# wenxuanliu/multimodal-vae

Measured on AMD Instinct MI355X. Metric: ELBO-steps/sec (whole node), MultiMNIST b=256 per GPU, higher is better.
Workload: dtype bf16; 1 GPU; multimnist_50x50_conv_mmvae_gru_text_3pass_elbo_step; batch_per_gpu=256, global_batch=256, n_latents=100, parallelism=dp1, hip_graph=False, optimizer=adam, mfma=bf16 in / fp32 acc; fp32 master weights, BN stats, PoE/KL/BCE/NLL, Adam

## Files before the change

multimodal-vae_amd/csrc/conv1.hip:

```cpp
#include "thin.h"
#include "convres_epi.h"

namespace {

constexpr int C1_IMG = 50, C1_OH = 25, C1_NPIX = 625, C1_TILES = 20, C1_ROWS = 640, C1_C = 32;
constexpr int C1_HW = 52;
constexpr int C1_PP = 48;
constexpr int C1_AP = 80;

typedef __attribute__((address_space(3))) s16x4 lds_s16x4e;
__device__ __forceinline__ bf16x8 tr_pair_e(const char* a0, const char* a1) {
    union { struct { s16x4 a, b; } s; bf16x8 v; } u;
    u.s.a = __builtin_amdgcn_ds_read_tr16_b64_v4i16((lds_s16x4e*)a0);
    u.s.b = __builtin_amdgcn_ds_read_tr16_b64_v4i16((lds_s16x4e*)a1);
    return u.v;
}

template <int NTHR>
__device__ __forceinline__ void c1_patches(const float* img, bf16* img_s, char* pat_s, int tid) {
    for (int i = tid; i < C1_HW * C1_HW; i += NTHR) {
        const int y = i / C1_HW - 1, x = i - (y + 1) * C1_HW - 1;
        img_s[i] = ((unsigned)y < (unsigned)C1_IMG && (unsigned)x < (unsigned)C1_IMG) ? (bf16)img[y * C1_IMG + x] : (bf16)0.f;
    }
    __syncthreads();
    for (int px = tid; px < C1_ROWS; px += NTHR) {
        bf16x8 lo, hi;
        if (px < C1_NPIX) {
            const int oy = px / C1_OH, ox = px - oy * C1_OH;
            const bf16* d0 = img_s + (2 * oy) * C1_HW + 2 * ox;
#pragma unroll
            for (int kw = 0; kw < 4; ++kw) {
                lo[kw] = d0[kw]; lo[4 + kw] = d0[C1_HW + kw];
                hi[kw] = d0[2 * C1_HW + kw]; hi[4 + kw] = d0[3 * C1_HW + kw];
            }
        } else {
#pragma unroll
            for (int j = 0; j < 8; ++j) { lo[j] = (bf16)0.f; hi[j] = (bf16)0.f; }
        }
        *reinterpret_cast<bf16x8*>(pat_s + px * C1_PP) = lo;
        *reinterpret_cast<bf16x8*>(pat_s + px * C1_PP + 16) = hi;
    }
    __syncthreads();
}

struct Conv1FwdArgs { const float* image; int B; const bf16* Wp; int Kpad; bf16* r1; bf16* a1; };

constexpr int C1F_WAVES = 4, C1F_NTHR = C1F_WAVES * 64;
constexpr int C1F_OFF_IMG = 0, C1F_OFF_PAT = C1F_OFF_IMG + ((C1_HW * C1_HW * 2 + 15) / 16) * 16, C1F_OFF_SCR = C1F_OFF_PAT + C1_ROWS * C1_PP,
              C1F_LDS = C1F_OFF_SCR + C1F_WAVES * 2560;

__global__ __launch_bounds__(C1F_NTHR) void conv1_fwd_mfma_kernel(const Conv1FwdArgs a) {
    extern __shared__ __attribute__((aligned(16))) char smem[];
    const int tid = threadIdx.x, lane = tid & 63;
    const int wave = __builtin_amdgcn_readfirstlane(tid >> 6);
    const int r = lane & 31, h = lane >> 5;
    const int n = blockIdx.x;
    c1_patches<C1F_NTHR>(a.image + (size_t)n * (C1_IMG * C1_IMG), reinterpret_cast<bf16*>(smem + C1F_OFF_IMG), smem + C1F_OFF_PAT, tid);
    const bf16x8 wb = *reinterpret_cast<const bf16x8*>(a.Wp + (size_t)r * a.Kpad + 8 * h);
    const size_t bytes = (size_t)a.B * C1_NPIX * C1_C * 2;
    const __amdgpu_buffer_rsrc_t rsrc_r = __builtin_amdgcn_make_buffer_rsrc(a.r1, 0, (int)bytes, 0x00020000);
    const __amdgpu_buffer_rsrc_t rsrc_a = __builtin_amdgcn_make_buffer_rsrc(a.a1, 0, (int)bytes, 0x00020000);
    char* const scr = smem + C1F_OFF_SCR + wave * 2560;
    float s1 = 0.f, s2 = 0.f;
    for (int t = wave; t < C1_TILES; t += C1F_WAVES) {
        f32x16 acc;
#pragma unroll
        for (int j = 0; j < 16; ++j) acc[j] = 0.f;
        const bf16x8 pa = *reinterpret_cast<const bf16x8*>(smem + C1F_OFF_PAT + (t * 32 + r) * C1_PP + h * 16);
        acc = __builtin_amdgcn_mfma_f32_32x32x16_bf16(pa, wb, acc, 0, 0, 0);
        const unsigned base = (unsigned)(((size_t)n * C1_NPIX + t * 32) * (C1_C * 2)) + (unsigned)((lane >> 4) * 16);
        const int p0 = t * 32 + (lane & 15), p1 = p0 + 16;
        const unsigned off0 = p0 < C1_NPIX ? base + (unsigned)((lane & 15) * (C1_C * 2)) : 0x40000000u;
        const unsigned off1 = p1 < C1_NPIX ? base + (unsigned)((16 + (lane & 15)) * (C1_C * 2)) : 0x40000000u;
        f32x16 act;
#pragma unroll
        for (int j = 0; j < 16; ++j) act[j] = swish_fast(acc[j]);
        cr_epilogue_tile<0, false>(acc, scr, lane, 32, off0, off1, rsrc_r, rsrc_r, 1.f, 0.f, 0.f, 0.f, s1, s2, true);
        cr_epilogue_tile<0, false>(act, scr, lane, 32, off0, off1, rsrc_a, rsrc_a, 1.f, 0.f, 0.f, 0.f, s1, s2, true);
    }
}

struct Conv1WgradArgs { const float* image; int B; const bf16* d1; float* dWp; int Kpad; };

constexpr int C1W_WAVES = 8, C1W_NTHR = C1W_WAVES * 64;
constexpr int C1W_OFF_D = 0, C1W_OFF_IMG = C1W_OFF_D + C1_ROWS * C1_AP, C1W_OFF_PAT = C1W_OFF_IMG + ((C1_HW * C1_HW * 2 + 15) / 16) * 16,
              C1W_OFF_RED = C1W_OFF_PAT + C1_ROWS * C1_PP, C1W_LDS = C1W_OFF_RED + C1W_WAVES * C1_C * 16 * 4;

__global__ __launch_bounds__(C1W_NTHR) void conv1_wgrad_mfma_kernel(const Conv1WgradArgs a) {
    extern __shared__ __attribute__((aligned(16))) char smem[];
    const int tid = threadIdx.x, lane = tid & 63;
    const int wave = __builtin_amdgcn_readfirstlane(tid >> 6);
    const int r = lane & 31, h = lane >> 5;
    const int n = blockIdx.x;
    char* const D_s = smem + C1W_OFF_D;
    {
        constexpr int NV = C1_NPIX * 4;
        const bf16* src = a.d1 + (size_t)n * C1_NPIX * C1_C;
        for (int v = tid; v < C1_ROWS * 4; v += C1W_NTHR) {
            i32x4c val = {0, 0, 0, 0};
            if (v < NV) val = *reinterpret_cast<const i32x4c*>(src + (size_t)v * 8);
            *reinterpret_cast<i32x4c*>(D_s + (v >> 2) * C1_AP + (v & 3) * 16) = val;
        }
    }
    c1_patches<C1W_NTHR>(a.image + (size_t)n * (C1_IMG * C1_IMG), reinterpret_cast<bf16*>(smem + C1W_OFF_IMG), smem + C1W_OFF_PAT, tid);
    const int g4 = lane >> 4, q = (lane & 15) >> 2, p = lane & 3;
    f32x16 acc;
#pragma unroll
    for (int j = 0; j < 16; ++j) acc[j] = 0.f;
    for (int ks = wave; ks < C1_ROWS / 16; ks += C1W_WAVES) {
        const int row = ks * 16 + 8 * h + q;
        const char* a0 = D_s + row * C1_AP + (16 * (g4 & 1) + 4 * p) * 2;
        const char* b0 = smem + C1W_OFF_PAT + row * C1_PP + (4 * p) * 2;
        acc = __builtin_amdgcn_mfma_f32_32x32x16_bf16(tr_pair_e(a0, a0 + 4 * C1_AP), tr_pair_e(b0, b0 + 4 * C1_PP), acc, 0, 0, 0);
    }
    float* wred = reinterpret_cast<float*>(smem + C1W_OFF_RED) + wave * (C1_C * 16);
    if (r < 16) {
#pragma unroll
        for (int j = 0; j < 16; ++j) wred[((j & 3) + 8 * (j >> 2) + 4 * h) * 16 + r] = acc[j];
    }
    __syncthreads();
    {
        const float* wr = reinterpret_cast<const float*>(smem + C1W_OFF_RED);
        for (int i = tid; i < C1_C * 16; i += C1W_NTHR) {
            float s = 0.f;
#pragma unroll
            for (int w = 0; w < C1W_WAVES; ++w) s += wr[w * C1_C * 16 + i];
            atomicAdd(a.dWp + (size_t)(i >> 4) * a.Kpad + (i & 15), s);
        }
    }
}

}

int launch_conv1_fwd_mfma(const float* image, int B, const bf16* Wp, int Kpad, bf16* r1, bf16* a1, hipStream_t s) {
    MMVAE_REQUIRE(image && Wp && r1 && a1 && Kpad >= 16 && (size_t)B * C1_NPIX * C1_C * 2 < 0x40000000ull, "conv1 fwd: arguments");
    Conv1FwdArgs a{image, B, Wp, Kpad, r1, a1};
    MMVAE_LAUNCH(conv1_fwd_mfma_kernel, dim3(B), dim3(C1F_NTHR), C1F_LDS, s, a);
    return mmvae_check_launch("conv1_fwd_mfma");
}
int launch_conv1_wgrad_mfma(const float* image, int B, const bf16* d1, float* dWp, int Kpad, hipStream_t s) {
    MMVAE_REQUIRE(image && d1 && dWp && Kpad >= 16, "conv1 wgrad: arguments");
    static std::atomic<unsigned> attr_set{0};
    if (mmvae_first_use_on_device(attr_set))
        hipFuncSetAttribute(reinterpret_cast<const void*>(&conv1_wgrad_mfma_kernel), hipFuncAttributeMaxDynamicSharedMemorySize, C1W_LDS);
    Conv1WgradArgs a{image, B, d1, dWp, Kpad};
    MMVAE_LAUNCH(conv1_wgrad_mfma_kernel, dim3(B), dim3(C1W_NTHR), C1W_LDS, s, a);
    return mmvae_check_launch("conv1_wgrad_mfma");
}
```

multimodal-vae_amd/csrc/convres_epi.h:

```cpp
#pragma once
#include "common.h"

namespace {

typedef __attribute__((ext_vector_type(16))) float f32x16;
typedef __attribute__((ext_vector_type(4))) int i32x4c;

__device__ __forceinline__ float dswish_fast(float x) {
    const float s = __builtin_amdgcn_rcpf(1.0f + __expf(-x));
    return s * (1.0f + x * (1.0f - s));
}
__device__ __forceinline__ float swish_fast(float x) { return x * __builtin_amdgcn_rcpf(1.0f + __expf(-x)); }

typedef __attribute__((ext_vector_type(2))) float f32x2;
typedef __attribute__((address_space(3))) s16x4 lds_s16x4c;

template <int MODE, bool PARTIAL>
__device__ __forceinline__ void cr_epilogue_tile(const f32x16& acc, char* scr, int lane, int rows_valid, unsigned off0, unsigned off1,
                                                 __amdgpu_buffer_rsrc_t orsrc, __amdgpu_buffer_rsrc_t rrsrc, float dsc, float dsh,
                                                 float dmean, float drstd, float& s1, float& s2, bool store) {
    constexpr int SP = 80;
    const int r = lane & 31, h = lane >> 5, g = lane >> 4, i = lane & 15, q = i >> 2, p = i & 3;
    float v[16];
#pragma unroll
    for (int j = 0; j < 16; ++j) v[j] = acc[j];
    if constexpr (MODE == 1) {
        const i32x4c r0 = __builtin_bit_cast(i32x4c, __builtin_amdgcn_raw_buffer_load_b128(rrsrc, (int)off0, 0, 0));
        const i32x4c r1 = __builtin_bit_cast(i32x4c, __builtin_amdgcn_raw_buffer_load_b128(rrsrc, (int)off1, 0, 0));
        *reinterpret_cast<i32x4c*>(scr + i * SP + g * 16) = r0;
        *reinterpret_cast<i32x4c*>(scr + (16 + i) * SP + g * 16) = r1;
        asm volatile("" ::: "memory");
        const char* rb = scr + (4 * h + q) * SP + (16 * ((lane >> 4) & 1) + 4 * p) * 2;
        f32x2 t1 = {0.f, 0.f}, t2 = {0.f, 0.f};
#pragma unroll
        for (int k = 0; k < 4; ++k) {
            const bf16x4 rv = __builtin_bit_cast(bf16x4, __builtin_amdgcn_ds_read_tr16_b64_v4i16((lds_s16x4c*)(rb + 8 * k * SP)));
#pragma unroll
            for (int e = 0; e < 4; e += 2) {
                const f32x2 rr = {(float)rv[e], (float)rv[e + 1]};
                const f32x2 x = rr * dsc + dsh;
                f32x2 d = {dswish_fast(x[0]), dswish_fast(x[1])};
                f32x2 o = {v[4 * k + e], v[4 * k + e + 1]};
                o *= d;
                if constexpr (PARTIAL) {
                    const int row = 8 * k + 4 * h + e;
                    o[0] = row < rows_valid ? o[0] : 0.f;
                    o[1] = row + 1 < rows_valid ? o[1] : 0.f;
                }
                t1 += o;
                t2 += o * ((rr - dmean) * drstd);
                v[4 * k + e] = o[0]; v[4 * k + e + 1] = o[1];
            }
        }
        s1 += t1[0] + t1[1];
        s2 += t2[0] + t2[1];
        asm volatile("" ::: "memory");
    } else {
        f32x2 t1 = {0.f, 0.f}, t2 = {0.f, 0.f};
#pragma unroll
        for (int j = 0; j < 16; j += 2) {
            f32x2 o = {v[j], v[j + 1]};
            if constexpr (PARTIAL) {
                const int row = (j & 3) + 8 * (j >> 2) + 4 * h;
                o[0] = row < rows_valid ? o[0] : 0.f;
                o[1] = row + 1 < rows_valid ? o[1] : 0.f;
                v[j] = o[0]; v[j + 1] = o[1];
            }
            t1 += o;
            t2 += o * o;
        }
        s1 += t1[0] + t1[1];
        s2 += t2[0] + t2[1];
    }
#pragma unroll
    for (int k = 0; k < 4; ++k) {
        bf16x4 o;
#pragma unroll
        for (int e = 0; e < 4; ++e) o[e] = (bf16)v[4 * k + e];
        *reinterpret_cast<bf16x4*>(scr + r * SP + (8 * k + 4 * h) * 2) = o;
    }
    asm volatile("" ::: "memory");
    if (store) {
        const char* ob = scr + (8 * g + q) * SP + (4 * p) * 2;
        union { struct { s16x4 a, b; } s; i32x4c v; } u0, u1;
        u0.s.a = __builtin_amdgcn_ds_read_tr16_b64_v4i16((lds_s16x4c*)(ob));
        u0.s.b = __builtin_amdgcn_ds_read_tr16_b64_v4i16((lds_s16x4c*)(ob + 4 * SP));
        u1.s.a = __builtin_amdgcn_ds_read_tr16_b64_v4i16((lds_s16x4c*)(ob + 32));
        u1.s.b = __builtin_amdgcn_ds_read_tr16_b64_v4i16((lds_s16x4c*)(ob + 4 * SP + 32));
        __builtin_amdgcn_raw_buffer_store_b128(u0.v, orsrc, (int)off0, 0, 0);
        __builtin_amdgcn_raw_buffer_store_b128(u1.v, orsrc, (int)off1, 0, 0);
    }
    asm volatile("" ::: "memory");
}

}
```

multimodal-vae_amd/csrc/dec_last.hip:

```cpp
#include "thin.h"
#include "bn_dev.h"
#include "convres_epi.h"

namespace {

constexpr int DL_IH = 25, DL_IW = 25, DL_OH = 50, DL_OW = 50, DL_C = 32, DL_NPIX = 625, DL_TILES = 20, DL_ROWS = 640;
constexpr int DL_AP = 80;
constexpr int DL_PP = 48;
constexpr int DL_DLW = 52;
constexpr int DL_WAVES = 8, DL_NTHR = DL_WAVES * 64;
constexpr int DL_OFF_A = 0;
constexpr int DL_OFF_P = DL_OFF_A + DL_ROWS * DL_AP;
constexpr int DL_OFF_DL = DL_OFF_P + DL_ROWS * 64;
constexpr int DL_OFF_SCR = DL_OFF_DL + DL_DLW * DL_DLW * 4;
constexpr int DL_OFF_TAB = DL_OFF_SCR + DL_WAVES * 2560;
constexpr int DL_LDS = DL_OFF_TAB + 2 * DL_C * 8;
static_assert(DL_ROWS * DL_PP <= DL_ROWS * 64, "the patches reuse the P buffer");
static_assert(DL_LDS <= 160 * 1024, "LDS budget");

typedef __attribute__((address_space(3))) s16x4 lds_s16x4d;
__device__ __forceinline__ bf16x8 tr_pair_d(const char* a0, const char* a1) {
    union { struct { s16x4 a, b; } s; bf16x8 v; } u;
    u.s.a = __builtin_amdgcn_ds_read_tr16_b64_v4i16((lds_s16x4d*)a0);
    u.s.b = __builtin_amdgcn_ds_read_tr16_b64_v4i16((lds_s16x4d*)a1);
    return u.v;
}

template <bool IW>
__global__ __launch_bounds__(DL_NTHR) void dec_last_mfma_kernel(const DecLastFusedArgs a) {
    extern __shared__ __attribute__((aligned(16))) char smem[];
    char* const A_s = smem + DL_OFF_A;
    float* const P_s = reinterpret_cast<float*>(smem + DL_OFF_P);
    char* const pat_s = smem + DL_OFF_P;
    float* const dl_s = reinterpret_cast<float*>(smem + DL_OFF_DL);
    char* const scr_s = smem + DL_OFF_SCR;
    float2* const aff_s = reinterpret_cast<float2*>(smem + DL_OFF_TAB);
    float2* const mr_s = aff_s + DL_C;
    __shared__ float part[DL_WAVES];

    const int tid = threadIdx.x, lane = tid & 63;
    const int wave = __builtin_amdgcn_readfirstlane(tid >> 6);
    const int r = lane & 31, h = lane >> 5;
    const int n_in_g = blockIdx.x, g = blockIdx.y;
    const long long n = (long long)g * a.B + n_in_g;
    const BnFinalizeArgs& f = a.fin;
    const bool bwd = g < a.bwd_groups;

    constexpr int NV = DL_NPIX * 4, IT = (NV + DL_NTHR - 1) / DL_NTHR;
    i32x4c rv[IT];
#pragma unroll
    for (int it = 0; it < IT; ++it) {
        const int v = tid + it * DL_NTHR;
        if (v < NV) rv[it] = *reinterpret_cast<const i32x4c*>(a.r + (size_t)n * DL_NPIX * DL_C + (size_t)v * 8);
    }
    if (tid < DL_C) {
        float2 aff, mr;
        bn_channel_tables(f, g, tid, aff, mr);
        aff_s[tid] = aff; mr_s[tid] = mr;
    }
    if (!IW && blockIdx.x == 0 && blockIdx.y == 0) {
        for (int i = tid; i < f.G * DL_C; i += DL_NTHR) {
            float2 aff, mr;
            bn_channel_tables(f, i / DL_C, i % DL_C, aff, mr);
            f.affine[i] = aff; f.meanrstd[i] = mr;
        }
        bn_running_update(f, tid, DL_NTHR);
    }
    {
        const i32x4c z = {0, 0, 0, 0};
        for (int i = tid * 16; i < (DL_ROWS - DL_NPIX) * DL_AP; i += DL_NTHR * 16)
            *reinterpret_cast<i32x4c*>(A_s + DL_NPIX * DL_AP + i) = z;
        if (!IW)
            for (int i = tid; i < DL_DLW * DL_DLW; i += DL_NTHR) dl_s[i] = 0.f;
    }
    bf16x8 wf[2], wd;
#pragma unroll
    for (int ks = 0; ks < 2; ++ks)
#pragma unroll
        for (int j = 0; j < 8; ++j) wf[ks][j] = r < 16 ? (bf16)a.w[(ks * 16 + 8 * h + j) * 16 + r] : (bf16)0.f;
#pragma unroll
    for (int j = 0; j < 8; ++j) wd[j] = (bf16)a.w[r * 16 + 8 * h + j];
    __syncthreads();
    {
        const int cv = tid & 3;
        float sc[8], sh[8];
#pragma unroll
        for (int j = 0; j < 8; ++j) { const float2 t = aff_s[cv * 8 + j]; sc[j] = t.x; sh[j] = t.y; }
#pragma unroll
        for (int it = 0; it < IT; ++it) {
            const int v = tid + it * DL_NTHR;
            if (v < NV) {
                const bf16x8 x = __builtin_bit_cast(bf16x8, rv[it]);
                bf16x8 o;
#pragma unroll
                for (int j = 0; j < 8; ++j) o[j] = (bf16)swish_fast((float)x[j] * sc[j] + sh[j]);
                *reinterpret_cast<bf16x8*>(A_s + (v >> 2) * DL_AP + cv * 16) = o;
            }
        }
    }
    __syncthreads();
    for (int t = wave; t < DL_TILES; t += DL_WAVES) {
        f32x16 acc;
#pragma unroll
        for (int j = 0; j < 16; ++j) acc[j] = 0.f;
        const char* ap = A_s + (t * 32 + r) * DL_AP + h * 16;
        const bf16x8 a0 = *reinterpret_cast<const bf16x8*>(ap), a1 = *reinterpret_cast<const bf16x8*>(ap + 32);
        acc = __builtin_amdgcn_mfma_f32_32x32x16_bf16(a0, wf[0], acc, 0, 0, 0);
        acc = __builtin_amdgcn_mfma_f32_32x32x16_bf16(a1, wf[1], acc, 0, 0, 0);
        if (r < 16) {
#pragma unroll
            for (int j = 0; j < 16; ++j) P_s[(t * 32 + (j & 3) + 8 * (j >> 2) + 4 * h) * 16 + r] = acc[j];
        }
    }
    __syncthreads();
    if constexpr (IW) {
        const float* const timg = a.target + (long long)(n / a.rows_per_target) * (DL_OH * DL_OW);
        float ll = 0.f;
        for (int o = tid; o < DL_OH * DL_OW; o += DL_NTHR) {
            const int oy = o / DL_OW, ox = o - oy * DL_OW;
            const int kh0 = (oy + 1) & 1, kw0 = (ox + 1) & 1;
            const int iy0 = (oy + 1 - kh0) >> 1, ix0 = (ox + 1 - kw0) >> 1;
            float acc = 0.f;
#pragma unroll
            for (int ty = 0; ty < 2; ++ty)
#pragma unroll
                for (int tx = 0; tx < 2; ++tx) {
                    const int iy = iy0 - ty, ix = ix0 - tx;
                    if ((unsigned)iy < (unsigned)DL_IH && (unsigned)ix < (unsigned)DL_IW)
                        acc += P_s[(iy * DL_IW + ix) * 16 + (kh0 + 2 * ty) * 4 + kw0 + 2 * tx];
                }
            ll += timg[o] * acc - (fmaxf(acc, 0.f) + log1pf(expf(-fabsf(acc))));
        }
        ll = wave_sum(ll);
        if (lane == 0) part[wave] = ll;
        __syncthreads();
        if (tid == 0) {
            float s = 0.f;
            for (int w = 0; w < DL_WAVES; ++w) s += part[w];
            a.loglik[n] = s;
        }
        return;
    }
    float loss = 0.f;
    for (int o = tid; o < DL_OH * DL_OW; o += DL_NTHR) {
        const int oy = o / DL_OW, ox = o - oy * DL_OW;
        const int kh0 = (oy + 1) & 1, kw0 = (ox + 1) & 1;
        const int iy0 = (oy + 1 - kh0) >> 1, ix0 = (ox + 1 - kw0) >> 1;
        float acc = 0.f;
#pragma unroll
        for (int ty = 0; ty < 2; ++ty)
#pragma unroll
            for (int tx = 0; tx < 2; ++tx) {
                const int iy = iy0 - ty, ix = ix0 - tx;
                if ((unsigned)iy < (unsigned)DL_IH && (unsigned)ix < (unsigned)DL_IW)
                    acc += P_s[(iy * DL_IW + ix) * 16 + (kh0 + 2 * ty) * 4 + kw0 + 2 * tx];
            }
        const long long oidx = n * (DL_OH * DL_OW) + o;
        const float p = __builtin_amdgcn_rcpf(1.0f + __expf(-acc));
        if (a.logits) a.logits[oidx] = acc;
        if (a.recon) a.recon[oidx] = p;
        if (a.target) {
            const float t = a.target[(long long)n_in_g * (DL_OH * DL_OW) + o];
            const float lp = fmaxf(__logf(p), -100.f), lq = fmaxf(__logf(1.0f - p), -100.f);
            loss += -(t * lp + (1.0f - t) * lq);
            const float pq = p * (1.0f - p);
            const float dl = a.coef[g] * (p - t) / fmaxf(pq, 1e-12f) * pq;
            if (a.dlogit) a.dlogit[oidx] = dl;
            dl_s[(oy + 1) * DL_DLW + ox + 1] = dl;
        }
    }
    if (a.loss_sum) {
        loss = wave_sum(loss);
        if (lane == 0) part[wave] = loss;
    }
    __syncthreads();
    if (a.loss_sum && tid == 0) {
        float s = 0.f;
        for (int w = 0; w < DL_WAVES; ++w) s += part[w];
        atomicAdd(a.loss_sum + (blockIdx.x % MMVAE_LOSS_SLOTS) * 16 + g, s);
    }
    if (!bwd) return;
    for (int px = tid; px < DL_ROWS; px += DL_NTHR) {
        bf16x8 lo, hi;
        if (px < DL_NPIX) {
            const int iy = px / DL_IW, ix = px - iy * DL_IW;
            const float* d0 = dl_s + (2 * iy) * DL_DLW + 2 * ix;
#pragma unroll
            for (int kw = 0; kw < 4; ++kw) {
                lo[kw] = (bf16)d0[kw]; lo[4 + kw] = (bf16)d0[DL_DLW + kw];
                hi[kw] = (bf16)d0[2 * DL_DLW + kw]; hi[4 + kw] = (bf16)d0[3 * DL_DLW + kw];
            }
        } else {
#pragma unroll
            for (int j = 0; j < 8; ++j) { lo[j] = (bf16)0.f; hi[j] = (bf16)0.f; }
        }
        *reinterpret_cast<bf16x8*>(pat_s + px * DL_PP) = lo;
        *reinterpret_cast<bf16x8*>(pat_s + px * DL_PP + 16) = hi;
    }
    __syncthreads();
    {
        const __amdgpu_buffer_rsrc_t orsrc = __builtin_amdgcn_make_buffer_rsrc(
            a.db, 0, (int)((size_t)a.bwd_groups * a.B * DL_NPIX * DL_C * 2), 0x00020000);
        const __amdgpu_buffer_rsrc_t rrsrc = __builtin_amdgcn_make_buffer_rsrc(
            const_cast<bf16*>(a.r), 0, (int)((size_t)a.bwd_groups * a.B * DL_NPIX * DL_C * 2), 0x00020000);
        const float2 af = aff_s[r], mr = mr_s[r];
        float s1 = 0.f, s2 = 0.f;
        char* const scr = scr_s + wave * 2560;
        for (int t = wave; t < DL_TILES; t += DL_WAVES) {
            f32x16 acc;
#pragma unroll
            for (int j = 0; j < 16; ++j) acc[j] = 0.f;
            const bf16x8 pa = *reinterpret_cast<const bf16x8*>(pat_s + (t * 32 + r) * DL_PP + h * 16);
            acc = __builtin_amdgcn_mfma_f32_32x32x16_bf16(pa, wd, acc, 0, 0, 0);
            const unsigned base = (unsigned)((n * DL_NPIX + t * 32) * (DL_C * 2)) + (unsigned)((lane >> 4) * 16);
            const int p0 = t * 32 + (lane & 15), p1 = p0 + 16;
            const unsigned off0 = p0 < DL_NPIX ? base + (unsigned)((lane & 15) * (DL_C * 2)) : 0x40000000u;
            const unsigned off1 = p1 < DL_NPIX ? base + (unsigned)((16 + (lane & 15)) * (DL_C * 2)) : 0x40000000u;
            const int left = DL_NPIX - t * 32;
            if (left >= 32) cr_epilogue_tile<1, false>(acc, scr, lane, 32, off0, off1, orsrc, rrsrc, af.x, af.y, mr.x, mr.y, s1, s2, true);
            else cr_epilogue_tile<1, true>(acc, scr, lane, left, off0, off1, orsrc, rrsrc, af.x, af.y, mr.x, mr.y, s1, s2, true);
        }
        const float t1 = s1 + __shfl_xor(s1, 32, 64), t2 = s2 + __shfl_xor(s2, 32, 64);
        if (h == 0) {
            const int slot = (int)(blockIdx.x + wave) % MMVAE_STAT_SLOTS;
            float2* d = a.red + ((size_t)g * MMVAE_STAT_SLOTS + slot) * DL_C + r;
            atomicAdd(&d->x, t1);
            atomicAdd(&d->y, t2);
        }
    }
    __syncthreads();
    {
        const int g4 = lane >> 4, q = (lane & 15) >> 2, p = lane & 3;
        f32x16 acc;
#pragma unroll
        for (int j = 0; j < 16; ++j) acc[j] = 0.f;
        for (int ks = wave; ks < DL_ROWS / 16; ks += DL_WAVES) {
            const int row = ks * 16 + 8 * h + q;
            const char* a0 = A_s + row * DL_AP + (16 * (g4 & 1) + 4 * p) * 2;
            const char* b0 = pat_s + row * DL_PP + (4 * p) * 2;
            const bf16x8 af2 = tr_pair_d(a0, a0 + 4 * DL_AP);
            const bf16x8 bf2 = tr_pair_d(b0, b0 + 4 * DL_PP);
            acc = __builtin_amdgcn_mfma_f32_32x32x16_bf16(af2, bf2, acc, 0, 0, 0);
        }
        float* wred = reinterpret_cast<float*>(scr_s) + wave * (DL_C * 16);
        if (r < 16) {
#pragma unroll
            for (int j = 0; j < 16; ++j) wred[((j & 3) + 8 * (j >> 2) + 4 * h) * 16 + r] = acc[j];
        }
    }
    __syncthreads();
    {
        const float* wred = reinterpret_cast<const float*>(scr_s);
        float* dst = a.wslab + ((size_t)g * gridDim.x + blockIdx.x) * DL_C * 16;
        for (int i = tid; i < DL_C * 16; i += DL_NTHR) {
            float s = 0.f;
#pragma unroll
            for (int w = 0; w < DL_WAVES; ++w) s += wred[w * DL_C * 16 + i];
            dst[i] = s;
        }
    }
}

constexpr int CL_IH = 32, CL_IW = 32, CL_OH = 64, CL_OW = 64, CL_C = 32, CL_CO = 3, CL_J = 48, CL_SR = 8, CL_NS = CL_IH / CL_SR;
constexpr int CL_NPIX = CL_IH * CL_IW;
constexpr int CL_AROWS = CL_SR + 2, CL_APX = CL_AROWS * CL_IW, CL_ATILES = CL_APX / 32;
constexpr int CL_OPX = CL_SR * CL_IW, CL_OTILES = CL_OPX / 32;
constexpr int CL_AP = 80;
constexpr int CL_PF = 49;
constexpr int CL_PP = 144;
constexpr int CL_DLR = 2 * CL_SR + 2, CL_DLW = CL_OW + 2;
constexpr int CL_WAVES = 8, CL_NTHR = CL_WAVES * 64;
constexpr int CL_OFF_A = 0;
constexpr int CL_OFF_P = CL_OFF_A + CL_APX * CL_AP;
constexpr int CL_P_BYTES = CL_APX * CL_PF * 4;
constexpr int CL_OFF_DL = CL_OFF_P + (CL_P_BYTES + 15) / 16 * 16;
constexpr int CL_OFF_SCR = CL_OFF_DL + (CL_CO * CL_DLR * CL_DLW * 4 + 15) / 16 * 16;
constexpr int CL_OFF_TAB = CL_OFF_SCR + CL_WAVES * 2560;
constexpr int CL_LDS = CL_OFF_TAB + 2 * CL_C * 8;
static_assert(CL_OPX * CL_PP <= CL_P_BYTES && CL_WAVES * CL_C * CL_J * 4 <= CL_P_BYTES, "patches / dW partials reuse the P buffer");
static_assert(CL_LDS <= 160 * 1024 - 64, "LDS budget");
static_assert(CL_OTILES == CL_WAVES, "one owned 32-pixel tile per wave");

__global__ __launch_bounds__(CL_NTHR) void dec_last_ca_kernel(const DecLastFusedArgs a) {
    extern __shared__ __attribute__((aligned(16))) char smem[];
    char* const A_s = smem + CL_OFF_A;
    float* const P_s = reinterpret_cast<float*>(smem + CL_OFF_P);
    char* const pat_s = smem + CL_OFF_P;
    float* const dl_s = reinterpret_cast<float*>(smem + CL_OFF_DL);
    char* const scr_s = smem + CL_OFF_SCR;
    float2* const aff_s = reinterpret_cast<float2*>(smem + CL_OFF_TAB);
    float2* const mr_s = aff_s + CL_C;
    __shared__ float part[CL_WAVES];

    const int tid = threadIdx.x, lane = tid & 63;
    const int wave = __builtin_amdgcn_readfirstlane(tid >> 6);
    const int r = lane & 31, h = lane >> 5;
    const int n_in_g = blockIdx.x, g = blockIdx.y;
    const long long n = (long long)g * a.B + n_in_g;
    const BnFinalizeArgs& f = a.fin;
    const bool bwd = g < a.bwd_groups;

    if (tid < CL_C) {
        float2 aff, mr;
        bn_channel_tables(f, g, tid, aff, mr);
        aff_s[tid] = aff; mr_s[tid] = mr;
    }
    if (blockIdx.x == 0 && blockIdx.y == 0) {
        for (int i = tid; i < f.G * CL_C; i += CL_NTHR) {
            float2 aff, mr;
            bn_channel_tables(f, i / CL_C, i % CL_C, aff, mr);
            f.affine[i] = aff; f.meanrstd[i] = mr;
        }
        bn_running_update(f, tid, CL_NTHR);
    }
    bf16x8 wf[2][2], wd[3];
#pragma unroll
    for (int ks = 0; ks < 2; ++ks)
#pragma unroll
        for (int nt = 0; nt < 2; ++nt) {
            const int j = nt * 32 + r, tap = j / CL_CO, co = j - tap * CL_CO;
#pragma unroll
            for (int e = 0; e < 8; ++e) wf[ks][nt][e] = j < CL_J ? (bf16)a.w[((ks * 16 + 8 * h + e) * CL_CO + co) * 16 + tap] : (bf16)0.f;
        }
#pragma unroll
    for (int ks = 0; ks < 3; ++ks)
#pragma unroll
        for (int e = 0; e < 8; ++e) {
            const int j = ks * 16 + 8 * h + e, tap = j / CL_CO, co = j - tap * CL_CO;
            wd[ks][e] = (bf16)a.w[(r * CL_CO + co) * 16 + tap];
        }
    __syncthreads();
    const int cv = tid & 3;
    float sc[8], sh[8];
#pragma unroll
    for (int e = 0; e < 8; ++e) { const float2 t = aff_s[cv * 8 + e]; sc[e] = t.x; sh[e] = t.y; }
    const float2 af = aff_s[r], mr = mr_s[r];

    const __amdgpu_buffer_rsrc_t orsrc = __builtin_amdgcn_make_buffer_rsrc(
        a.db, 0, (int)((size_t)a.bwd_groups * a.B * CL_NPIX * CL_C * 2), 0x00020000);
    const __amdgpu_buffer_rsrc_t rrsrc = __builtin_amdgcn_make_buffer_rsrc(
        const_cast<bf16*>(a.r), 0, (int)((size_t)a.bwd_groups * a.B * CL_NPIX * CL_C * 2), 0x00020000);
    f32x16 accw[2];
#pragma unroll
    for (int nt = 0; nt < 2; ++nt)
#pragma unroll
        for (int e = 0; e < 16; ++e) accw[nt][e] = 0.f;
    float s1 = 0.f, s2 = 0.f, loss = 0.f;
    const bf16* const rimg = a.r + (size_t)n * CL_NPIX * CL_C;
    constexpr int NV = CL_APX * 4, IT = (NV + CL_NTHR - 1) / CL_NTHR;

    constexpr int NO = CL_CO * CL_DLR * CL_OW;
    constexpr int ND = CL_CO * CL_DLR * CL_DLW, DT = (ND + CL_NTHR - 1) / CL_NTHR;
    i32x4c rv[IT];
    auto fetch_rows = [&](int y0) {
#pragma unroll
        for (int it = 0; it < IT; ++it) {
            const int v = tid + it * CL_NTHR, px = v >> 2, iy = y0 - 1 + px / CL_IW;
            rv[it] = i32x4c{0, 0, 0, 0};
            if (v < NV && (unsigned)iy < (unsigned)CL_IH)
                rv[it] = *reinterpret_cast<const i32x4c*>(rimg + ((size_t)(iy * CL_IW + (px & (CL_IW - 1))) * CL_C + cv * 8));
        }
    };
    fetch_rows(0);
    const float* const timg = a.target ? a.target + (size_t)n_in_g * CL_CO * CL_OH * CL_OW : nullptr;
    float tv[DT];
    auto fetch_targets = [&](int y0) {
#pragma unroll
        for (int k = 0; k < DT; ++k) {
            const int i = tid + k * CL_NTHR;
            const int co = i / (CL_DLR * CL_DLW), rem = i - co * (CL_DLR * CL_DLW);
            const int lo = rem / CL_DLW, c = rem - lo * CL_DLW, oy = 2 * y0 - 1 + lo;
            tv[k] = 0.f;
            if (timg && i < ND && c >= 1 && c <= CL_OW && (unsigned)oy < (unsigned)CL_OH) tv[k] = timg[(co * CL_OH + oy) * CL_OW + c - 1];
        }
    };
    fetch_targets(0);

    for (int strip = 0; strip < CL_NS; ++strip) {
        const int y0 = strip * CL_SR;
        __syncthreads();
#pragma unroll
        for (int k = 0; k < DT; ++k) {
            const int i = tid + k * CL_NTHR;
            if (i < ND) dl_s[i] = tv[k];
        }
#pragma unroll
        for (int it = 0; it < IT; ++it) {
            const int v = tid + it * CL_NTHR, px = v >> 2, iy = y0 - 1 + px / CL_IW;
            if (v < NV) {
                bf16x8 o;
                if ((unsigned)iy < (unsigned)CL_IH) {
                    const bf16x8 x = __builtin_bit_cast(bf16x8, rv[it]);
#pragma unroll
                    for (int e = 0; e < 8; ++e) o[e] = (bf16)swish_fast((float)x[e] * sc[e] + sh[e]);
                } else {
#pragma unroll
                    for (int e = 0; e < 8; ++e) o[e] = (bf16)0.f;
                }
                *reinterpret_cast<bf16x8*>(A_s + px * CL_AP + cv * 16) = o;
            }
        }
        if (strip + 1 < CL_NS) { fetch_rows(y0 + CL_SR); fetch_targets(y0 + CL_SR); }
        __syncthreads();
        if (!(a.dbg & 16))
        for (int t = wave; t < CL_ATILES; t += CL_WAVES) {
            const char* ap = A_s + (t * 32 + r) * CL_AP + h * 16;
            const bf16x8 a0 = *reinterpret_cast<const bf16x8*>(ap), a1 = *reinterpret_cast<const bf16x8*>(ap + 32);
#pragma unroll
            for (int nt = 0; nt < 2; ++nt) {
                f32x16 acc;
#pragma unroll
                for (int e = 0; e < 16; ++e) acc[e] = 0.f;
                acc = __builtin_amdgcn_mfma_f32_32x32x16_bf16(a0, wf[0][nt], acc, 0, 0, 0);
                acc = __builtin_amdgcn_mfma_f32_32x32x16_bf16(a1, wf[1][nt], acc, 0, 0, 0);
                const int j = nt * 32 + r;
                if (j < CL_J) {
#pragma unroll
                    for (int e = 0; e < 16; ++e) P_s[(t * 32 + (e & 3) + 8 * (e >> 2) + 4 * h) * CL_PF + j] = acc[e];
                }
            }
        }
        __syncthreads();
#pragma unroll 2
        for (int o = (a.dbg & 1) ? NO : tid; o < NO; o += CL_NTHR) {
            const int co = o / (CL_DLR * CL_OW), rem = o - co * (CL_DLR * CL_OW);
            const int lo = rem / CL_OW, ox = rem - lo * CL_OW, oy = 2 * y0 - 1 + lo;
            if ((unsigned)oy >= (unsigned)CL_OH) continue;
            const int kh0 = (oy + 1) & 1, kw0 = (ox + 1) & 1;
            const int iy0 = (oy + 1 - kh0) >> 1, ix0 = (ox + 1 - kw0) >> 1;
            float acc = 0.f;
#pragma unroll
            for (int ty = 0; ty < 2; ++ty)
#pragma unroll
                for (int tx = 0; tx < 2; ++tx) {
                    const int iy = iy0 - ty, ix = ix0 - tx, ixc = min(max(ix, 0), CL_IW - 1);
                    const float pv = P_s[((iy - y0 + 1) * CL_IW + ixc) * CL_PF + ((kh0 + 2 * ty) * 4 + kw0 + 2 * tx) * CL_CO + co];
                    acc += ix == ixc ? pv : 0.f;
                }
            const bool owned = lo >= 1 && lo <= 2 * CL_SR;
            const long long oidx = ((n * CL_CO + co) * CL_OH + oy) * CL_OW + ox;
            const float p = __builtin_amdgcn_rcpf(1.0f + __expf(-acc));
            if (owned) {
                if (a.logits) a.logits[oidx] = acc;
                if (a.recon) a.recon[oidx] = p;
            }
            if (a.target) {
                const float t = dl_s[(co * CL_DLR + lo) * CL_DLW + ox + 1];
                const float pq = p * (1.0f - p);
                const float dl = a.coef[g] * (p - t) / fmaxf(pq, 1e-12f) * pq;
                if (owned) {
                    const float lp = fmaxf(__logf(p), -100.f), lq = fmaxf(__logf(1.0f - p), -100.f);
                    loss += -(t * lp + (1.0f - t) * lq);
                    if (a.dlogit) a.dlogit[oidx] = dl;
                }
                dl_s[(co * CL_DLR + lo) * CL_DLW + ox + 1] = dl;
            }
        }
        if (!bwd) continue;
        __syncthreads();
        if (!(a.dbg & 2)) {
            const int px = tid >> 1, half = tid & 1;
            const int iyl = px / CL_IW, ix = px - iyl * CL_IW;
            bf16 v[24];
#pragma unroll
            for (int kk = 0; kk < 2; ++kk)
#pragma unroll
                for (int kw = 0; kw < 4; ++kw)
#pragma unroll
                    for (int co = 0; co < CL_CO; ++co)
                        v[(kk * 4 + kw) * CL_CO + co] = (bf16)dl_s[(co * CL_DLR + 2 * iyl + 2 * half + kk) * CL_DLW + 2 * ix + kw];
            char* dst = pat_s + px * CL_PP + half * 48;
#pragma unroll
            for (int q = 0; q < 3; ++q) {
                bf16x8 o;
#pragma unroll
                for (int e = 0; e < 8; ++e) o[e] = v[q * 8 + e];
                *reinterpret_cast<bf16x8*>(dst + q * 16) = o;
            }
            if (half) {
                const i32x4c z = {0, 0, 0, 0};
                *reinterpret_cast<i32x4c*>(pat_s + px * CL_PP + 96) = z;
                *reinterpret_cast<i32x4c*>(pat_s + px * CL_PP + 112) = z;
            }
        }
        __syncthreads();
        if (!(a.dbg & 4)) {
            const int t = wave;
            f32x16 acc;
#pragma unroll
            for (int e = 0; e < 16; ++e) acc[e] = 0.f;
#pragma unroll
            for (int ks = 0; ks < 3; ++ks) {
                const bf16x8 pa = *reinterpret_cast<const bf16x8*>(pat_s + (t * 32 + r) * CL_PP + ks * 32 + h * 16);
                acc = __builtin_amdgcn_mfma_f32_32x32x16_bf16(pa, wd[ks], acc, 0, 0, 0);
            }
            const unsigned base = (unsigned)((n * CL_NPIX + y0 * CL_IW + t * 32) * (CL_C * 2)) + (unsigned)((lane >> 4) * 16);
            const unsigned off0 = base + (unsigned)((lane & 15) * (CL_C * 2)), off1 = base + (unsigned)((16 + (lane & 15)) * (CL_C * 2));
            cr_epilogue_tile<1, false>(acc, scr_s + wave * 2560, lane, 32, off0, off1, orsrc, rrsrc, af.x, af.y, mr.x, mr.y, s1, s2, true);
        }
        if (!(a.dbg & 8)) {
            const int g4 = lane >> 4, q = (lane & 15) >> 2, p = lane & 3;
            for (int ks = wave; ks < CL_OPX / 16; ks += CL_WAVES) {
                const int row = ks * 16 + 8 * h + q;
                const char* a0 = A_s + (row + CL_IW) * CL_AP + (16 * (g4 & 1) + 4 * p) * 2;
                const bf16x8 af2 = tr_pair_d(a0, a0 + 4 * CL_AP);
#pragma unroll
                for (int nt = 0; nt < 2; ++nt) {
                    const char* b0 = pat_s + row * CL_PP + (nt * 32 + 16 * (g4 & 1) + 4 * p) * 2;
                    const bf16x8 bf2 = tr_pair_d(b0, b0 + 4 * CL_PP);
                    accw[nt] = __builtin_amdgcn_mfma_f32_32x32x16_bf16(af2, bf2, accw[nt], 0, 0, 0);
                }
            }
        }
    }
    if (a.loss_sum) {
        loss = wave_sum(loss);
        if (lane == 0) part[wave] = loss;
    }
    __syncthreads();
    if (a.loss_sum && tid == 0) {
        float s = 0.f;
        for (int w = 0; w < CL_WAVES; ++w) s += part[w];
        atomicAdd(a.loss_sum + (blockIdx.x % MMVAE_LOSS_SLOTS) * 16 + g, s);
    }
    if (!bwd) return;
    {
        const float t1 = s1 + __shfl_xor(s1, 32, 64), t2 = s2 + __shfl_xor(s2, 32, 64);
        if (h == 0) {
            const int slot = (int)(blockIdx.x + wave) % MMVAE_STAT_SLOTS;
            float2* d = a.red + ((size_t)g * MMVAE_STAT_SLOTS + slot) * CL_C + r;
            atomicAdd(&d->x, t1);
            atomicAdd(&d->y, t2);
        }
    }
    float* const wred = P_s;
#pragma unroll
    for (int nt = 0; nt < 2; ++nt) {
        const int j = nt * 32 + r;
        if (j < CL_J) {
#pragma unroll
            for (int e = 0; e < 16; ++e) wred[(wave * CL_C + (e & 3) + 8 * (e >> 2) + 4 * h) * CL_J + j] = accw[nt][e];
        }
    }
    __syncthreads();
    float* dst = a.wslab + ((size_t)g * gridDim.x + blockIdx.x) * CL_C * CL_J;
    for (int i = tid; i < CL_C * CL_J; i += CL_NTHR) {
        float s = 0.f;
#pragma unroll
        for (int w = 0; w < CL_WAVES; ++w) s += wred[w * CL_C * CL_J + i];
        dst[i] = s;
    }
}

}

bool dec_last_ca_applies(const DecLastFusedArgs& a) {
    return a.Cin == CL_C && a.Cout == CL_CO && a.IH == CL_IH && a.IW == CL_IW && a.act == ACT_SWISH && mmvae_knob("dec_last_ca", 1) != 0 &&
           (size_t)a.G * a.B * CL_NPIX * CL_C * 2 < 0x40000000ull;
}
int launch_dec_last_ca(const DecLastFusedArgs& a, hipStream_t s) {
    MMVAE_REQUIRE(dec_last_ca_applies(a), "dec_last_ca: not the 32x32x32 -> 64x64x3 tail");
    MMVAE_REQUIRE(a.r && a.w && a.G >= 1 && a.B >= 1 && a.bwd_groups >= 0 && a.bwd_groups <= a.G, "dec_last_ca: arguments");
    MMVAE_REQUIRE(a.bwd_groups == 0 || (a.target && a.db && a.red && a.wslab), "dec_last_ca: backward outputs missing");
    static std::atomic<unsigned> attr_set{0};
    if (mmvae_first_use_on_device(attr_set))
        hipFuncSetAttribute(reinterpret_cast<const void*>(&dec_last_ca_kernel), hipFuncAttributeMaxDynamicSharedMemorySize, CL_LDS);
    DecLastFusedArgs b = a;
    b.dbg = mmvae_knob("dec_last_ca_dbg", 0);
    MMVAE_LAUNCH(dec_last_ca_kernel, dim3(a.B, a.G), dim3(CL_NTHR), CL_LDS, s, b);
    return mmvae_check_launch("dec_last_ca");
}

bool dec_last_mfma_applies(const DecLastFusedArgs& a) {
    return a.Cin == 32 && a.Cout == 1 && a.IH == DL_IH && a.IW == DL_IW && a.act == ACT_SWISH && mmvae_knob("dec_last_mfma", 1) != 0 &&
           (size_t)a.G * a.B * DL_NPIX * DL_C * 2 < 0x40000000ull;
}
int launch_dec_last_mfma(const DecLastFusedArgs& a, hipStream_t s) {
    static std::atomic<unsigned> attr_set{0};
    if (mmvae_first_use_on_device(attr_set)) {
        hipFuncSetAttribute(reinterpret_cast<const void*>(&dec_last_mfma_kernel<false>), hipFuncAttributeMaxDynamicSharedMemorySize, DL_LDS);
        hipFuncSetAttribute(reinterpret_cast<const void*>(&dec_last_mfma_kernel<true>), hipFuncAttributeMaxDynamicSharedMemorySize, DL_LDS);
    }
    if (a.loglik) {
        MMVAE_REQUIRE(a.target && a.rows_per_target >= 1 && a.bwd_groups == 0 && !a.fin.training, "dec_last_mfma: importance-weighted form arguments");
        MMVAE_LAUNCH(dec_last_mfma_kernel<true>, dim3(a.B, a.G), dim3(DL_NTHR), DL_LDS, s, a);
        return mmvae_check_launch("dec_last_mfma_iw");
    }
    MMVAE_LAUNCH(dec_last_mfma_kernel<false>, dim3(a.B, a.G), dim3(DL_NTHR), DL_LDS, s, a);
    return mmvae_check_launch("dec_last_mfma");
}
```

multimodal-vae_amd/csrc/multimnist.hip:

```cpp
#include "multimnist.h"
#include <memory>
#include "mlp_tail.h"
#include "plan_base.h"
#include "thin.h"
#include "text_plan.h"
#include <cstring>

namespace {
constexpr int IMG = 50, NPIX = 2500;
}

struct MMPlan : PlanBase {
    int ldz, kx, kz;
    int lde;
    ConvL conv[4], convT[4];
    LinL fc[3], up;
    BnL bn[6];
    int H = TXT_H;
    const char *te_name = "text_encoder", *td_name = "text_decoder";
    TextGruIdx te_f, te_r, td0, td1;
    const float* step_image = nullptr;
    hipEvent_t ev_dz = nullptr;
    hipEvent_t ev_txtgrads = nullptr;
    int te_h2p, te_h2pT, g_te_h2p, td_z2h, td_z2hT, g_td_z2h, td_h2o, td_h2oT, g_td_h2o;
    bool mlp_tail = false;
    int mt_w2, mt_w3, mt_w3t, mt_w2t;
    bool waist = false;
    int wa_w2, wa_w3, wa_w3t, wa_w2t;
    struct W {
        char* zero_begin; size_t zero_bytes;
        float2 *st_e[3], *red_e[3], *st_d[3], *red_d[3];
        float* sums; float* dz_img; float* dz_txt;
        float2 *aff_e[3], *mr_e[3], *aff_d[3], *mr_d[3];
        bf16 *patches1, *r1, *r2, *r3, *r4, *y1, *y2;
        bf16 *a1, *a2, *a3, *a4, *ay1, *ay2, *au, *aq1, *aq2, *aq3;
        float* encout; uint8_t *m1, *m2, *gkeep;
        float *txtout, *te_gates_f, *te_gates_r; bf16 *te_x, *te_hprev, *te_hsum;
        float *eps, *mu, *logvar, *z_f32; bf16* z_bf;
        bf16 *u, *q1, *q2, *q3; float *logits, *recon, *dlogit;
        float *words, *dwords, *td_gates; long long* tokens;
        bf16 *td_x0, *td_h0p, *td_mid, *td_h1p, *td_hz, *td_zbf;
        bf16 *dgi0, *dgh0, *dgi1, *dgh1, *dlogit_bf, *dhinit;
        bf16 *patches4, *d3, *d2, *d1, *du;
        bf16 *d_encout; float* d_txtout; bf16* te_dout_bf; bf16 *te_dgi_f, *te_dgh_f, *te_dgi_r;
        bf16 *dy2, *dy1, *db4, *dr4, *d3e, *d2e, *d1e;
        bf16 *d3r, *d2r, *d1r, *d3er, *d2er;
        float* tmp_f32;
        float* slab; size_t slab_floats;
    } w;
};

namespace {

void build_params(MMPlan& P) {
    const int D = P.D;
    auto bn = [&](const std::string& n, int c) { add_param(P, n + ".weight", {c}); add_param(P, n + ".bias", {c}); };
    add_param(P, "image_encoder.features.0.weight", {32, 1, 4, 4});
    add_param(P, "image_encoder.features.2.weight", {64, 32, 4, 4}); bn("image_encoder.features.3", 64);
    add_param(P, "image_encoder.features.5.weight", {128, 64, 4, 4}); bn("image_encoder.features.6", 128);
    add_param(P, "image_encoder.features.8.weight", {256, 128, 4, 4}); bn("image_encoder.features.9", 256);
    add_param(P, "image_encoder.classifier.0.weight", {400, 1024}); add_param(P, "image_encoder.classifier.0.bias", {400});
    add_param(P, "image_encoder.classifier.3.weight", {200, 400}); add_param(P, "image_encoder.classifier.3.bias", {200});
    add_param(P, "image_encoder.classifier.6.weight", {2 * D, 200}); add_param(P, "image_encoder.classifier.6.bias", {2 * D});
    add_param(P, "image_decoder.upsample.0.weight", {1024, D}); add_param(P, "image_decoder.upsample.0.bias", {1024});
    add_param(P, "image_decoder.hallucinate.0.weight", {256, 128, 4, 4}); bn("image_decoder.hallucinate.1", 128);
    add_param(P, "image_decoder.hallucinate.3.weight", {128, 64, 4, 4}); bn("image_decoder.hallucinate.4", 64);
    add_param(P, "image_decoder.hallucinate.6.weight", {64, 32, 5, 5}); bn("image_decoder.hallucinate.7", 32);
    add_param(P, "image_decoder.hallucinate.9.weight", {32, 1, 4, 4});
    text_add_encoder_params(P);
    text_add_decoder_params(P);
}

void build_plan(MMPlan& P) {
    const int D = P.D;
    P.ldz = round_up(D + 1, 8); P.kz = round_up(D, 32); P.kx = txt_kx(P.H, D);
    P.lde = round_up(2 * D, 8);
    build_params(P);
    const char* bnn[6] = {"image_encoder.features.3", "image_encoder.features.6", "image_encoder.features.9",
                          "image_decoder.hallucinate.1", "image_decoder.hallucinate.4", "image_decoder.hallucinate.7"};
    const int bnc[6] = {64, 128, 256, 128, 64, 32};
    long long so = 0;
    for (int i = 0; i < 6; ++i) {
        P.bn[i] = BnL{off(P, std::string(bnn[i]) + ".weight"), off(P, std::string(bnn[i]) + ".bias"), bnc[i], so, i};
        P.bn_names.push_back(bnn[i]); P.bn_list.push_back(P.bn[i]);
        so += 2 * bnc[i];
    }
    build_conv(P, P.conv[0], "image_encoder.features.0.weight", ConvGeom{1, 32, 4, 4, 2, 1, 50, 50, 25, 25, false}, -1, false, true, false);
    build_conv(P, P.conv[1], "image_encoder.features.2.weight", ConvGeom{32, 64, 4, 4, 2, 1, 25, 25, 12, 12, false}, 0, true, false, false);
    build_conv(P, P.conv[2], "image_encoder.features.5.weight", ConvGeom{64, 128, 4, 4, 2, 1, 12, 12, 6, 6, false}, 1, true, false, false);
    build_conv(P, P.conv[3], "image_encoder.features.8.weight", ConvGeom{128, 256, 4, 4, 2, 0, 6, 6, 2, 2, false}, 2, true, false, false);
    build_conv(P, P.convT[0], "image_decoder.hallucinate.0.weight", ConvGeom{256, 128, 4, 4, 2, 0, 2, 2, 6, 6, true}, 3, true, false, false);
    build_conv(P, P.convT[1], "image_decoder.hallucinate.3.weight", ConvGeom{128, 64, 4, 4, 2, 1, 6, 6, 12, 12, true}, 4, true, false, false);
    build_conv(P, P.convT[2], "image_decoder.hallucinate.6.weight", ConvGeom{64, 32, 5, 5, 2, 1, 12, 12, 25, 25, true}, 5, true, false, false);
    build_conv(P, P.convT[3], "image_decoder.hallucinate.9.weight", ConvGeom{32, 1, 4, 4, 2, 1, 25, 25, 50, 50, true}, -1, true, false, true);
    add_frag_packs(P, P.conv[2]);
    add_frag_packs(P, P.convT[1]);
    add_frag_packs(P, P.conv[3]);
    add_frag_packs(P, P.convT[0]);

    {
        LinL& f = P.fc[0];
        f.w_off = off(P, "image_encoder.classifier.0.weight"); f.b_off = off(P, "image_encoder.classifier.0.bias");
        f.N = 400; f.K = 1024; f.pk_dgrad = -1;
        PackDesc d = pack_dense(f.w_off, 400, 1024, npad_for(400), 1024, 1024, 0);
        d.TW = 2; d.C = 256; d.s_ty = 2; d.s_tx = 1; d.s_c = 4;
        f.pk_fwd = P.pk.add(d);
        PackDesc gd = d; gd.Npad = round_up(400, 64);
        f.gk = P.gk.add(gd);
        for (int sidx = 0; sidx < 4; ++sidx)
            f.pk_dgrad4[sidx] = P.pk.add(pack_dense(f.w_off + sidx, 256, 400, npad_for(256), round_up(400, 64), 4, 1024));
    }
    auto lin = [&](LinL& f, const std::string& n, int N, int K) {
        f.w_off = off(P, n + ".weight"); f.b_off = off(P, n + ".bias"); f.N = N; f.K = K;
        f.pk_fwd = P.pk.add(pack_dense(f.w_off, N, K, npad_for(N), round_up(round_up(K, 8), 64), K, 1));
        f.gk = P.gk.add(pack_dense(f.w_off, N, K, round_up(N, 64), round_up(round_up(K, 8), 64), K, 1));
        f.pk_dgrad = P.pk.add(pack_dense(f.w_off, K, N, npad_for(K), round_up(round_up(N, 8), 64), 1, K));
    };
    lin(P.fc[1], "image_encoder.classifier.3", 200, 400);
    lin(P.fc[2], "image_encoder.classifier.6", 2 * D, 200);
    if (D == 100) {
        P.mlp_tail = true;
        auto fragd = [&](PackDesc d) { d.frag = 1; return P.pk.add(d); };
        P.mt_w2 = fragd(pack_dense(P.fc[1].w_off, 200, 400, 208, 416, 400, 1));
        P.mt_w3 = fragd(pack_dense(P.fc[2].w_off, 200, 200, 208, 224, 200, 1));
        P.mt_w3t = fragd(pack_dense(P.fc[2].w_off, 200, 200, 208, 224, 1, 200));
        P.mt_w2t = fragd(pack_dense(P.fc[1].w_off, 400, 200, 400, 224, 1, 400));
        P.waist = true; P.wa_w2 = P.mt_w2; P.wa_w3 = P.mt_w3; P.wa_w3t = P.mt_w3t; P.wa_w2t = P.mt_w2t;
    } else if (mlp2_latent1_compiled(D)) {
        P.waist = true;
        auto fragd = [&](PackDesc d) { d.frag = 1; return P.pk.add(d); };
        P.wa_w2 = fragd(pack_dense(P.fc[1].w_off, 200, 400, 208, 416, 400, 1));
        P.wa_w3 = fragd(pack_dense(P.fc[2].w_off, 2 * D, 200, round_up(2 * D, 16), 224, 200, 1));
        P.wa_w3t = fragd(pack_dense(P.fc[2].w_off, 200, 2 * D, 208, round_up(2 * D, 32), 1, 200));
        P.wa_w2t = fragd(pack_dense(P.fc[1].w_off, 400, 200, 400, 224, 1, 400));
    }
    {
        LinL& f = P.up;
        f.w_off = off(P, "image_decoder.upsample.0.weight"); f.b_off = off(P, "image_decoder.upsample.0.bias");
        f.N = 1024; f.K = D;
        PackDesc d = pack_dense(f.w_off, 1024, D, npad_for(1024), round_up(P.ldz, 64), 0, 1);
        d.NL = 256; d.s_nhi = D; d.s_nlo = 4 * D;
        d.bias_off = f.b_off; d.b_nhi = 1; d.b_nlo = 4;
        f.pk_fwd = P.pk.add(d);
        PackDesc gd = d; f.gk = P.gk.add(gd);
        PackDesc t = pack_dense(f.w_off, D, 1024, npad_for(D), 1024, 1, 0);
        t.TW = 4; t.C = 256; t.s_ty = 0; t.s_tx = D; t.s_c = 4 * D;
        f.pk_dgrad = P.pk.add(t);
    }
    text_build_packs(P);
    for (PackDesc& d : P.pk.d) {
        d.part = 0;
        for (const ParamInfo& pi : P.params)
            if (d.src_off >= pi.offset && d.src_off < pi.offset + pi.numel)
                d.part = pi.name.rfind("text_", 0) == 0 ? 1 : pi.name.rfind("image_decoder.", 0) == 0 ? 2 : 0;
    }
    {
        auto late = [&](int idx) { if (idx >= 0) P.pk.d[idx].part = 2; };
        for (int l = 0; l < 4; ++l)
            for (int i = 0; i < 4; ++i) { late(P.conv[l].pk_dgrad[i]); late(P.conv[l].pk_dgrad_f[i]); }
        for (int i = 0; i < 4; ++i) late(P.fc[0].pk_dgrad4[i]);
        late(P.fc[1].pk_dgrad); late(P.fc[2].pk_dgrad);
        if (P.waist) { late(P.wa_w3t); late(P.wa_w2t); }
    }
    for (PackDesc& d : P.gk.d)
        for (const ParamInfo& pi : P.params)
            if (d.src_off >= pi.offset && d.src_off < pi.offset + pi.numel)
                d.part = pi.name.rfind("image_decoder.", 0) == 0 || pi.name.rfind("text_decoder.", 0) == 0;
}

void carve(MMPlan& P, Workspace& ws) {
    MMPlan::W& w = P.w;
    const size_t B = P.B, D = P.D, B3 = (size_t)P.carve_passes * B, B2 = (size_t)(P.carve_passes < 2 ? P.carve_passes : 2) * B;
    char* z0 = ws.take<char>(0);
    const int ec[3] = {64, 128, 256}, dc[3] = {128, 64, 32};
    const int SS = MMVAE_STAT_SLOTS;
    for (int i = 0; i < 3; ++i) { w.st_e[i] = ws.take<float2>(SS * ec[i]); w.red_e[i] = ws.take<float2>(SS * ec[i]); }
    for (int i = 0; i < 3; ++i) { w.st_d[i] = ws.take<float2>(3 * SS * dc[i]); w.red_d[i] = ws.take<float2>(3 * SS * dc[i]); }
    w.sums = ws.take<float>(16 * MMVAE_LOSS_SLOTS);
    P.sk_cnt = ws.take<unsigned>(1024);
    w.dz_img = ws.take<float>(B3 * D);
    w.dz_txt = ws.take<float>(B3 * D);
    char* z1 = ws.take<char>(0);
    w.zero_begin = z0; w.zero_bytes = (size_t)(z1 - z0);
    for (int i = 0; i < 3; ++i) { w.aff_e[i] = ws.take<float2>(ec[i]); w.mr_e[i] = ws.take<float2>(ec[i]); }
    for (int i = 0; i < 3; ++i) { w.aff_d[i] = ws.take<float2>(3 * dc[i]); w.mr_d[i] = ws.take<float2>(3 * dc[i]); }
    w.patches1 = ws.take<bf16>(B * 625 * 16);
    w.r1 = ws.take<bf16>(B * 625 * 32); w.r2 = ws.take<bf16>(B * 144 * 64); w.r3 = ws.take<bf16>(B * 36 * 128);
    w.r4 = ws.take<bf16>(B * 4 * 256);
    w.y1 = ws.take<bf16>(B2 * 400); w.y2 = ws.take<bf16>(B2 * 200);
    w.a1 = ws.take<bf16>(B * 625 * 32); w.a2 = ws.take<bf16>(B * 144 * 64); w.a3 = ws.take<bf16>(B * 36 * 128);
    w.a4 = ws.take<bf16>(B * 4 * 256); w.ay1 = ws.take<bf16>(B2 * 400); w.ay2 = ws.take<bf16>(B2 * 200);
    w.au = ws.take<bf16>(B3 * 1024); w.aq1 = ws.take<bf16>(B3 * 36 * 128); w.aq2 = ws.take<bf16>(B3 * 144 * 64);
    w.aq3 = ws.take<bf16>(B3 * 625 * 32);
    w.encout = ws.take<float>(B2 * 2 * D);
    w.m1 = ws.take<uint8_t>(B2 * 400); w.m2 = ws.take<uint8_t>(B2 * 200); w.gkeep = ws.take<uint8_t>(4 * B3 * P.H);
    carve_text_enc(w, ws, B, D, P.H);
    w.eps = ws.take<float>(B3 * D); w.mu = ws.take<float>(B3 * D); w.logvar = ws.take<float>(B3 * D);
    w.z_f32 = ws.take<float>(B3 * D); w.z_bf = ws.take<bf16>(B3 * P.ldz);
    w.u = ws.take<bf16>(B3 * 1024); w.q1 = ws.take<bf16>(B3 * 36 * 128); w.q2 = ws.take<bf16>(B3 * 144 * 64);
    w.q3 = ws.take<bf16>(B3 * 625 * 32);
    w.logits = ws.take<float>(B3 * NPIX); w.recon = ws.take<float>(B3 * NPIX); w.dlogit = ws.take<float>(B3 * NPIX);
    carve_text_dec(w, ws, B3, P.H, P.kx, P.kz);
    w.patches4 = ws.take<bf16>(B3 * 625 * 16);
    w.d3 = ws.take<bf16>(B3 * 625 * 32); w.d2 = ws.take<bf16>(B3 * 144 * 64); w.d1 = ws.take<bf16>(B3 * 36 * 128);
    w.du = ws.take<bf16>(B3 * 1024);
    w.d_encout = ws.take<bf16>(B2 * P.lde);
    carve_text_enc_bwd(w, ws, B, D, P.H);
    w.dy2 = ws.take<bf16>(B2 * 200); w.dy1 = ws.take<bf16>(B2 * 400);
    w.db4 = ws.take<bf16>(B2 * 1024); w.dr4 = ws.take<bf16>(B * 1024);
    w.d3e = ws.take<bf16>(B * 36 * 128); w.d2e = ws.take<bf16>(B * 144 * 64); w.d1e = ws.take<bf16>(B * 625 * 32);
    w.d3r = ws.take<bf16>(B3 * 625 * 32); w.d2r = ws.take<bf16>(B3 * 144 * 64); w.d1r = ws.take<bf16>(B3 * 36 * 128);
    w.d3er = ws.take<bf16>(B * 36 * 128); w.d2er = ws.take<bf16>(B * 144 * 64);
    w.tmp_f32 = ws.take<float>(B3 * NPIX);
    P.sk_floats = (size_t)256 * 128 * 128;
    P.sk_buf = ws.take<float>(P.sk_floats);
    w.slab_floats = (size_t)(P.carve_passes >= 3 ? 48 : 16) << 20;
    w.slab = ws.take<float>(w.slab_floats);
}

int enc_fwd(MMPlan& P, const float* image, int variants, const uint8_t* m1, const uint8_t* m2, int dropout, int training,
            int bn_updates, float* out, hipStream_t s, bool fuse = false, const Mlp2Latent1FwdArgs* waist = nullptr, bool tail_only = false) {
    MMPlan::W& w = P.w;
    const int B = P.B;
    const int rows = variants * B;
    const bool drop = training && dropout;
    const float ms = 1.f / (1.f - DROP_P);
    if (!tail_only) {
    if (fuse && mmvae_knob("mm_conv1_mfma", 1)) {
        const PackDesc& d = P.pk.d[P.conv[0].pk_fwd[0]];
        MMVAE_TRY(launch_conv1_fwd_mfma(image, B, P.buf.packed + d.dst_off, d.Kpad, w.r1, w.a1, s));
    } else {
    MMVAE_TRY(launch_im2col_small(image, B, 1, IMG, IMG, 4, 4, 2, 1, 25, 25, w.patches1, 16, s));
    {
        GatherPlan pl = dense_plan(B * 625, 16, 16, 32);
        GemmParams g = gemm_of(P, pl, P.conv[0].pk_fwd, 1, B * 625);
        g.c.A = w.patches1; g.out_bf = w.r1; g.ldo = 32; g.out_act_bf = w.a1; g.e_act = ACT_SWISH;
        MMVAE_TRY(launch_gemm_gather(g, s));
    }
    }
    bf16* r[4] = {w.r1, w.r2, w.r3, w.r4};
    bf16* a[4] = {w.a1, w.a2, w.a3, w.a4};
    for (int l = 1; l < 4; ++l) {
        const ConvL& L = P.conv[l];
        GemmParams g = gemm_of(P, L.fwd, L.pk_fwd, 1, B, L.pk_fwd_f);
        g.c.A = a[l - 1];
        g.out_bf = r[l]; g.ldo = L.g.Cout;
        g.colstats = training ? w.st_e[l - 1] : nullptr;
        GatherTransform tr{};
        if (fuse && l >= 2) {
            const int prows = B * P.conv[l - 1].g.OH * P.conv[l - 1].g.OW;
            tr.kind = 1;
            tr.fin = bn_fin_args(P, P.bn[P.conv[l - 1].bn], prows, 1, w.st_e[l - 2], bn_updates, w.aff_e[l - 2], w.mr_e[l - 2], training);
            g.c.A = r[l - 1]; g.tr = &tr;
            if (mmvae_knob("mm_stage_out", 1)) tr.out = a[l - 1];
        }
        MMVAE_TRY(launch_gemm_gather(g, s));
        const int rows = B * L.g.OH * L.g.OW;
        if (fuse && l <= 2) continue;
        MMVAE_TRY(bn_act(P, P.bn[L.bn], r[l], a[l], rows, rows, 1, w.st_e[l - 1], bn_updates, w.aff_e[l - 1], w.mr_e[l - 1], training, s));
    }
    {
        GatherPlan pl = plan_fwdform(2, 2, 1, 1, 256, 2, 2, 1, 0, 400, 1, rows);
        GemmParams g = gemm_of(P, pl, &P.fc[0].pk_fwd, 1, rows);
        g.c.A = w.a4; g.c.a_bcast_n = B;
        g.bias = P.buf.params + P.fc[0].b_off; g.out_bf = w.y1; g.ldo = 400;
        g.out_act_bf = w.ay1; g.e_act = ACT_SWISH; if (drop) { g.e_mask = m1; g.e_mask_scale = ms; }
        MMVAE_TRY(launch_gemm_gather(g, s));
    }
    }
    if (waist) {
        Mlp2Latent1FwdArgs a = *waist;
        a.rows = rows; a.x = w.ay1;
        a.w2 = P.buf.packed + P.pk.d[P.wa_w2].dst_off; a.b2 = P.buf.params + P.fc[1].b_off;
        a.w3 = P.buf.packed + P.pk.d[P.wa_w3].dst_off; a.b3 = P.buf.params + P.fc[2].b_off;
        if (drop) { a.mask = m2; a.mask_scale = ms; }
        a.y2 = w.y2; a.ay2 = w.ay2; a.out = out;
        return launch_mlp2_latent1_fwd(a, s);
    }
    if (P.mlp_tail) {
        Mlp2FwdArgs a{};
        a.rows = rows; a.x = w.ay1;
        a.w2 = P.buf.packed + P.pk.d[P.mt_w2].dst_off; a.b2 = P.buf.params + P.fc[1].b_off;
        a.w3 = P.buf.packed + P.pk.d[P.mt_w3].dst_off; a.b3 = P.buf.params + P.fc[2].b_off;
        if (drop) { a.mask = m2; a.mask_scale = ms; }
        a.y2 = w.y2; a.ay2 = w.ay2; a.out = out;
        return launch_mlp2_fwd(a, s);
    }
    {
        GatherPlan pl = dense_plan(rows, 400, 400, 200);
        GemmParams g = gemm_of(P, pl, &P.fc[1].pk_fwd, 1, rows);
        g.c.A = w.ay1;
        g.bias = P.buf.params + P.fc[1].b_off; g.out_bf = w.y2; g.ldo = 200;
        g.out_act_bf = w.ay2; g.e_act = ACT_SWISH; if (drop) { g.e_mask = m2; g.e_mask_scale = ms; }
        MMVAE_TRY(launch_gemm_gather(g, s));
    }
    {
        GatherPlan pl = dense_plan(rows, 200, 200, 2 * P.D);
        GemmParams g = gemm_of(P, pl, &P.fc[2].pk_fwd, 1, rows);
        g.c.A = w.ay2;
        g.bias = P.buf.params + P.fc[2].b_off; g.out_f = out; g.ldo = 2 * P.D;
        MMVAE_TRY(launch_gemm_gather(g, s));
    }
    return MMVAE_OK;
}

int enc_bwd(MMPlan& P, const bf16* d_out, int variants, const uint8_t* m1, const uint8_t* m2, int dropout, hipStream_t s, bool fuse = false,
            const Mlp2Latent1BwdArgs* waist = nullptr, float* loss_out = nullptr, bool tail_only = false) {
    MMPlan::W& w = P.w;
    const int B = P.B, rows = variants * B, D2 = 2 * P.D;
    const float ms = 1.f / (1.f - DROP_P);
    auto cls_w = std::make_shared<std::vector<WgradParams>>();
    if (waist) {
        Mlp2Latent1BwdArgs a = *waist;
        a.rows = rows;
        a.w3t = P.buf.packed + P.pk.d[P.wa_w3t].dst_off; a.w2t = P.buf.packed + P.pk.d[P.wa_w2t].dst_off;
        a.y2 = w.y2; a.y1 = w.y1;
        if (dropout) { a.mask2 = m2; a.mask1 = m1; a.mask_scale = ms; }
        a.dy2 = w.dy2; a.dy1 = w.dy1;
        a.db2 = P.buf.grads + P.fc[1].b_off; a.db1 = P.buf.grads + P.fc[0].b_off;
        a.d_enc_out = w.d_encout; a.lde = P.lde;
        MMVAE_TRY(launch_mlp2_latent1_bwd(a, s));
        {
            hipStream_t fs = s;
            MMVAE_TRY(wgrad_side_stream(P, s, &fs));
            MMVAE_TRY(launch_mlp2_latent1_finish(a.scratch, rows, P.D, P.buf.grads + P.fc[2].b_off, w.sums, loss_out, fs));
        }
        GatherPlan p3 = dense_plan(rows, 200, 200, D2);
        WgradParams g3 = wgrad_of(P, p3, &P.fc[2].gk, 1, rows);
        g3.c.A = w.ay2; g3.P = w.d_encout; g3.ldp = P.lde;
        MMVAE_TRY(wgrad_async(P, g3, s));
        GatherPlan p2 = dense_plan(rows, 400, 400, 200);
        WgradParams g2 = wgrad_of(P, p2, &P.fc[1].gk, 1, rows);
        g2.c.A = w.ay1; g2.P = w.dy2; g2.ldp = 200;
        MMVAE_TRY(wgrad_async(P, g2, s));
    } else if (P.mlp_tail) {
        {
            GatherPlan pl = dense_plan(rows, 200, 200, D2);
            WgradParams g = wgrad_of(P, pl, &P.fc[2].gk, 1, rows);
            g.c.A = w.ay2; g.P = d_out; g.ldp = P.lde;
            if (fuse) cls_w->push_back(g);
            else MMVAE_TRY(wgrad_async(P, g, s));
        }
        Mlp2BwdArgs a{};
        a.rows = rows; a.d_out = d_out;
        a.w3t = P.buf.packed + P.pk.d[P.mt_w3t].dst_off; a.w2t = P.buf.packed + P.pk.d[P.mt_w2t].dst_off;
        a.y2 = w.y2; a.y1 = w.y1;
        if (dropout) { a.mask2 = m2; a.mask1 = m1; a.mask_scale = ms; }
        a.dy2 = w.dy2; a.dy1 = w.dy1;
        a.db2 = P.buf.grads + P.fc[1].b_off; a.db1 = P.buf.grads + P.fc[0].b_off;
        MMVAE_TRY(launch_mlp2_bwd(a, s));
        GatherPlan pl = dense_plan(rows, 400, 400, 200);
        WgradParams g = wgrad_of(P, pl, &P.fc[1].gk, 1, rows);
        g.c.A = w.ay1; g.P = w.dy2; g.ldp = 200;
        if (fuse) cls_w->push_back(g);
        else MMVAE_TRY(wgrad_async(P, g, s));
    } else {
    {
        GatherPlan pl = dense_plan(rows, 200, 200, D2);
        WgradParams g = wgrad_of(P, pl, &P.fc[2].gk, 1, rows);
        g.c.A = w.ay2; g.P = d_out; g.ldp = P.lde;
        MMVAE_TRY(wgrad_async(P, g, s));
        GatherPlan pd = dense_plan(rows, P.lde, P.lde, 200);
        GemmParams d = gemm_of(P, pd, &P.fc[2].pk_dgrad, 1, rows);
        d.c.A = d_out; d.out_bf = w.dy2; d.ldo = 200;
        d.d_r = w.y2; d.d_ld = 200; d.d_act = ACT_SWISH; if (dropout) { d.d_mask = m2; d.d_mask_scale = ms; }
        d.d_colsum = P.buf.grads + P.fc[1].b_off;
        MMVAE_TRY(launch_gemm_gather(d, s));
    }
    {
        GatherPlan pl = dense_plan(rows, 400, 400, 200);
        WgradParams g = wgrad_of(P, pl, &P.fc[1].gk, 1, rows);
        g.c.A = w.ay1; g.P = w.dy2; g.ldp = 200;
        MMVAE_TRY(wgrad_async(P, g, s));
        GatherPlan pd = dense_plan(rows, 200, 200, 400);
        GemmParams d = gemm_of(P, pd, &P.fc[1].pk_dgrad, 1, rows);
        d.c.A = w.dy2; d.out_bf = w.dy1; d.ldo = 400;
        d.d_r = w.y1; d.d_ld = 400; d.d_act = ACT_SWISH; if (dropout) { d.d_mask = m1; d.d_mask_scale = ms; }
        d.d_colsum = P.buf.grads + P.fc[0].b_off;
        MMVAE_TRY(launch_gemm_gather(d, s));
    }
    }
    if (tail_only) return MMVAE_OK;
    {
        GatherPlan pl = plan_fwdform(2, 2, 1, 1, 256, 2, 2, 1, 0, 400, 1, rows);
        WgradParams g = wgrad_of(P, pl, &P.fc[0].gk, 1, rows);
        g.c.A = w.a4; g.c.a_bcast_n = B;
        g.P = w.dy1; g.ldp = 400;
        if (P.mlp_tail && fuse) {
            MMPlan* pp = &P;
            cls_w->push_back(g);
            side_later(P, [pp, cls_w](hipStream_t ws_) {
                MMVAE_TRY(launch_wgrad_group(cls_w->data(), (int)cls_w->size(), ws_, &pp->slab));
                return pp->batch_reduce ? MMVAE_OK : launch_wgrad_reduce(&pp->slab, ws_, true);
            }, mmvae_knob("mm_cls_lane", 1));
        } else {
            MMVAE_TRY(wgrad_async(P, g, s));
        }
        GatherPlan pd{};
        pd.c.AH = 1; pd.c.AW = 1; pd.c.Ald = 400; pd.c.C = 400; pd.c.sy = pd.c.sx = 1; pd.c.dy = pd.c.dx = 1;
        pd.c.OH = 2; pd.c.OW = 2; pd.c.osy = pd.c.osx = 1; pd.c.N = 256; pd.c.nclasses = 4;
        for (int sidx = 0; sidx < 4; ++sidx) {
            GatherClass& k = pd.cls[sidx];
            k.OY = 1; k.OX = 1; k.TH = 1; k.TW = 1; k.offy = 0; k.offx = 0; k.ooy = sidx / 2; k.oox = sidx % 2;
            k.K = 400; k.Kpad = round_up(400, 64);
        }
        GemmParams d = gemm_of(P, pd, P.fc[0].pk_dgrad4, 1, rows);
        d.c.A = w.dy1; d.out_bf = w.db4; d.ldo = 256;
        d.d_r = w.r4; d.d_ld = 256; d.d_bcast_n = B; d.d_act = ACT_SWISH;
        d.d_affine = w.aff_e[2]; d.d_meanrstd = w.mr_e[2]; d.d_red = w.red_e[2];
        MMVAE_TRY(launch_gemm_gather(d, s));
    }
    bf16* r[4] = {w.r1, w.r2, w.r3, w.r4};
    bf16* a[4] = {w.a1, w.a2, w.a3, w.a4};
    bf16* dr[4] = {w.d1e, w.d2e, w.d3e, w.dr4};
    bf16* drr[4] = {nullptr, w.d2er, w.d3er, nullptr};
    for (int l = 3; l >= 1; --l) {
        const ConvL& L = P.conv[l];
        const BnL& b = P.bn[L.bn];
        const int pix = L.g.OH * L.g.OW;
        const bool fl = fuse && l < 3;
        BnBwdApplyArgs x{};
        x.db = (l == 3) ? w.db4 : dr[l];
        x.db2 = (l == 3 && variants == 2) ? w.db4 + (size_t)B * 1024 : nullptr;
        x.r = r[l]; x.dr = fl ? drr[l] : dr[l]; x.rows = B * pix; x.C = L.g.Cout; x.ld = L.g.Cout; x.rows_per_group = B * pix; x.G = 1;
        x.red = w.red_e[l - 1]; x.meanrstd = w.mr_e[l - 1]; x.gamma = P.buf.params + b.w_off;
        x.dgamma = P.buf.grads + b.w_off; x.dbeta = P.buf.grads + b.b_off;
        if (!fl) MMVAE_TRY(launch_bn_bwd_apply(x, s));
        WgradParams gw = wgrad_of(P, L.fwd, L.gk, 1, B);
        gw.c.A = a[l - 1]; gw.P = x.dr; gw.ldp = L.g.Cout;
        if (fuse) {
            MMPlan* pp = &P;
            {
                const bool byp = mmvae_knob("mm_stage_out", 1) != 0;
                const bool actp = l >= 2 && !byp;
                const bool bnb = fl && !(byp && l == 2);
                const int prows = B * P.conv[l >= 2 ? l - 1 : 1].g.OH * P.conv[l >= 2 ? l - 1 : 1].g.OW;
                const BnL bp = P.bn[P.conv[l >= 2 ? l - 1 : 1].bn];
                const bf16* rin = r[l >= 2 ? l - 1 : 1]; bf16* ao = a[l >= 2 ? l - 1 : 1]; const float2* st = w.st_e[l >= 2 ? l - 2 : 0];
                WgradParams g0 = wgrad_of(P, L.fwd, L.gk, 1, B);
                g0.c.A = a[l - 1]; g0.P = x.dr; g0.ldp = L.g.Cout;
                side_later(P, [pp, x, g0, bnb, actp, bp, rin, ao, st, prows](hipStream_t ws_) {
                    if (bnb) MMVAE_TRY(launch_bn_bwd_apply(x, ws_));
                    if (actp) MMVAE_TRY(bn_act_side(*pp, bp, rin, ao, prows, prows, 1, st, 1, ws_));
                    return wgrad_on(*pp, g0, ws_);
                }, l == 1 ? 1 : l == 2 ? mmvae_knob("mm_conv3_lane", 0) : mmvae_knob("mm_conv4_lane", 0));
            }
            if (fuse && l == 1) MMVAE_TRY(side_flush(P, s));
        }
        {
            GemmParams d = gemm_of(P, L.dgrad, L.pk_dgrad, 1, B, L.pk_dgrad_f);
            d.c.A = dr[l]; d.out_bf = dr[l - 1]; d.ldo = L.g.Cin;
            d.d_r = r[l - 1]; d.d_ld = L.g.Cin; d.d_act = ACT_SWISH;
            if (l > 1) { d.d_affine = w.aff_e[l - 2]; d.d_meanrstd = w.mr_e[l - 2]; d.d_red = w.red_e[l - 2]; }
            GatherTransform tr{};
            if (fl) {
                tr.kind = 2; tr.r = r[l]; tr.red = w.red_e[l - 1]; tr.mr = w.mr_e[l - 1]; tr.gamma = P.buf.params + b.w_off;
                tr.inv_cnt = 1.f / (float)(B * pix); tr.groups = 1;
                if (l == 2 && mmvae_knob("mm_stage_out", 1)) {
                    tr.out = drr[l]; tr.dgamma = P.buf.grads + b.w_off; tr.dbeta = P.buf.grads + b.b_off;
                }
                d.tr = &tr;
            }
            const bool flush = fuse && P.wgrad_forked && (mmvae_knob("mm_forks", 0) ? l == 2 : l >= 2);
            if (flush) arm_fork(P);
            MMVAE_TRY(launch_gemm_gather(d, s));
            if (flush) { MMVAE_TRY(commit_fork(P, s)); MMVAE_TRY(side_flush(P, s)); }
        }
        if (!fuse) MMVAE_TRY(wgrad_async(P, gw, s));
    }
    if (fuse && !P.wgrad_forked) MMVAE_TRY(side_flush(P, s));
    if (fuse && mmvae_knob("mm_conv1_mfma", 1) && P.step_image) {
        const PackDesc& gd = P.gk.d[P.conv[0].gk[0]];
        MMVAE_TRY(launch_conv1_wgrad_mfma(P.step_image, B, w.d1e, P.buf.gpk + gd.dst_off, gd.Kpad, s));
    } else {
        GatherPlan pl = dense_plan(B * 625, 16, 16, 32);
        WgradParams g = wgrad_of(P, pl, P.conv[0].gk, 1, B * 625);
        g.c.A = w.patches1; g.P = w.d1e; g.ldp = 32;
        MMVAE_TRY(launch_wgrad(g, s, nullptr));
    }
    return MMVAE_OK;
}

int fused_tail(MMPlan& P, int groups, int training, const ConvTLastFwdArgs* last, int last_groups, int fused_bwd_groups, hipStream_t s) {
    MMPlan::W& w = P.w;
    const int B = P.B;
    const ConvL& L = P.convT[2];
    const BnL& b = P.bn[L.bn];
    DecLastFusedArgs x{};
    x.r = w.q3; x.act = ACT_SWISH; x.w = P.buf.params + P.convT[3].w_off;
    x.G = last_groups > 0 ? last_groups : groups; x.B = B; x.IH = 25; x.IW = 25; x.Cin = 32;
    x.bwd_groups = std::min(fused_bwd_groups, x.G);
    BnFinalizeArgs& f = x.fin;
    f.stats = w.st_d[2]; f.G = groups; f.C = b.C; f.count = (float)(B * L.g.OH * L.g.OW);
    f.gamma = P.buf.params + b.w_off; f.beta = P.buf.params + b.b_off;
    f.running_mean = P.buf.bn_stats + b.stat_off; f.running_var = P.buf.bn_stats + b.stat_off + b.C;
    f.num_batches_tracked = P.buf.bn_nbt + b.idx;
    f.updates_per_group = 1; f.affine = w.aff_d[2]; f.meanrstd = w.mr_d[2]; f.eps = BN_EPS; f.momentum = BN_MOM; f.training = training;
    f.skip_update_mask = groups > 1 ? P.dec_skip_mask : 0u;
    x.target = last->target; x.logits = last->logits; x.recon = last->recon; x.dlogit = nullptr;
    for (int k = 0; k < 4; ++k) x.coef[k] = last->coef[k];
    x.loss_sum = last->loss_sum;
    if (last->loglik) { x.loglik = last->loglik; x.rows_per_target = last->rows_per_target; x.B = last->rows; }
    if (x.bwd_groups > 0) {
        const int chunks = x.bwd_groups * B * (dec_last_mfma_applies(x) ? 1 : dec_last_fused_strips(25));
        x.wslab = P.slab.take((size_t)chunks * 32 * 16);
        MMVAE_REQUIRE(x.wslab != nullptr, "fused decoder tail: the weight-gradient slab pool is exhausted");
        x.db = w.d3; x.red = w.red_d[2];
        WgradSlabJob j{};
        const PackDesc& gd = P.gk.d[P.convT[3].gk[0]];
        j.dst = P.buf.gpk + gd.dst_off; j.slab = x.wslab; j.N = 32; j.K = 16; j.Kpad = gd.Kpad; j.chunks = chunks;
        j.chunk_stride = 32 * 16; j.src_ld = 16; j.stream = s;
        P.slab.jobs.push_back(j);
    }
    return launch_dec_last_fused(x, s);
}

int dec_fwd(MMPlan& P, int groups, int training, ConvTLastFwdArgs* last, hipStream_t s, int last_groups = -1, int fused_bwd_groups = -1,
            bool fuse = false) {
    MMPlan::W& w = P.w;
    const int B = P.B, rows = groups * B;
    {
        GatherPlan pl = dense_plan(rows, P.ldz, P.ldz, 1024);
        GemmParams g = gemm_of(P, pl, &P.up.pk_fwd, 1, rows);
        g.c.A = w.z_bf; g.out_bf = w.u; g.ldo = 1024; g.out_act_bf = w.au; g.e_act = ACT_SWISH;
        MMVAE_TRY(launch_gemm_gather(g, s));
    }
    bf16* q[4] = {w.u, w.q1, w.q2, w.q3};
    bf16* aq[4] = {w.au, w.aq1, w.aq2, w.aq3};
    for (int l = 0; l < 3; ++l) {
        const ConvL& L = P.convT[l];
        {
            GemmParams g = gemm_of(P, L.fwd, L.pk_fwd, groups, B, L.pk_fwd_f);
            g.c.A = aq[l];
            g.out_bf = q[l + 1]; g.ldo = L.g.Cout;
            g.colstats = training ? w.st_d[l] : nullptr;
            GatherTransform tr{};
            if (fuse && l >= 1) {
                const ConvL& Lp = P.convT[l - 1];
                const int prpg = B * Lp.g.OH * Lp.g.OW;
                tr.kind = 1;
                tr.fin = bn_fin_args(P, P.bn[Lp.bn], prpg, groups, w.st_d[l - 1], 1, w.aff_d[l - 1], w.mr_d[l - 1], training);
                g.c.A = q[l]; g.tr = &tr;
                if (mmvae_knob("mm_stage_out", 1)) tr.out = aq[l];
            }
            MMVAE_TRY(launch_gemm_gather(g, s));
        }
        const int rpg = B * L.g.OH * L.g.OW;
        if (l == 2 && fused_bwd_groups >= 0) continue;
        if (fuse && l <= 1) continue;
        MMVAE_TRY(bn_act(P, P.bn[L.bn], q[l + 1], aq[l + 1], groups * rpg, rpg, groups, w.st_d[l], 1, w.aff_d[l], w.mr_d[l], training, s));
    }
    if (fused_bwd_groups >= 0) return fused_tail(P, groups, training, last, last_groups, fused_bwd_groups, s);
    ConvTLastFwdArgs x = *last;
    x.act = w.aq3; x.w = P.buf.params + P.convT[3].w_off; x.G = last_groups > 0 ? last_groups : groups; x.B = B; x.IH = 25; x.IW = 25; x.Cin = 32; x.Cout = 1;
    return launch_convt_last_fwd(x, s);
}

int dec_bwd(MMPlan& P, const float* dlogit, int groups, float* dz, hipStream_t s, bool last_fused = false, bool fuse = false,
            int fwd_groups = 0, int training = 1) {
    MMPlan::W& w = P.w;
    const int B = P.B, rows = groups * B;
    bf16* q[4] = {w.u, w.q1, w.q2, w.q3};
    bf16* aq[4] = {w.au, w.aq1, w.aq2, w.aq3};
    bf16* dq[4] = {w.du, w.d1, w.d2, w.d3};
    bf16* dqr[4] = {nullptr, w.d1r, w.d2r, w.d3r};
    if (last_fused) {
        if (P.wgrad_forked) {
            PlanBase* pb = &P;
            side_later(P, [pb, s](hipStream_t wst) {
                for (WgradSlabJob& j : pb->slab.jobs) if (j.stream == s && j.src_ld == 16) j.stream = wst;
                return launch_wgrad_reduce(&pb->slab, wst, true);
            });
        }
    } else {
        const ConvL& L = P.convT[3];
        MMVAE_TRY(launch_im2col_small(dlogit, rows, 1, IMG, IMG, 4, 4, 2, 1, 25, 25, w.patches4, 16, s));
        {
            GatherPlan pd = dense_plan(B * 625, 16, 16, 32);
            GemmParams d = gemm_of(P, pd, L.pk_dgrad, groups, B * 625);
            d.c.A = w.patches4; d.out_bf = w.d3; d.ldo = 32;
            d.d_r = w.q3; d.d_ld = 32; d.d_act = ACT_SWISH; d.d_affine = w.aff_d[2]; d.d_meanrstd = w.mr_d[2]; d.d_red = w.red_d[2];
            arm_fork(P);
            MMVAE_TRY(launch_gemm_gather(d, s));
            MMVAE_TRY(commit_fork(P, s));
        }
        GatherPlan pl = plan_fwdform(1, 1, 25, 25, 16, 1, 1, 1, 0, 32, groups, B);
        WgradParams g = wgrad_of(P, pl, L.gk, groups, B);
        g.c.A = w.patches4; g.c.AH = 25; g.c.AW = 25; g.c.sy = g.c.sx = 1;
        g.P = w.aq3; g.ldp = 32;
        MMVAE_TRY(wgrad_async(P, g, s));
    }
    for (int l = 2; l >= 0; --l) {
        const ConvL& L = P.convT[l];
        const BnL& b = P.bn[L.bn];
        const int pix = L.g.OH * L.g.OW;
        const bool fl = fuse;
        BnBwdApplyArgs x{};
        x.db = dq[l + 1]; x.r = q[l + 1]; x.dr = fl ? dqr[l + 1] : dq[l + 1]; x.rows = rows * pix; x.C = L.g.Cout; x.ld = L.g.Cout;
        x.rows_per_group = B * pix; x.G = groups;
        x.red = w.red_d[l]; x.meanrstd = w.mr_d[l]; x.gamma = P.buf.params + b.w_off;
        x.dgamma = P.buf.grads + b.w_off; x.dbeta = P.buf.grads + b.b_off;
        if (!fl) MMVAE_TRY(launch_bn_bwd_apply(x, s));
        WgradParams gw = convT_wgrad(P, L, groups, B, aq[l], x.dr);
        if (fl) {
            MMPlan* pp = &P;
            const ConvL& Lp = P.convT[l >= 1 ? l - 1 : 0];
            const int prpg = B * Lp.g.OH * Lp.g.OW;
            {
                const bool byp = mmvae_knob("mm_stage_out", 1) != 0;
                const bool actp = l >= 1 && !byp;
                const BnL bp = P.bn[Lp.bn];
                const bf16* qin = q[l]; bf16* aqo = aq[l]; const float2* st = w.st_d[l >= 1 ? l - 1 : 0];
                side_later(P, [pp, x, gw, byp, actp, bp, qin, aqo, st, groups, prpg, training](hipStream_t ws_) {
                    if (!byp) MMVAE_TRY(launch_bn_bwd_apply(x, ws_));
                    if (actp) MMVAE_TRY(bn_act_side(*pp, bp, qin, aqo, groups * prpg, prpg, groups, st, training, ws_));
                    return wgrad_on(*pp, gw, ws_);
                });
            }
        } else if (fuse || l == 0) {
            MMPlan* pp = &P;
            side_later(P, [pp, gw](hipStream_t ws_) { return wgrad_on(*pp, gw, ws_); });
        }
        {
            GemmParams d = gemm_of(P, L.dgrad, L.pk_dgrad, groups, B, L.pk_dgrad_f);
            d.c.A = dq[l + 1]; d.out_bf = dq[l]; d.ldo = L.g.Cin;
            d.d_r = q[l]; d.d_ld = L.g.Cin; d.d_act = ACT_SWISH;
            if (l > 0) { d.d_affine = w.aff_d[l - 1]; d.d_meanrstd = w.mr_d[l - 1]; d.d_red = w.red_d[l - 1]; }
            GatherTransform tr{};
            if (fl) {
                tr.kind = 2; tr.r = q[l + 1]; tr.red = w.red_d[l]; tr.mr = w.mr_d[l]; tr.gamma = P.buf.params + b.w_off;
                tr.inv_cnt = 1.f / (float)(B * pix); tr.groups = groups;
                if (mmvae_knob("mm_stage_out", 1)) { tr.out = dqr[l + 1]; tr.dgamma = P.buf.grads + b.w_off; tr.dbeta = P.buf.grads + b.b_off; }
                d.tr = &tr;
            }
            const bool flush = P.wgrad_forked && ((l == 2 && !mmvae_knob("mm_forks", 0)) || l == 0);
            if (flush) arm_fork(P);
            MMVAE_TRY(launch_gemm_gather(d, s));
            if (flush) { MMVAE_TRY(commit_fork(P, s)); if (l == 2) MMVAE_TRY(side_flush(P, s)); }
        }
        if (!fl && !(fuse || l == 0)) MMVAE_TRY(wgrad_async(P, gw, s));
    }
    {
        GatherPlan pl = dense_plan(rows, P.ldz, P.ldz, 1024);
        WgradParams g = wgrad_of(P, pl, &P.up.gk, 1, rows);
        g.c.A = w.z_bf; g.P = w.du; g.ldp = 1024;
        MMPlan* pp = &P;
        side_later(P, [pp, g](hipStream_t ws_) { return wgrad_on(*pp, g, ws_); });
        MMVAE_TRY(side_flush(P, s));
        GatherPlan pd = dense_plan(rows, 1024, 1024, P.D);
        GemmParams d = gemm_of(P, pd, &P.up.pk_dgrad, 1, rows);
        d.c.A = w.du; d.out_f = dz; d.ldo = P.D;
        MMVAE_TRY(launch_gemm_gather(d, s));
    }
    return MMVAE_OK;
}

TextEncArgs te_args(MMPlan& P, const long long* text, float* out, bool save) { return text_enc_args(P, text, out, save); }
int txt_enc_bwd(MMPlan& P, const long long* text, const float* d_out, hipStream_t s) { return text_enc_bwd(P, text, d_out, s); }
TextDecArgs td_args(MMPlan& P, const float* z, int groups, bool save) { return text_dec_args(P, z, groups, save); }
int txt_dec_bwd(MMPlan& P, const TextDecArgs& f, const float* dwords, float* dz, hipStream_t s) {
    const int R = f.R;
    const TextDecBwdArgs a = text_dec_bwd_args(P, f, dwords, dz);
    P.ev_dz = nullptr;
    const bool own_ev = P.in_step && s == P.st_text && mmvae_knob("mm_dz_event", 1) != 0;
    if (own_ev) {
        P.ev_dz = next_ev(P);
        if (!P.capturing && !mmvae_knob("no_stop_events", 0)) mmvae_arm_stop_event(P.ev_dz);
    }
    MMVAE_TRY(launch_text_decoder_bwd(a, s));
    if (own_ev && (mmvae_take_stop_event() != nullptr || P.capturing || mmvae_knob("no_stop_events", 0)) && hipEventRecord(P.ev_dz, s) != hipSuccess) {
        mmvae_set_error("text decoder event failed: %s", hipGetErrorString(hipGetLastError()));
        return MMVAE_EHIP;
    }
    MMVAE_TRY(text_dec_wgrads(P, R, s));
    P.ev_txtgrads = nullptr;
    if (own_ev) {
        P.ev_txtgrads = next_ev(P);
        if (hipEventRecord(P.ev_txtgrads, s) != hipSuccess) {
            mmvae_set_error("text decoder event failed: %s", hipGetErrorString(hipGetLastError()));
            return MMVAE_EHIP;
        }
    }
    return MMVAE_OK;
}

}

MMPlan* mm_create(int D, int B) {
    if (D < 1 || D > 127 || B < 1) { mmvae_set_error("mm_create: need 1 <= n_latents <= 127 and batch >= 1"); return nullptr; }
    MMPlan* P = new MMPlan();
    P->D = D; P->B = B;
    P->single_wgrad_stream = true;
    build_plan(*P);
    plan_size_workspaces(*P, carve);
    return P;
}
void mm_destroy(MMPlan* P) { delete P; }
int mm_early_ranges(const MMPlan* P, long long* ranges, int cap) {
    int n = 0;
    for (const ParamInfo& pi : P->params) {
        if (pi.name.rfind("image_decoder.", 0) != 0 && pi.name.rfind("text_decoder.", 0) != 0) continue;
        if (n > 0 && ranges[2 * (n - 1)] + ranges[2 * (n - 1) + 1] == pi.offset) { ranges[2 * (n - 1) + 1] += pi.numel; continue; }
        if (n == cap) return 0;
        ranges[2 * n] = pi.offset; ranges[2 * n + 1] = pi.numel; ++n;
    }
    for (int r = 0; r < n; ++r)
        if (ranges[2 * r] % 4 != 0 || ranges[2 * r + 1] % 4 != 0) return 0;
    return n;
}
PlanBase* mm_base(MMPlan* P) { return P; }

static int use_ws(MMPlan* P, void* ws, size_t bytes, bool module = true) { return plan_use_ws(P, ws, bytes, module, carve); }

static int mm_step_body(MMPlan* Pp, const mmvae_mm_step_io& io, int training, int do_backward, hipStream_t s);
int mm_step_fwd_bwd(MMPlan* Pp, const mmvae_mm_step_io& io, int training, int do_backward, hipStream_t s) {
    if (const mmvae_early_adam* e = io.early_adam) {
        MMVAE_REQUIRE(e->m && e->v && e->state && e->gmap && e->ran, "mmvae_mm_step: early_adam with a null field");
        *e->ran = 0;
    }
    return plan_step(Pp, io, training, do_backward, s, mm_step_body);
}
static int mm_step_body(MMPlan* Pp, const mmvae_mm_step_io& io, int training, int do_backward, hipStream_t s) {
    MMVAE_TRY(use_ws(Pp, io.ws, io.ws_bytes, false));
    MMPlan& P = *Pp;
    MMPlan::W& w = P.w;
    const int B = P.B, D = P.D, B3 = 3 * B;
    MMVAE_REQUIRE(io.image && io.text && io.sums, "step: image/text/sums must be given");
    const float* eps = io.eps;
    const uint8_t *m1 = io.enc_mask1, *m2 = io.enc_mask2, *gk = io.gru_keep;
    const bool serial0 = mmvae_serial();
    const bool staged = mmvae_knob("mm_stage_begin", 1) != 0 && !serial0;
    StepBeginArgs sb{}, sb2{};
    sb.zero_ptr[0] = w.zero_begin; sb.zero_bytes[0] = w.zero_bytes;
    StepBeginArgs& sz = staged ? sb2 : sb;
    if (do_backward) {
        sz.zero_ptr[1] = P.buf.gpk; sz.zero_bytes[1] = (size_t)P.gk.mat_elems * sizeof(float);
        sz.zero_ptr[2] = P.buf.grads; sz.zero_bytes[2] = (size_t)(P.nparams / 4) * 16;
        const int skipz = mmvae_knob("dbg_begin_skip_zero", 0);
        if (skipz & 1) sz.zero_ptr[1] = nullptr;
        if (skipz & 2) sz.zero_ptr[2] = nullptr;
    }
    sb.p = DROP_P; sb.seed = io.seed; sb.step = io.step_counter;
    if (training && !eps) { sb.eps = w.eps; sb.n_eps = (long long)B3 * D; eps = w.eps; }
    if (training && io.enc_dropout && !m1) { sb.mask[0] = w.m1; sb.n_mask[0] = (long long)2 * B * 400; m1 = w.m1; }
    if (training && io.enc_dropout && !m2) { sb.mask[1] = w.m2; sb.n_mask[1] = (long long)2 * B * 200; m2 = w.m2; }
    if (training && io.gru_dropout && !gk) { sb.mask[2] = w.gkeep; sb.n_mask[2] = (long long)4 * B3 * P.H; gk = w.gkeep; }
    const int skipb = mmvae_knob("dbg_begin_skip", 0);
    if (skipb & 2) { sb.eps = nullptr; sb.mask[0] = sb.mask[1] = sb.mask[2] = nullptr; }
    if (skipb & 4) sb.zero_ptr[0] = nullptr;
    const bool pack_now = io.pack_first && !(skipb & 1);
    if (pack_now) {
        MMVAE_TRY(step_begin_with_pack(sb, P.buf.desc_dev, P.pk.d.data(), (int)P.pk.d.size(), P.buf.params, P.buf.packed, P.buf.packed_vec));
        if (staged) sb.pack_parts = 1u << 0;
    }
    MMVAE_TRY(ensure_streams(P));
    P.in_step = true;
    {
        hipStreamCaptureStatus cs = hipStreamCaptureStatusNone;
        P.capturing = hipStreamIsCapturing(s, &cs) == hipSuccess && cs == hipStreamCaptureStatusActive;
    }
    arm_fork(P);
    MMVAE_TRY(launch_step_begin(sb, s));
    MMVAE_TRY(commit_fork(P, s));
    if (do_backward && P.nparams % 4 != 0)
        MMVAE_TRY(launch_fill_zero(P.buf.grads + (P.nparams / 4) * 4, (size_t)(P.nparams % 4) * sizeof(float), s));
    const int enc_drop = training && io.enc_dropout;
    const int sk[3] = {io.pass_skip[0] != 0, io.pass_skip[1] != 0, io.pass_skip[2] != 0};
    P.dec_skip_mask = (unsigned)(sk[0] | (sk[1] << 1) | (sk[2] << 2));
    const int enc_updates = 2 - sk[0] - sk[1];
    const bool serial = mmvae_serial();
    hipStream_t T = serial ? s : P.st_text;
    if (T != s) MMVAE_TRY(fork_to(P, T));
    if (staged && pack_now) {
        StepBeginArgs st1{};
        MMVAE_TRY(step_begin_with_pack(st1, P.buf.desc_dev, P.pk.d.data(), (int)P.pk.d.size(), P.buf.params, P.buf.packed, P.buf.packed_vec));
        st1.pack_parts = 1u << 1;
        MMVAE_TRY(launch_step_begin(st1, T));
    }
    {
        TextEncArgs a = te_args(P, io.text, w.txtout, do_backward);
        MMVAE_TRY(launch_text_encoder_fwd(a, T));
    }
    if (staged && (pack_now || sb2.zero_ptr[1] || sb2.zero_ptr[2])) {
        if (pack_now) {
            MMVAE_TRY(step_begin_with_pack(sb2, P.buf.desc_dev, P.pk.d.data(), (int)P.pk.d.size(), P.buf.params, P.buf.packed, P.buf.packed_vec));
            sb2.pack_parts = 1u << 2;
        }
        MMVAE_TRY(launch_step_begin(sb2, T));
    }
    P.step_image = io.image;
    const bool fuse = mmvae_knob("mm_fuse_bn", 1) != 0 && mmvae_knob("convres", 1) != 0 && B % 8 == 0;
    MMVAE_TRY(enc_fwd(P, io.image, 2, m1, m2, enc_drop, training, enc_updates, w.encout, s, fuse));
    MMVAE_TRY(edge(P, T, s));
    Latent3Args la{};
    la.B = B; la.D = D; la.img_out = w.encout; la.txt_out = w.txtout; la.eps = eps;
    la.mu = io.mu ? io.mu : w.mu; la.logvar = io.logvar ? io.logvar : w.logvar;
    la.z_f32 = w.z_f32; la.z_bf = w.z_bf; la.ldz = P.ldz; la.kl_sum = w.sums + 8; la.training = training;
    arm_fork(P);
    MMVAE_TRY(launch_latent3_fwd(la, s));
    MMVAE_TRY(commit_fork(P, s));
    if (T != s) MMVAE_TRY(fork_to(P, T));
    TextDecArgs td = td_args(P, w.z_f32, 3, do_backward);
    td.keep = (training && io.gru_dropout) ? gk : nullptr; td.keep_scale = 1.f / (1.f - DROP_P);
    td.force_tokens = io.force_tokens;
    if (io.recon_text) td.words = io.recon_text;
    if (io.tokens) td.tokens_out = io.tokens;
    td.target = io.text; td.nll_sum = w.sums + 4; td.dwords = do_backward ? w.dwords : nullptr;
    for (int k = 0; k < 3; ++k) td.nll_coef[k] = sk[k] ? 0.f : io.lambda_yx[k] / (float)(B * TXT_T);
    if (const int half = mmvae_knob("dbg_text_rows_div", 0)) td.R = max(16, td.R / half);
    MMVAE_TRY(launch_text_decoder_fwd(td, T));
    if (do_backward) MMVAE_TRY(txt_dec_bwd(P, td, w.dwords, w.dz_txt, T));
    ConvTLastFwdArgs last{};
    last.target = io.image; last.recon = io.recon_image; last.dlogit = do_backward ? w.dlogit : nullptr; last.loss_sum = w.sums;
    for (int k = 0; k < 3; ++k) last.coef[k] = sk[k] ? 0.f : io.lambda_xy[k] / (float)(B * NPIX);
    int last_groups = 3;
    if (!io.recon_image)
        while (last_groups > 1 && last.coef[last_groups - 1] == 0.f) --last_groups;
    int img_groups = 3;
    while (img_groups > 0 && (io.lambda_xy[img_groups - 1] == 0.f || sk[img_groups - 1])) --img_groups;
    const bool fuse_tail = P.slab.pool != nullptr;
    MMVAE_TRY(dec_fwd(P, 3, training, &last, s, last_groups, fuse_tail ? (do_backward ? std::min(img_groups, last_groups) : 0) : -1, fuse));
    if (!do_backward) {
        MMVAE_TRY(edge(P, T, s));
        P.in_step = false;
        hipLaunchKernelGGL(sum_slots_kernel, dim3(1), dim3(64), 0, s, w.sums, io.sums);
        return mmvae_check_launch("sum_slots");
    }

    P.wgrad_forked = mmvae_knob("mm_wgrad_inline", 0) == 0;
    int rc = MMVAE_OK;
    P.deferred.clear();
    P.defer_wgrad = false;
    if (img_groups > 0) rc = dec_bwd(P, w.dlogit, img_groups, w.dz_img, s, fuse_tail, fuse, 3, training);
    if (io.early_adam && rc == MMVAE_OK && img_groups > 0 && fuse && fuse_tail && P.wgrad_forked && !serial && T != s && !io.dp_split &&
        io.defer_unpack && P.ev_txtgrads && P.side_pending.empty() && P.st_wgrad2 == P.st_wgrad && mmvae_knob("mm_early_adam", 1)) {
        hipStream_t Wst = P.st_wgrad;
        AdamArgs ad{};
        const mmvae_early_adam& ea = *io.early_adam;
        ad.p = P.buf.params; ad.g = P.buf.grads; ad.m = ea.m; ad.v = ea.v; ad.n = P.nparams; ad.step = ea.state;
        ad.lr = ea.lr; ad.b1 = ea.beta1; ad.b2 = ea.beta2; ad.eps = ea.eps; ad.grad_scale = ea.grad_scale;
        ad.gmap = ea.gmap; ad.gpk = P.buf.gpk; ad.gpk_vec = P.buf.gpk_vec; ad.g_out = P.buf.grads;
        long long rg[8];
        ad.nr = mm_early_ranges(&P, rg, 4);
        for (int r = 0; r < ad.nr; ++r) { ad.roff[r] = rg[2 * r]; ad.rlen[r] = rg[2 * r + 1]; }
        ad.no_advance = 1;
        if (ad.nr > 0) {
            if (hipStreamWaitEvent(Wst, P.ev_txtgrads, 0) != hipSuccess) { mmvae_set_error("early optimizer part: %s", hipGetErrorString(hipGetLastError())); rc = MMVAE_EHIP; }
            if (rc == MMVAE_OK) rc = launch_adam(ad, Wst);
            if (rc == MMVAE_OK) *ea.ran = 1;
        }
    }
    if (rc == MMVAE_OK) {
        const int k = mmvae_knob("dbg_skip_edges", 0);
        if (P.ev_dz && T != s) {
            if (k != 1 && k != 3 && hipStreamWaitEvent(s, P.ev_dz, 0) != hipSuccess) {
                mmvae_set_error("stream join failed: %s", hipGetErrorString(hipGetLastError()));
                rc = MMVAE_EHIP;
            }
        } else {
            rc = edge(P, T, s);
        }
    }
    const bool dp_split = io.dp_split && !io.defer_unpack;
    if (dp_split && rc == MMVAE_OK) {
        rc = edge(P, s, T);
        if (rc == MMVAE_OK && P.st_wgrad != T) rc = edge(P, P.st_wgrad, T);
        if (rc == MMVAE_OK && P.st_wgrad2 != P.st_wgrad && P.st_wgrad2 != T) rc = edge(P, P.st_wgrad2, T);
        if (rc == MMVAE_OK) rc = launch_wgrad_reduce(&P.slab, T);
        if (rc == MMVAE_OK)
            rc = plan_unpack(P, T, false, 1);
        if (rc == MMVAE_OK) {
            if (!P.ev_early) hipEventCreateWithFlags(&P.ev_early, hipEventDisableTiming);
            if (hipEventRecord(P.ev_early, T) != hipSuccess) { mmvae_set_error("early-gradient event failed"); rc = MMVAE_EHIP; }
        }
    }
    Latent3BwdArgs lb{};
    lb.f = la; lb.dz_a = w.dz_img; lb.dz_b = w.dz_txt;
    for (int k = 0; k < 3; ++k) lb.kl_coef[k] = sk[k] ? 0.f : io.kl_lambda / (float)B;
    lb.d_img_out_bf = w.d_encout; lb.ld_img_out_bf = P.lde; lb.d_img_bias = P.buf.grads + P.fc[2].b_off; lb.d_txt_out = w.d_txtout;
    lb.loss_slots = w.sums; lb.loss_out = io.sums;
    if (rc == MMVAE_OK) {
        arm_fork(P);
        rc = launch_latent3_bwd(lb, s);
        if (rc == MMVAE_OK) rc = commit_fork(P, s);
    }
    if (rc == MMVAE_OK) rc = flush_wgrads(P, s);
    if (rc == MMVAE_OK && T != s) rc = fork_to(P, T);
    if (rc == MMVAE_OK) rc = txt_enc_bwd(P, io.text, w.d_txtout, T);
    if (rc == MMVAE_OK) rc = enc_bwd(P, w.d_encout, 2, m1, m2, enc_drop, s, fuse);
    P.wgrad_forked = false;
    P.in_step = false;
    MMVAE_TRY(rc);
    MMVAE_TRY(join_sides(P, T, s));
    MMVAE_TRY(launch_wgrad_reduce(&P.slab, s));
    if (dp_split) return plan_unpack(P, s, false, 0);
    if (!io.defer_unpack) MMVAE_TRY(plan_unpack(P, s, true));
    return MMVAE_OK;
}
int mm_wait_early_grads(MMPlan* P, hipStream_t s) {
    MMVAE_REQUIRE(P && P->ev_early, "mm_wait_early_grads: no dp_split step has run on this plan");
    if (hipStreamWaitEvent(s, P->ev_early, 0) != hipSuccess) {
        mmvae_set_error("mm_wait_early_grads: %s", hipGetErrorString(hipGetLastError()));
        return MMVAE_EHIP;
    }
    return MMVAE_OK;
}

static int mm_image_waist_default(int D) { return D == 20 ? 1 : 0; }
struct ImageMiddle {
    bool waist; int training, enc_drop;
    const float* eps; const uint8_t *m1, *m2; float *mu, *logvar;
    const float* dz; float kl_coef; float* loss_out;
};
static Latent1Args image_latent_args(MMPlan& P, const ImageMiddle& m) {
    MMPlan::W& w = P.w;
    Latent1Args la{};
    la.B = P.B; la.D = P.D; la.enc_out = w.encout; la.eps = m.eps; la.mu = m.mu; la.logvar = m.logvar;
    la.z_f32 = w.z_f32; la.z_bf = w.z_bf; la.ldz = P.ldz; la.kl_sum = w.sums + 8; la.training = m.training;
    la.scratch = w.tmp_f32;
    return la;
}
static int image_middle_fwd(MMPlan& P, const ImageMiddle& m, const float* image, hipStream_t s, bool tail_only = false) {
    MMPlan::W& w = P.w;
    if (m.waist) {
        Mlp2Latent1FwdArgs wf{};
        wf.D = P.D; wf.ldz = P.ldz; wf.training = m.training; wf.eps = m.eps; wf.mu = m.mu; wf.logvar = m.logvar;
        wf.z_f32 = w.z_f32; wf.z_bf = w.z_bf; wf.scratch = reinterpret_cast<double*>(w.tmp_f32);
        return enc_fwd(P, image, 1, m.m1, m.m2, m.enc_drop, m.training, 1, w.encout, s, false, &wf, tail_only);
    }
    MMVAE_TRY(enc_fwd(P, image, 1, m.m1, m.m2, m.enc_drop, m.training, 1, w.encout, s, false, nullptr, tail_only));
    return launch_latent1_fwd(image_latent_args(P, m), s);
}
static int image_middle_bwd(MMPlan& P, const ImageMiddle& m, hipStream_t s, bool tail_only = false) {
    MMPlan::W& w = P.w;
    if (m.waist) {
        Mlp2Latent1BwdArgs wb{};
        wb.D = P.D; wb.training = m.training; wb.mu = m.mu; wb.logvar = m.logvar; wb.eps = m.eps; wb.dz = m.dz;
        wb.kl_coef = m.kl_coef; wb.scratch = reinterpret_cast<double*>(w.tmp_f32);
        return enc_bwd(P, w.d_encout, 1, m.m1, m.m2, m.enc_drop, s, false, &wb, m.loss_out, tail_only);
    }
    Latent1BwdArgs lb{};
    lb.f = image_latent_args(P, m); lb.dz = m.dz; lb.kl_coef = m.kl_coef;
    lb.d_enc_out = w.d_encout; lb.ld = P.lde; lb.d_bias = P.buf.grads + P.fc[2].b_off;
    lb.loss_slots = w.sums; lb.loss_out = m.loss_out;
    MMVAE_TRY(launch_latent1_bwd(lb, s));
    return enc_bwd(P, w.d_encout, 1, m.m1, m.m2, m.enc_drop, s, false, nullptr, nullptr, tail_only);
}
static int mm_image_step_body(MMPlan* Pp, const mmvae_image_step_io& io, int training, int do_backward, hipStream_t s) {
    MMVAE_TRY(use_ws(Pp, io.ws, io.ws_bytes));
    MMPlan& P = *Pp;
    MMPlan::W& w = P.w;
    const int B = P.B, D = P.D;
    MMVAE_REQUIRE(io.image && io.sums, "image step: image/sums must be given");
    const int wk = mmvae_knob("mm_image_waist", -1);
    ImageMiddle m{};
    m.waist = P.waist && (wk < 0 ? mm_image_waist_default(D) : wk) != 0;
    MMVAE_REQUIRE(launch_latent1_scratch_floats(B, D) <= (size_t)B * NPIX && 2 * mlp2_latent1_scratch_doubles(B, D) <= (size_t)B * NPIX,
                  "image step: no room for the latent block's partial sums");
    m.training = training; m.enc_drop = training && io.enc_dropout;
    m.eps = io.eps; m.m1 = io.enc_mask1; m.m2 = io.enc_mask2;
    StepBeginArgs sb{};
    sb.zero_ptr[0] = w.zero_begin; sb.zero_bytes[0] = w.zero_bytes;
    if (do_backward) {
        sb.zero_ptr[1] = P.buf.gpk; sb.zero_bytes[1] = (size_t)P.gk.mat_elems * sizeof(float);
        sb.zero_ptr[2] = P.buf.grads; sb.zero_bytes[2] = (size_t)(P.nparams / 4) * 16;
    }
    sb.p = DROP_P; sb.seed = io.seed; sb.step = io.step_counter;
    if (training && !m.eps) { sb.eps = w.eps; sb.n_eps = (long long)B * D; m.eps = w.eps; }
    if (m.enc_drop && !m.m1) { sb.mask[0] = w.m1; sb.n_mask[0] = (long long)B * 400; m.m1 = w.m1; }
    if (m.enc_drop && !m.m2) { sb.mask[1] = w.m2; sb.n_mask[1] = (long long)B * 200; m.m2 = w.m2; }
    MMVAE_TRY(launch_step_begin(sb, s));
    if (do_backward && P.nparams % 4 != 0)
        MMVAE_TRY(launch_fill_zero(P.buf.grads + (P.nparams / 4) * 4, (size_t)(P.nparams % 4) * sizeof(float), s));
    MMVAE_TRY(ensure_streams(P));
    P.in_step = true;
    {
        hipStreamCaptureStatus cs = hipStreamCaptureStatusNone;
        P.capturing = hipStreamIsCapturing(s, &cs) == hipSuccess && cs == hipStreamCaptureStatusActive;
    }
    m.mu = io.mu ? io.mu : w.mu;
    m.logvar = io.logvar ? io.logvar : w.logvar;
    MMVAE_TRY(image_middle_fwd(P, m, io.image, s));
    ConvTLastFwdArgs last{};
    last.target = io.image; last.recon = io.recon_image; last.dlogit = do_backward ? w.dlogit : nullptr; last.loss_sum = w.sums;
    last.coef[0] = io.lambda_x / (float)(B * NPIX);
    MMVAE_TRY(dec_fwd(P, 1, training, &last, s));
    if (!do_backward) {
        P.in_step = false;
        if (m.waist)
            return launch_mlp2_latent1_finish(reinterpret_cast<double*>(w.tmp_f32), B, D, nullptr, w.sums, io.sums, s);
        hipLaunchKernelGGL(sum_slots_kernel, dim3(1), dim3(64), 0, s, w.sums, io.sums);
        return mmvae_check_launch("sum_slots");
    }
    P.wgrad_forked = true;
    P.deferred.clear();
    P.defer_wgrad = false;
    int rc = MMVAE_OK;
    const bool img_term = io.lambda_x != 0.f;
    if (img_term) rc = dec_bwd(P, w.dlogit, 1, w.dz_img, s);
    m.dz = img_term ? w.dz_img : nullptr; m.kl_coef = io.kl_lambda / (float)B; m.loss_out = io.sums;
    if (rc == MMVAE_OK) rc = image_middle_bwd(P, m, s);
    P.wgrad_forked = false;
    P.in_step = false;
    MMVAE_TRY(rc);
    MMVAE_TRY(join_sides(P, s, s));
    if (io.defer_unpack) return launch_wgrad_reduce(&P.slab, s);
    return plan_unpack(P, s, true);
}
static int mm_image_middle_replay(MMPlan* Pp, void* ws, size_t wsb, const std::string& what, hipStream_t s) {
    MMVAE_REQUIRE(what == "waist_fwd" || what == "chain_fwd" || what == "waist_bwd" || what == "chain_bwd", "bench_layer: unknown layer 'image_step:%s'", what.c_str());
    MMVAE_TRY(use_ws(Pp, ws, wsb));
    MMPlan& P = *Pp;
    MMPlan::W& w = P.w;
    ImageMiddle m{};
    m.waist = what.compare(0, 5, "waist") == 0;
    MMVAE_REQUIRE(!m.waist || P.waist, "bench_layer: no waist is compiled for n_latents = %d", P.D);
    m.training = 1; m.enc_drop = 1; m.eps = w.eps; m.m1 = w.m1; m.m2 = w.m2; m.mu = w.mu; m.logvar = w.logvar;
    m.dz = w.dz_img; m.kl_coef = 1e-3f / (float)P.B; m.loss_out = w.tmp_f32 + (size_t)P.B * NPIX - 16;
    if (what.compare(6, 3, "fwd") == 0) return image_middle_fwd(P, m, nullptr, s, true);
    MMVAE_TRY(image_middle_bwd(P, m, s, true));
    return launch_wgrad_reduce(&P.slab, s);
}
size_t mm_image_step_workspace_bytes(const MMPlan* P) { return P->ws_bytes_module; }
int mm_image_step(MMPlan* P, const mmvae_image_step_io& io, int training, int do_backward, hipStream_t s) {
    return plan_step(P, io, training, do_backward, s, mm_image_step_body);
}

int mm_image_encoder_fwd(MMPlan* P, void* ws, size_t wsb, const float* image, const uint8_t* m1, const uint8_t* m2,
                         int training, float* out, hipStream_t s) {
    MMVAE_TRY(use_ws(P, ws, wsb));
    MMPlan::W& w = P->w;
    MMVAE_TRY(launch_fill_zero(w.zero_begin, w.zero_bytes, s));
    return enc_fwd(*P, image, 1, m1, m2, training && m1 != nullptr, training, 1, out, s);
}
static __global__ void cast_rows_pad_kernel(const float* x, int rows, int cols, bf16* out, int ld) {
    int i = blockIdx.x * blockDim.x + threadIdx.x;
    if (i >= rows * ld) return;
    int r = i / ld, c = i - r * ld;
    out[i] = (bf16)(c < cols ? x[(size_t)r * cols + c] : 0.0f);
}
int mm_image_encoder_bwd(MMPlan* P, void* ws, size_t wsb, const float* d_out, const uint8_t* m1, const uint8_t* m2, hipStream_t s) {
    MMVAE_TRY(use_ws(P, ws, wsb));
    MMPlan::W& w = P->w;
    const int rows = P->B, D2 = 2 * P->D;
    MMVAE_TRY(plan_zero_gpk(*P, s));
    hipLaunchKernelGGL(cast_rows_pad_kernel, dim3(ceil_div(rows * P->lde, 256)), dim3(256), 0, s, d_out, rows, D2, w.d_encout, P->lde);
    hipLaunchKernelGGL(colsum_kernel, dim3(ceil_div(D2, 64)), dim3(64), 0, s, d_out, rows, D2, P->buf.grads + P->fc[2].b_off);
    MMVAE_TRY(mmvae_check_launch("image encoder bwd prologue"));
    MMVAE_TRY(enc_bwd(*P, w.d_encout, 1, m1, m2, m1 != nullptr, s));
    return plan_unpack(*P, s, true);
}
int mm_image_decoder_fwd(MMPlan* P, void* ws, size_t wsb, const float* z, int training, float* recon, hipStream_t s) {
    MMVAE_TRY(use_ws(P, ws, wsb));
    MMPlan::W& w = P->w;
    const int rows = P->B;
    MMVAE_TRY(launch_fill_zero(w.zero_begin, w.zero_bytes, s));
    hipLaunchKernelGGL(cast_z_kernel, dim3(ceil_div(rows * P->ldz, 256)), dim3(256), 0, s, z, rows, P->D, w.z_bf, P->ldz);
    MMVAE_TRY(mmvae_check_launch("cast_z"));
    ConvTLastFwdArgs last{};
    last.recon = recon;
    return dec_fwd(*P, 1, training, &last, s);
}
int mm_image_decoder_bwd(MMPlan* P, void* ws, size_t wsb, const float* d_recon, const float* recon, float* dz, hipStream_t s) {
    MMVAE_TRY(use_ws(P, ws, wsb));
    MMPlan::W& w = P->w;
    const int rows = P->B;
    MMVAE_TRY(plan_zero_gpk(*P, s));
    hipLaunchKernelGGL(sigmoid_bwd_kernel, dim3(ceil_div(rows * NPIX, 256)), dim3(256), 0, s, d_recon, recon, (long long)rows * NPIX, w.dlogit);
    MMVAE_TRY(mmvae_check_launch("sigmoid_bwd"));
    MMVAE_TRY(dec_bwd(*P, w.dlogit, 1, dz, s));
    return plan_unpack(*P, s, true);
}
int mm_text_encoder_fwd(MMPlan* P, void* ws, size_t wsb, const long long* text, float* out, hipStream_t s) {
    MMVAE_TRY(use_ws(P, ws, wsb));
    TextEncArgs a = te_args(*P, text, out, true);
    return launch_text_encoder_fwd(a, s);
}
int mm_text_encoder_bwd(MMPlan* P, void* ws, size_t wsb, const long long* text, const float* d_out, hipStream_t s) {
    MMVAE_TRY(use_ws(P, ws, wsb));
    MMVAE_TRY(plan_zero_gpk(*P, s));
    MMVAE_TRY(txt_enc_bwd(*P, text, d_out, s));
    return plan_unpack(*P, s, true);
}
int mm_text_decoder_fwd(MMPlan* P, void* ws, size_t wsb, const float* z, int training, const uint8_t* keep,
                        const long long* force_tokens, float* words, long long* tokens, hipStream_t s) {
    MMVAE_TRY(use_ws(P, ws, wsb));
    TextDecArgs a = td_args(*P, z, 1, true);
    a.keep = training ? keep : nullptr; a.keep_scale = 1.f / (1.f - DROP_P);
    a.force_tokens = force_tokens; a.words = words; a.tokens_out = tokens;
    return launch_text_decoder_fwd(a, s);
}
int mm_text_decoder_bwd(MMPlan* P, void* ws, size_t wsb, const float* z, const uint8_t* keep, const long long* force_tokens,
                        const float* words, const long long* tokens, const float* d_words, float* dz, hipStream_t s) {
    MMVAE_TRY(use_ws(P, ws, wsb));
    MMVAE_TRY(plan_zero_gpk(*P, s));
    TextDecArgs a = td_args(*P, z, 1, true);
    a.keep = keep; a.keep_scale = 1.f / (1.f - DROP_P);
    a.force_tokens = force_tokens; a.words = const_cast<float*>(words); a.tokens_out = const_cast<long long*>(tokens);
    MMVAE_TRY(txt_dec_bwd(*P, a, d_words, dz, s));
    return plan_unpack(*P, s, true);
}

static int iw_image_rows(MMPlan* P, void* ws, size_t wsb, const float* z, const float* image, int B, int K, float* loglik_x, hipStream_t s,
                         const char* who) {
    MMVAE_REQUIRE(B >= 1 && K >= 1 && (long long)B * K <= P->B, "%s: %d examples x %d particles exceed the plan's %d rows", who, B, K, P->B);
    MMVAE_TRY(use_ws(P, ws, wsb));
    MMPlan::W& w = P->w;
    const int rows = B * K;
    MMVAE_TRY(launch_fill_zero(w.zero_begin, w.zero_bytes, s));
    hipLaunchKernelGGL(cast_z_kernel, dim3(ceil_div(rows * P->ldz, 256)), dim3(256), 0, s, z, rows, P->D, w.z_bf, P->ldz);
    MMVAE_TRY(mmvae_check_launch("cast_z"));
    ConvTLastFwdArgs last{};
    last.target = image; last.loglik = loglik_x; last.rows_per_target = K; last.rows = rows;
    return dec_fwd(*P, 1, 0, &last, s, -1, 0);
}
int mm_iw_score(MMPlan* P, void* ws, size_t wsb, const float* z, const float* image, int B, int K, float* loglik_x, float* words,
                hipStream_t s) {
    MMVAE_REQUIRE(P && z && image && loglik_x && words, "mmvae_mm_iw_score: null argument");
    MMVAE_TRY(iw_image_rows(P, ws, wsb, z, image, B, K, loglik_x, s, "mmvae_mm_iw_score"));
    TextDecArgs a = td_args(*P, z, 1, false);
    a.R = B * K; a.words = words;
    return launch_text_decoder_fwd(a, s);
}
int mm_iw_score_image(MMPlan* P, void* ws, size_t wsb, const float* z, const float* image, int B, int K, float* loglik_x, hipStream_t s) {
    MMVAE_REQUIRE(P && z && image && loglik_x, "mmvae_mm_iw_score_image: null argument");
    return iw_image_rows(P, ws, wsb, z, image, B, K, loglik_x, s, "mmvae_mm_iw_score_image");
}

static bool layer_gemm(MMPlan& P, const std::string& name, GemmParams& g) {
    MMPlan::W& w = P.w;
    const int B = P.B;
    bf16* r[4] = {w.r1, w.r2, w.r3, w.r4};
    bf16* a[4] = {w.a1, w.a2, w.a3, w.a4};
    bf16* dre[4] = {w.d1e, w.d2e, w.d3e, w.dr4};
    bf16* q[4] = {w.u, w.q1, w.q2, w.q3};
    bf16* aq[4] = {w.au, w.aq1, w.aq2, w.aq3};
    bf16* dq[4] = {w.du, w.d1, w.d2, w.d3};
    if (name == "enc_conv1") {
        GatherPlan pl = dense_plan(B * 625, 16, 16, 32);
        g = gemm_of(P, pl, P.conv[0].pk_fwd, 1, B * 625);
        g.c.A = w.patches1; g.out_bf = w.r1; g.ldo = 32; g.out_act_bf = w.a1; g.e_act = ACT_SWISH;
        return true;
    }
    for (int l = 1; l < 4; ++l) {
        const ConvL& L = P.conv[l];
        if (name == "enc_conv" + std::to_string(l + 1)) {
            g = gemm_of(P, L.fwd, L.pk_fwd, 1, B, L.pk_fwd_f);
            g.c.A = a[l - 1];
            g.out_bf = r[l]; g.ldo = L.g.Cout; g.colstats = w.st_e[l - 1];
            return true;
        }
        if (name == "enc_conv" + std::to_string(l + 1) + "_dgrad") {
            g = gemm_of(P, L.dgrad, L.pk_dgrad, 1, B, L.pk_dgrad_f);
            g.c.A = dre[l]; g.out_bf = dre[l - 1]; g.ldo = L.g.Cin;
            g.d_r = r[l - 1]; g.d_ld = L.g.Cin; g.d_act = ACT_SWISH;
            if (l > 1) { g.d_affine = w.aff_e[l - 2]; g.d_meanrstd = w.mr_e[l - 2]; g.d_red = w.red_e[l - 2]; }
            return true;
        }
    }
    {
        const int rows = 2 * B;
        const float ms = 1.f / (1.f - DROP_P);
        if (name == "enc_fc1") {
            GatherPlan pl = plan_fwdform(2, 2, 1, 1, 256, 2, 2, 1, 0, 400, 1, rows);
            g = gemm_of(P, pl, &P.fc[0].pk_fwd, 1, rows);
            g.c.A = w.a4; g.c.a_bcast_n = B; g.bias = P.buf.params + P.fc[0].b_off; g.out_bf = w.y1; g.ldo = 400;
            g.out_act_bf = w.ay1; g.e_act = ACT_SWISH; g.e_mask = w.m1; g.e_mask_scale = ms;
            return true;
        }
        if (name == "enc_fc2") {
            GatherPlan pl = dense_plan(rows, 400, 400, 200);
            g = gemm_of(P, pl, &P.fc[1].pk_fwd, 1, rows);
            g.c.A = w.ay1; g.bias = P.buf.params + P.fc[1].b_off; g.out_bf = w.y2; g.ldo = 200;
            g.out_act_bf = w.ay2; g.e_act = ACT_SWISH; g.e_mask = w.m2; g.e_mask_scale = ms;
            return true;
        }
        if (name == "enc_fc3") {
            GatherPlan pl = dense_plan(rows, 200, 200, 2 * P.D);
            g = gemm_of(P, pl, &P.fc[2].pk_fwd, 1, rows);
            g.c.A = w.ay2; g.bias = P.buf.params + P.fc[2].b_off; g.out_f = w.tmp_f32; g.ldo = 2 * P.D;
            return true;
        }
        if (name == "enc_fc3_dgrad") {
            GatherPlan pd = dense_plan(rows, P.lde, P.lde, 200);
            g = gemm_of(P, pd, &P.fc[2].pk_dgrad, 1, rows);
            g.c.A = w.d_encout; g.out_bf = w.dy2; g.ldo = 200;
            g.d_r = w.y2; g.d_ld = 200; g.d_act = ACT_SWISH; g.d_mask = w.m2; g.d_mask_scale = ms;
            g.d_colsum = w.tmp_f32;
            return true;
        }
        if (name == "enc_fc2_dgrad") {
            GatherPlan pd = dense_plan(rows, 200, 200, 400);
            g = gemm_of(P, pd, &P.fc[1].pk_dgrad, 1, rows);
            g.c.A = w.dy2; g.out_bf = w.dy1; g.ldo = 400;
            g.d_r = w.y1; g.d_ld = 400; g.d_act = ACT_SWISH; g.d_mask = w.m1; g.d_mask_scale = ms;
            g.d_colsum = w.tmp_f32;
            return true;
        }
        if (name == "dec_up") {
            GatherPlan pl = dense_plan(3 * B, P.ldz, P.ldz, 1024);
            g = gemm_of(P, pl, &P.up.pk_fwd, 1, 3 * B);
            g.c.A = w.z_bf; g.out_bf = w.u; g.ldo = 1024; g.out_act_bf = w.au; g.e_act = ACT_SWISH;
            return true;
        }
        if (name == "dec_up_dgrad") {
            GatherPlan pd = dense_plan(rows, 1024, 1024, P.D);
            g = gemm_of(P, pd, &P.up.pk_dgrad, 1, rows);
            g.c.A = w.du; g.out_f = w.tmp_f32; g.ldo = P.D;
            return true;
        }
    }
    if (name == "dec_last_dgrad_gemm") {
        const ConvL& L = P.convT[3];
        GatherPlan pl = dense_plan(B * 625, 16, 16, 32);
        g = gemm_of(P, pl, L.pk_dgrad, 2, B * 625);
        g.c.A = w.patches4; g.out_bf = w.d3; g.ldo = 32;
        g.d_r = w.q3; g.d_ld = 32; g.d_act = ACT_SWISH; g.d_affine = w.aff_d[2]; g.d_meanrstd = w.mr_d[2]; g.d_red = w.red_d[2];
        return true;
    }
    for (int l = 0; l < 3; ++l) {
        const ConvL& L = P.convT[l];
        if (name == "dec_convT" + std::to_string(l + 1)) {
            g = gemm_of(P, L.fwd, L.pk_fwd, 3, B, L.pk_fwd_f);
            g.c.A = aq[l];
            g.out_bf = q[l + 1]; g.ldo = L.g.Cout; g.colstats = w.st_d[l];
            return true;
        }
        if (name == "dec_convT" + std::to_string(l + 1) + "_dgrad") {
            g = gemm_of(P, L.dgrad, L.pk_dgrad, 2, B, L.pk_dgrad_f);
            g.c.A = dq[l + 1]; g.out_bf = dq[l]; g.ldo = L.g.Cin;
            g.d_r = q[l]; g.d_ld = L.g.Cin; g.d_act = ACT_SWISH;
            if (l > 0) { g.d_affine = w.aff_d[l - 1]; g.d_meanrstd = w.mr_d[l - 1]; g.d_red = w.red_d[l - 1]; }
            return true;
        }
    }
    return false;
}
static bool layer_wgrad(MMPlan& P, const std::string& name, WgradParams& g) {
    MMPlan::W& w = P.w;
    const int B = P.B;
    bf16* a[4] = {w.a1, w.a2, w.a3, w.a4};
    bf16* dre[4] = {w.d1e, w.d2e, w.d3e, w.dr4};
    bf16* aq[4] = {w.au, w.aq1, w.aq2, w.aq3};
    bf16* dq[4] = {w.du, w.d1, w.d2, w.d3};
    for (int l = 0; l < 3; ++l)
        if (name == "dec_convT" + std::to_string(l + 1) + "_wgrad") {
            const ConvL& L = P.convT[l];
            g = convT_wgrad(P, L, 2, B, aq[l], dq[l + 1]);
            return true;
        }
    for (int l = 1; l < 4; ++l)
        if (name == "enc_conv" + std::to_string(l + 1) + "_wgrad") {
            const ConvL& L = P.conv[l];
            g = wgrad_of(P, L.fwd, L.gk, 1, B);
            g.c.A = a[l - 1]; g.P = dre[l]; g.ldp = L.g.Cout;
            return true;
        }
    if (name == "dec_last_wgrad") {
        GatherPlan pl = plan_fwdform(1, 1, 25, 25, 16, 1, 1, 1, 0, 32, 2, B);
        g = wgrad_of(P, pl, P.convT[3].gk, 2, B);
        g.c.A = w.patches4; g.c.AH = 25; g.c.AW = 25; g.c.sy = g.c.sx = 1;
        g.P = w.aq3; g.ldp = 32;
        return true;
    }
    if (name == "enc_conv1_wgrad") {
        GatherPlan pl = dense_plan(B * 625, 16, 16, 32);
        g = wgrad_of(P, pl, P.conv[0].gk, 1, B * 625);
        g.c.A = w.patches1; g.P = w.d1e; g.ldp = 32;
        return true;
    }
    return false;
}
static double wgrad_flops(const WgradParams& g) {
    double f = 0;
    for (int i = 0; i < g.c.nclasses; ++i) f += 2.0 * g.c.groups * g.cls[i].rows_per_group * (double)g.c.N * g.cls[i].K;
    return f;
}
static double gemm_flops(const GemmParams& g) {
    double f = 0;
    for (int i = 0; i < g.c.nclasses; ++i) f += 2.0 * g.c.groups * g.cls[i].rows_per_group * (double)g.c.N * g.cls[i].K;
    return f;
}
int mm_bench_layer(MMPlan* P, void* ws, size_t wsb, const char* layer, int iters, hipStream_t s) {
    if (std::strncmp(layer, "image_step:", 11) == 0) {
        for (int i = 0; i < iters; ++i) MMVAE_TRY(mm_image_middle_replay(P, ws, wsb, layer + 11, s));
        return MMVAE_OK;
    }
    MMVAE_TRY(use_ws(P, ws, wsb, false));
    if (std::string(layer) == "dec_last_fused") {
        ConvTLastFwdArgs last{};
        last.target = (const float*)P->w.tmp_f32; last.loss_sum = P->w.sums;
        last.coef[0] = last.coef[1] = 1.f / (float)(P->B * NPIX);
        for (int i = 0; i < iters; ++i) {
            P->slab.reset(P->w.slab, P->w.slab_floats);
            MMVAE_TRY(fused_tail(*P, 3, 1, &last, 2, 2, s));
            P->slab.jobs.clear(); P->slab.ring_jobs.clear();
        }
        return MMVAE_OK;
    }
    WgradParams wg{};
    if (layer_wgrad(*P, layer, wg)) {
        for (int i = 0; i < iters; ++i) {
            P->slab.reset(P->w.slab, P->w.slab_floats);
            MMVAE_TRY(launch_wgrad(wg, s, &P->slab));
            MMVAE_TRY(launch_wgrad_reduce(&P->slab, s));
        }
        return MMVAE_OK;
    }
    GemmParams g{};
    MMVAE_REQUIRE(layer_gemm(*P, layer, g), "bench_layer: unknown layer '%s'", layer);
    for (int i = 0; i < iters; ++i) MMVAE_TRY(launch_gemm_gather(g, s));
    return MMVAE_OK;
}
double mm_layer_flops(const MMPlan* Pc, const char* layer) {
    MMPlan& P = *const_cast<MMPlan*>(Pc);
    GemmParams g{};
    WgradParams wg{};
    if (std::string(layer) == "dec_last_fused") return 3.0 * 2.0 * 2 * P.B * 625 * 16 * 32;
    if (P.bound && layer_wgrad(P, layer, wg)) return wgrad_flops(wg);
    if (!P.bound || !layer_gemm(P, layer, g)) return -1.0;
    return gemm_flops(g);
}
double mm_layer_algo_flops(const MMPlan* Pc, const char* layer) {
    const MMPlan& P = *Pc;
    const std::string name = layer;
    const int B = P.B;
    auto conv = [&](const ConvL& L, int images) {
        const ConvGeom& g = L.g;
        const double pix = g.transposed ? (double)g.IH * g.IW : (double)g.OH * g.OW;
        return 2.0 * pix * g.KH * g.KW * g.Cin * g.Cout * images;
    };
    for (int l = 0; l < 4; ++l) {
        const std::string e = "enc_conv" + std::to_string(l + 1), d = "dec_convT" + std::to_string(l + 1);
        if (name == e || name == e + "_dgrad" || name == e + "_wgrad") return conv(P.conv[l], B);
        if (name == d) return conv(P.convT[l], 3 * B);
        if (name == d + "_dgrad" || name == d + "_wgrad") return conv(P.convT[l], 2 * B);
    }
    if (name == "dec_last_wgrad" || name == "dec_last_dgrad_gemm") return conv(P.convT[3], 2 * B);
    return mm_layer_flops(Pc, layer);
}
double mm_layer_algo_bytes(const MMPlan* Pc, const char* layer) {
    const MMPlan& P = *Pc;
    const std::string name = layer;
    const int B = P.B;
    auto conv = [&](const ConvL& L, int images, bool wgrad) {
        const ConvGeom& g = L.g;
        const double act = (double)images * ((double)g.IH * g.IW * g.Cin + (double)g.OH * g.OW * g.Cout) * 2.0;
        return act + (double)g.Cin * g.Cout * g.KH * g.KW * (wgrad ? 4.0 : 2.0);
    };
    for (int l = 0; l < 4; ++l) {
        const std::string e = "enc_conv" + std::to_string(l + 1), d = "dec_convT" + std::to_string(l + 1);
        if (name == e || name == e + "_dgrad") return conv(P.conv[l], B, false);
        if (name == e + "_wgrad") return conv(P.conv[l], B, true);
        if (name == d) return conv(P.convT[l], 3 * B, false);
        if (name == d + "_dgrad") return conv(P.convT[l], 2 * B, false);
        if (name == d + "_wgrad") return conv(P.convT[l], 2 * B, true);
    }
    return 0.0;
}
long long mm_debug_offset(MMPlan* P, const char* name) {
    Workspace ws((void*)0x1000, (size_t)1 << 40);
    const bool one_pass = std::strncmp(name, "image_step:", 11) == 0;
    if (one_pass) name += 11;
    P->carve_passes = one_pass ? 1 : 3;
    carve(*P, ws);
    P->carve_passes = 3;
    MMPlan::W& w = P->w;
    std::map<std::string, const void*> m = {
        {"patches1", w.patches1}, {"r1", w.r1}, {"r2", w.r2}, {"r3", w.r3}, {"r4", w.r4}, {"y1", w.y1}, {"y2", w.y2},
        {"encout", w.encout}, {"txtout", w.txtout}, {"z_bf", w.z_bf}, {"z_f32", w.z_f32}, {"u", w.u}, {"q1", w.q1}, {"q2", w.q2},
        {"q3", w.q3}, {"logits", w.logits}, {"dlogit", w.dlogit}, {"d3", w.d3}, {"d2", w.d2}, {"d1", w.d1}, {"du", w.du},
        {"dz_img", w.dz_img}, {"dz_txt", w.dz_txt}, {"d_encout", w.d_encout}, {"d_txtout", w.d_txtout}, {"dy2", w.dy2},
        {"dy1", w.dy1}, {"db4", w.db4}, {"dr4", w.dr4}, {"d3e", w.d3e}, {"d2e", w.d2e}, {"d1e", w.d1e},
        {"aff_d0", w.aff_d[0]}, {"aff_d1", w.aff_d[1]}, {"aff_d2", w.aff_d[2]}, {"st_d0", w.st_d[0]}, {"patches4", w.patches4},
        {"tmp_f32", w.tmp_f32}, {"aff_e0", w.aff_e[0]}, {"aff_e1", w.aff_e[1]}, {"aff_e2", w.aff_e[2]},
        {"eps", w.eps}, {"m1", w.m1}, {"m2", w.m2}, {"gkeep", w.gkeep},
        {"st_e0", w.st_e[0]}, {"st_e1", w.st_e[1]}, {"st_e2", w.st_e[2]}, {"st_d1", w.st_d[1]}, {"st_d2", w.st_d[2]},
        {"red_e0", w.red_e[0]}, {"red_e1", w.red_e[1]}, {"red_e2", w.red_e[2]},
        {"red_d0", w.red_d[0]}, {"red_d1", w.red_d[1]}, {"red_d2", w.red_d[2]},
        {"a1", w.a1}, {"a2", w.a2}, {"a3", w.a3}, {"aq1", w.aq1}, {"aq2", w.aq2}, {"aq3", w.aq3},
        {"a4", w.a4}, {"au", w.au}, {"ay1", w.ay1}, {"ay2", w.ay2}, {"slab", w.slab},
        {"mr_e0", w.mr_e[0]}, {"mr_e1", w.mr_e[1]}, {"mr_e2", w.mr_e[2]}, {"mr_d0", w.mr_d[0]}, {"mr_d1", w.mr_d[1]}, {"mr_d2", w.mr_d[2]},
        {"mu", w.mu}, {"logvar", w.logvar}, {"recon", w.recon}, {"sums", w.sums},
    };
    auto it = m.find(name);
    if (it == m.end()) return -1;
    return (long long)((const char*)it->second - (const char*)0x1000);
}
```

multimodal-vae_amd/csrc/thin.h:

```cpp
#pragma once
#include "common.h"
#include "elementwise.h"

struct ConvTLastFwdArgs {
    const bf16* act;
    const float* w;
    int G, B, IH, IW, Cin, Cout;
    const float* target;
    float* logits;
    float* recon;
    float* dlogit;
    float coef[4];
    float* loss_sum;
    float* loglik = nullptr; int rows_per_target = 1; int rows = 0;
};
int launch_convt_last_fwd(const ConvTLastFwdArgs& a, hipStream_t s);

struct ConvTLastDgradArgs {
    const float* dlogit;
    const float* w;
    int G, B, IH, IW, Cin, Cout;
    const bf16* r;
    const float2* affine;
    const float2* meanrstd;
    int act;
    bf16* db;
    float2* red;
};
int launch_convt_last_dgrad(const ConvTLastDgradArgs& a, hipStream_t s);

struct DecLastFusedArgs {
    const bf16* r;
    BnFinalizeArgs fin;
    int act;
    const float* w;
    int G, B, IH, IW, Cin;
    int dbg = 0;
    int Cout = 1;
    int bwd_groups;
    const float* target;
    float* logits; float* recon; float* dlogit;
    float coef[4];
    float* loss_sum;
    bf16* db;
    float2* red;
    float* wslab;
    float* loglik = nullptr;
    int rows_per_target = 1;
};
int dec_last_fused_strips(int IH);
bool dec_last_mfma_applies(const DecLastFusedArgs& a);
int launch_dec_last_mfma(const DecLastFusedArgs& a, hipStream_t s);
int launch_dec_last_fused(const DecLastFusedArgs& a, hipStream_t s);
bool dec_last_ca_applies(const DecLastFusedArgs& a);
int launch_dec_last_ca(const DecLastFusedArgs& a, hipStream_t s);

int launch_conv1_fwd_mfma(const float* image, int B, const bf16* Wp, int Kpad, bf16* r1, bf16* a1, hipStream_t s);
int launch_conv1_wgrad_mfma(const float* image, int B, const bf16* d1, float* dWp, int Kpad, hipStream_t s);
```

Measured before the change: 1751 ELBO-steps/s.

## Split conv1 forward and last decoder layer into row halves per image

The conv1 forward kernel and the fused last-decoder kernel now launch two workgroups per image, each owning half the output rows and staging only its rows plus halo into LDS. This doubles grid parallelism and shrinks LDS per workgroup so two workgroups fit per CU, aiming to raise occupancy on a thin per-image layer. The cost is redundant halo loads, extra patch staging, and for the decoder a partial weight-gradient reduction across halves. A shared geometry header checks the partition with static asserts.

```diff
diff --git a/multimodal-vae_amd/csrc/conv1.hip b/multimodal-vae_amd/csrc/conv1.hip
--- a/multimodal-vae_amd/csrc/conv1.hip
+++ b/multimodal-vae_amd/csrc/conv1.hip
@@ -1,5 +1,6 @@
 #include "thin.h"
 #include "convres_epi.h"
+#include "thin_split_geo.h"
 
 namespace {
 
@@ -7,6 +8,8 @@
 constexpr int C1_HW = 52;
 constexpr int C1_PP = 48;
 constexpr int C1_AP = 80;
+static_assert(c1s::IMG == C1_IMG && c1s::OH == C1_OH && c1s::NPIX == C1_NPIX && c1s::C == C1_C && c1s::HALVES * c1s::TILES == C1_TILES &&
+              c1s::PP == C1_PP, "thin_split_geo.h describes this layer");
 
 typedef __attribute__((address_space(3))) s16x4 lds_s16x4e;
 __device__ __forceinline__ bf16x8 tr_pair_e(const char* a0, const char* a1) {
@@ -41,43 +44,6 @@
         *reinterpret_cast<bf16x8*>(pat_s + px * C1_PP + 16) = hi;
     }
     __syncthreads();
-}
-
-struct Conv1FwdArgs { const float* image; int B; const bf16* Wp; int Kpad; bf16* r1; bf16* a1; };
-
-constexpr int C1F_WAVES = 4, C1F_NTHR = C1F_WAVES * 64;
-constexpr int C1F_OFF_IMG = 0, C1F_OFF_PAT = C1F_OFF_IMG + ((C1_HW * C1_HW * 2 + 15) / 16) * 16, C1F_OFF_SCR = C1F_OFF_PAT + C1_ROWS * C1_PP,
-              C1F_LDS = C1F_OFF_SCR + C1F_WAVES * 2560;
-
-__global__ __launch_bounds__(C1F_NTHR) void conv1_fwd_mfma_kernel(const Conv1FwdArgs a) {
-    extern __shared__ __attribute__((aligned(16))) char smem[];
-    const int tid = threadIdx.x, lane = tid & 63;
-    const int wave = __builtin_amdgcn_readfirstlane(tid >> 6);
-    const int r = lane & 31, h = lane >> 5;
-    const int n = blockIdx.x;
-    c1_patches<C1F_NTHR>(a.image + (size_t)n * (C1_IMG * C1_IMG), reinterpret_cast<bf16*>(smem + C1F_OFF_IMG), smem + C1F_OFF_PAT, tid);
-    const bf16x8 wb = *reinterpret_cast<const bf16x8*>(a.Wp + (size_t)r * a.Kpad + 8 * h);
-    const size_t bytes = (size_t)a.B * C1_NPIX * C1_C * 2;
-    const __amdgpu_buffer_rsrc_t rsrc_r = __builtin_amdgcn_make_buffer_rsrc(a.r1, 0, (int)bytes, 0x00020000);
-    const __amdgpu_buffer_rsrc_t rsrc_a = __builtin_amdgcn_make_buffer_rsrc(a.a1, 0, (int)bytes, 0x00020000);
-    char* const scr = smem + C1F_OFF_SCR + wave * 2560;
-    float s1 = 0.f, s2 = 0.f;
-    for (int t = wave; t < C1_TILES; t += C1F_WAVES) {
-        f32x16 acc;
-#pragma unroll
-        for (int j = 0; j < 16; ++j) acc[j] = 0.f;
-        const bf16x8 pa = *reinterpret_cast<const bf16x8*>(smem + C1F_OFF_PAT + (t * 32 + r) * C1_PP + h * 16);
-        acc = __builtin_amdgcn_mfma_f32_32x32x16_bf16(pa, wb, acc, 0, 0, 0);
-        const unsigned base = (unsigned)(((size_t)n * C1_NPIX + t * 32) * (C1_C * 2)) + (unsigned)((lane >> 4) * 16);
-        const int p0 = t * 32 + (lane & 15), p1 = p0 + 16;
-        const unsigned off0 = p0 < C1_NPIX ? base + (unsigned)((lane & 15) * (C1_C * 2)) : 0x40000000u;
-        const unsigned off1 = p1 < C1_NPIX ? base + (unsigned)((16 + (lane & 15)) * (C1_C * 2)) : 0x40000000u;
-        f32x16 act;
-#pragma unroll
-        for (int j = 0; j < 16; ++j) act[j] = swish_fast(acc[j]);
-        cr_epilogue_tile<0, false>(acc, scr, lane, 32, off0, off1, rsrc_r, rsrc_r, 1.f, 0.f, 0.f, 0.f, s1, s2, true);
-        cr_epilogue_tile<0, false>(act, scr, lane, 32, off0, off1, rsrc_a, rsrc_a, 1.f, 0.f, 0.f, 0.f, s1, s2, true);
-    }
 }
 
 struct Conv1WgradArgs { const float* image; int B; const bf16* d1; float* dWp; int Kpad; };
@@ -130,13 +96,101 @@
     }
 }
 
+struct Conv1FwdArgs { const float* image; int B; const bf16* Wp; int Kpad; bf16* r1; bf16* a1; };
+
+template <int NTHR>
+struct C1sImage {
+    static constexpr int IT = (c1s::LD_VEC + NTHR - 1) / NTHR;
+    float2 v[IT];
+    __device__ __forceinline__ void fetch(const float* img, int z, int tid, bool vec) {
+        const float* src = img + c1s::ld_row0(z) * c1s::IMG;
+#pragma unroll
+        for (int it = 0; it < IT; ++it) {
+            const int i = tid + it * NTHR;
+            v[it] = float2{0.f, 0.f};
+            if (i < c1s::LD_VEC) {
+                if (vec) v[it] = *reinterpret_cast<const float2*>(src + 2 * i);
+                else v[it] = float2{src[2 * i], src[2 * i + 1]};
+            }
+        }
+    }
+    __device__ __forceinline__ void stage(bf16* img_s, char* pat_s, int z, int tid) {
+#pragma unroll
+        for (int it = 0; it < IT; ++it) {
+            const int i = tid + it * NTHR;
+            if (i < c1s::LD_VEC) {
+                const int lr = i / (c1s::IMG / 2), c = i - lr * (c1s::IMG / 2);
+                bf16x2 o;
+                o[0] = (bf16)v[it].x; o[1] = (bf16)v[it].y;
+                *reinterpret_cast<bf16x2*>(img_s + c1s::cell(z, c1s::ld_row0(z) + lr, 2 * c)) = o;
+            }
+        }
+        {
+            unsigned* w = reinterpret_cast<unsigned*>(img_s);
+            if (tid < c1s::IROWS) { w[tid * (c1s::IW / 2)] = 0u; w[tid * (c1s::IW / 2) + c1s::IW / 2 - 1] = 0u; }
+            if (tid >= 32 && tid < 32 + c1s::IW / 2) w[c1s::pad_row(z) * (c1s::IW / 2) + tid - 32] = 0u;
+        }
+        __syncthreads();
+        const int np = c1s::npix(z);
+        for (int i = tid; i < 2 * c1s::PIX; i += NTHR) {
+            const int lp = i >> 1, half = i & 1;
+            bf16x8 o;
+            if (lp < np) {
+                const bf16* d0 = img_s + c1s::window(z, lp, half);
+#pragma unroll
+                for (int kw = 0; kw < 4; ++kw) { o[kw] = d0[kw]; o[4 + kw] = d0[c1s::IW + kw]; }
+            } else {
+#pragma unroll
+                for (int j = 0; j < 8; ++j) o[j] = (bf16)0.f;
+            }
+            *reinterpret_cast<bf16x8*>(pat_s + lp * c1s::PP + half * 16) = o;
+        }
+        __syncthreads();
+    }
+};
+
+__global__ __launch_bounds__(c1s::F_NTHR) void conv1_fwd_half_kernel(const Conv1FwdArgs a, const bool vec) {
+    extern __shared__ __attribute__((aligned(16))) char smem[];
+    const int tid = threadIdx.x, lane = tid & 63;
+    const int wave = __builtin_amdgcn_readfirstlane(tid >> 6);
+    const int r = lane & 31, h = lane >> 5;
+    const int n = blockIdx.x, z = blockIdx.y;
+    C1sImage<c1s::F_NTHR> im;
+    im.fetch(a.image + (size_t)n * (C1_IMG * C1_IMG), z, tid, vec);
+    const bf16x8 wb = *reinterpret_cast<const bf16x8*>(a.Wp + (size_t)r * a.Kpad + 8 * h);
+    im.stage(reinterpret_cast<bf16*>(smem + c1s::F_OFF_IMG), smem + c1s::F_OFF_PAT, z, tid);
+    const size_t bytes = (size_t)a.B * C1_NPIX * C1_C * 2;
+    const __amdgpu_buffer_rsrc_t rsrc_r = __builtin_amdgcn_make_buffer_rsrc(a.r1, 0, (int)bytes, 0x00020000);
+    const __amdgpu_buffer_rsrc_t rsrc_a = __builtin_amdgcn_make_buffer_rsrc(a.a1, 0, (int)bytes, 0x00020000);
+    char* const scr = smem + c1s::F_OFF_SCR + wave * 2560;
+    float s1 = 0.f, s2 = 0.f;
+    for (int tl = wave; tl < c1s::TILES; tl += c1s::F_WAVES) {
+        const int t = z * c1s::TILES + tl;
+        f32x16 acc;
+#pragma unroll
+        for (int j = 0; j < 16; ++j) acc[j] = 0.f;
+        const bf16x8 pa = *reinterpret_cast<const bf16x8*>(smem + c1s::F_OFF_PAT + (tl * 32 + r) * c1s::PP + h * 16);
+        acc = __builtin_amdgcn_mfma_f32_32x32x16_bf16(pa, wb, acc, 0, 0, 0);
+        const unsigned base = (unsigned)(((size_t)n * C1_NPIX + t * 32) * (C1_C * 2)) + (unsigned)((lane >> 4) * 16);
+        const int p0 = t * 32 + (lane & 15), p1 = p0 + 16;
+        const unsigned off0 = p0 < C1_NPIX ? base + (unsigned)((lane & 15) * (C1_C * 2)) : 0x40000000u;
+        const unsigned off1 = p1 < C1_NPIX ? base + (unsigned)((16 + (lane & 15)) * (C1_C * 2)) : 0x40000000u;
+        f32x16 act;
+#pragma unroll
+        for (int j = 0; j < 16; ++j) act[j] = swish_fast(acc[j]);
+        cr_epilogue_tile<0, false>(acc, scr, lane, 32, off0, off1, rsrc_r, rsrc_r, 1.f, 0.f, 0.f, 0.f, s1, s2, true);
+        cr_epilogue_tile<0, false>(act, scr, lane, 32, off0, off1, rsrc_a, rsrc_a, 1.f, 0.f, 0.f, 0.f, s1, s2, true);
+    }
+}
+
 }
 
 int launch_conv1_fwd_mfma(const float* image, int B, const bf16* Wp, int Kpad, bf16* r1, bf16* a1, hipStream_t s) {
     MMVAE_REQUIRE(image && Wp && r1 && a1 && Kpad >= 16 && (size_t)B * C1_NPIX * C1_C * 2 < 0x40000000ull, "conv1 fwd: arguments");
     Conv1FwdArgs a{image, B, Wp, Kpad, r1, a1};
-    MMVAE_LAUNCH(conv1_fwd_mfma_kernel, dim3(B), dim3(C1F_NTHR), C1F_LDS, s, a);
-    return mmvae_check_launch("conv1_fwd_mfma");
+    const bool vec = reinterpret_cast<uintptr_t>(image) % 8 == 0;
+    MMVAE_LAUNCH(conv1_fwd_half_kernel, dim3(B, c1s::HALVES), dim3(c1s::F_NTHR), c1s::F_LDS, s, a, vec);
+    return mmvae_check_launch("conv1_fwd_half");
 }
 int launch_conv1_wgrad_mfma(const float* image, int B, const bf16* d1, float* dWp, int Kpad, hipStream_t s) {
     MMVAE_REQUIRE(image && d1 && dWp && Kpad >= 16, "conv1 wgrad: arguments");
diff --git a/multimodal-vae_amd/csrc/convres_epi.h b/multimodal-vae_amd/csrc/convres_epi.h
--- a/multimodal-vae_amd/csrc/convres_epi.h
+++ b/multimodal-vae_amd/csrc/convres_epi.h
@@ -16,17 +16,15 @@
 typedef __attribute__((address_space(3))) s16x4 lds_s16x4c;
 
 template <int MODE, bool PARTIAL>
-__device__ __forceinline__ void cr_epilogue_tile(const f32x16& acc, char* scr, int lane, int rows_valid, unsigned off0, unsigned off1,
-                                                 __amdgpu_buffer_rsrc_t orsrc, __amdgpu_buffer_rsrc_t rrsrc, float dsc, float dsh,
-                                                 float dmean, float drstd, float& s1, float& s2, bool store) {
+__device__ __forceinline__ void cr_epilogue_tile_r(const f32x16& acc, char* scr, int lane, int rows_valid, unsigned off0, unsigned off1,
+                                                   __amdgpu_buffer_rsrc_t orsrc, const i32x4c r0, const i32x4c r1, float dsc, float dsh,
+                                                   float dmean, float drstd, float& s1, float& s2, bool store) {
     constexpr int SP = 80;
     const int r = lane & 31, h = lane >> 5, g = lane >> 4, i = lane & 15, q = i >> 2, p = i & 3;
     float v[16];
 #pragma unroll
     for (int j = 0; j < 16; ++j) v[j] = acc[j];
     if constexpr (MODE == 1) {
-        const i32x4c r0 = __builtin_bit_cast(i32x4c, __builtin_amdgcn_raw_buffer_load_b128(rrsrc, (int)off0, 0, 0));
-        const i32x4c r1 = __builtin_bit_cast(i32x4c, __builtin_amdgcn_raw_buffer_load_b128(rrsrc, (int)off1, 0, 0));
         *reinterpret_cast<i32x4c*>(scr + i * SP + g * 16) = r0;
         *reinterpret_cast<i32x4c*>(scr + (16 + i) * SP + g * 16) = r1;
         asm volatile("" ::: "memory");
@@ -92,5 +90,16 @@
     }
     asm volatile("" ::: "memory");
 }
+template <int MODE, bool PARTIAL>
+__device__ __forceinline__ void cr_epilogue_tile(const f32x16& acc, char* scr, int lane, int rows_valid, unsigned off0, unsigned off1,
+                                                 __amdgpu_buffer_rsrc_t orsrc, __amdgpu_buffer_rsrc_t rrsrc, float dsc, float dsh,
+                                                 float dmean, float drstd, float& s1, float& s2, bool store) {
+    i32x4c r0 = {0, 0, 0, 0}, r1 = {0, 0, 0, 0};
+    if constexpr (MODE == 1) {
+        r0 = __builtin_bit_cast(i32x4c, __builtin_amdgcn_raw_buffer_load_b128(rrsrc, (int)off0, 0, 0));
+        r1 = __builtin_bit_cast(i32x4c, __builtin_amdgcn_raw_buffer_load_b128(rrsrc, (int)off1, 0, 0));
+    }
+    cr_epilogue_tile_r<MODE, PARTIAL>(acc, scr, lane, rows_valid, off0, off1, orsrc, r0, r1, dsc, dsh, dmean, drstd, s1, s2, store);
+}
 
 }
diff --git a/multimodal-vae_amd/csrc/dec_last.hip b/multimodal-vae_amd/csrc/dec_last.hip
--- a/multimodal-vae_amd/csrc/dec_last.hip
+++ b/multimodal-vae_amd/csrc/dec_last.hip
@@ -1,6 +1,7 @@
 #include "thin.h"
 #include "bn_dev.h"
 #include "convres_epi.h"
+#include "thin_split_geo.h"
 
 namespace {
 
@@ -26,14 +27,10 @@
     return u.v;
 }
 
-template <bool IW>
 __global__ __launch_bounds__(DL_NTHR) void dec_last_mfma_kernel(const DecLastFusedArgs a) {
     extern __shared__ __attribute__((aligned(16))) char smem[];
     char* const A_s = smem + DL_OFF_A;
     float* const P_s = reinterpret_cast<float*>(smem + DL_OFF_P);
-    char* const pat_s = smem + DL_OFF_P;
-    float* const dl_s = reinterpret_cast<float*>(smem + DL_OFF_DL);
-    char* const scr_s = smem + DL_OFF_SCR;
     float2* const aff_s = reinterpret_cast<float2*>(smem + DL_OFF_TAB);
     float2* const mr_s = aff_s + DL_C;
     __shared__ float part[DL_WAVES];
@@ -44,7 +41,6 @@
     const int n_in_g = blockIdx.x, g = blockIdx.y;
     const long long n = (long long)g * a.B + n_in_g;
     const BnFinalizeArgs& f = a.fin;
-    const bool bwd = g < a.bwd_groups;
 
     constexpr int NV = DL_NPIX * 4, IT = (NV + DL_NTHR - 1) / DL_NTHR;
     i32x4c rv[IT];
@@ -58,28 +54,16 @@
         bn_channel_tables(f, g, tid, aff, mr);
         aff_s[tid] = aff; mr_s[tid] = mr;
     }
-    if (!IW && blockIdx.x == 0 && blockIdx.y == 0) {
-        for (int i = tid; i < f.G * DL_C; i += DL_NTHR) {
-            float2 aff, mr;
-            bn_channel_tables(f, i / DL_C, i % DL_C, aff, mr);
-            f.affine[i] = aff; f.meanrstd[i] = mr;
-        }
-        bn_running_update(f, tid, DL_NTHR);
-    }
     {
         const i32x4c z = {0, 0, 0, 0};
         for (int i = tid * 16; i < (DL_ROWS - DL_NPIX) * DL_AP; i += DL_NTHR * 16)
             *reinterpret_cast<i32x4c*>(A_s + DL_NPIX * DL_AP + i) = z;
-        if (!IW)
-            for (int i = tid; i < DL_DLW * DL_DLW; i += DL_NTHR) dl_s[i] = 0.f;
-    }
-    bf16x8 wf[2], wd;
+    }
+    bf16x8 wf[2];
 #pragma unroll
     for (int ks = 0; ks < 2; ++ks)
 #pragma unroll
         for (int j = 0; j < 8; ++j) wf[ks][j] = r < 16 ? (bf16)a.w[(ks * 16 + 8 * h + j) * 16 + r] : (bf16)0.f;
-#pragma unroll
-    for (int j = 0; j < 8; ++j) wd[j] = (bf16)a.w[r * 16 + 8 * h + j];
     __syncthreads();
     {
         const int cv = tid & 3;
@@ -113,7 +97,7 @@
         }
     }
     __syncthreads();
-    if constexpr (IW) {
+    {
         const float* const timg = a.target + (long long)(n / a.rows_per_target) * (DL_OH * DL_OW);
         float ll = 0.f;
         for (int o = tid; o < DL_OH * DL_OW; o += DL_NTHR) {
@@ -139,34 +123,177 @@
             for (int w = 0; w < DL_WAVES; ++w) s += part[w];
             a.loglik[n] = s;
         }
-        return;
-    }
+    }
+}
+
+__global__ __launch_bounds__(dls::MAX_WAVES * 64, dls::MAX_WAVES / 2) void dec_last_half_kernel(const DecLastFusedArgs a) {
+    constexpr int WAVES = dls::MAX_WAVES, NTHR = WAVES * 64;
+    static_assert( DL_AP == dls::AP && DL_PP == dls::PP && DL_DLW == dls::DLW && DL_C == dls::C && DL_IW == dls::IW &&
+                  DL_NPIX == dls::NPIX && DL_OW == dls::OW, "thin_split_geo.h describes this layer");
+    extern __shared__ __attribute__((aligned(16))) char smem[];
+    char* const A_s = smem + dls::OFF_A;
+    float* const P_s = reinterpret_cast<float*>(smem + dls::OFF_P);
+    char* const pat_s = smem + dls::OFF_P;
+    float* const dl_s = reinterpret_cast<float*>(smem + dls::OFF_DL);
+    char* const scr_s = smem + dls::OFF_DL;
+    float2* const aff_s = reinterpret_cast<float2*>(smem + dls::OFF_TAB);
+    float2* const mr_s = aff_s + DL_C;
+    __shared__ float part[dls::MAX_WAVES];
+    __shared__ float2 wsum[dls::MAX_WAVES][DL_C];
+
+    const int tid = threadIdx.x, lane = tid & 63;
+    const int wave = __builtin_amdgcn_readfirstlane(tid >> 6);
+    const int r = lane & 31, h = lane >> 5;
+    const int n_in_g = blockIdx.x, g = blockIdx.y, z = blockIdx.z;
+    const long long n = (long long)g * a.B + n_in_g;
+    const BnFinalizeArgs& f = a.fin;
+    const bool bwd = g < a.bwd_groups;
+    const int st_pix = dls::st_pix(z), own_pix = dls::own_pix(z), own_tiles = dls::own_tiles(z);
+
+    constexpr int NV = dls::ST_ROWS_MAX * 4, IT = NV / NTHR;
+    static_assert(NV % NTHR == 0, "whole trips");
+    i32x4c rv[IT];
+    const int gp0 = dls::st_lo(z) * DL_IW;
+#pragma unroll
+    for (int it = 0; it < IT; ++it) {
+        const int v = tid + it * NTHR, gp = gp0 + (v >> 2);
+        rv[it] = i32x4c{0, 0, 0, 0};
+        if ((v >> 2) < st_pix && (unsigned)gp < (unsigned)DL_NPIX)
+            rv[it] = *reinterpret_cast<const i32x4c*>(a.r + ((size_t)n * DL_NPIX + gp) * DL_C + (size_t)(v & 3) * 8);
+    }
+    constexpr int ND = dls::LO_ROWS_MAX * DL_DLW, DT = (ND + NTHR - 1) / NTHR;
+    float tv[DT];
+    {
+        const float* const timg = a.target ? a.target + (long long)n_in_g * (DL_OH * DL_OW) : nullptr;
+        const int lo_lo = dls::lo_lo(z), lo_rows = dls::lo_rows(z);
+#pragma unroll
+        for (int k = 0; k < DT; ++k) {
+            const int i = tid + k * NTHR;
+            const int l = i / DL_DLW, c = i - l * DL_DLW, oy = lo_lo + l;
+            tv[k] = 0.f;
+            if (timg && l < lo_rows && c >= 1 && c <= DL_OW && (unsigned)oy < (unsigned)DL_OH) tv[k] = timg[oy * DL_OW + c - 1];
+        }
+    }
+    if (tid < DL_C) {
+        float2 aff, mr;
+        bn_channel_tables(f, g, tid, aff, mr);
+        aff_s[tid] = aff; mr_s[tid] = mr;
+    }
+    if (blockIdx.x == 0 && blockIdx.y == 0 && blockIdx.z == 0) {
+        for (int i = tid; i < f.G * DL_C; i += NTHR) {
+            float2 aff, mr;
+            bn_channel_tables(f, i / DL_C, i % DL_C, aff, mr);
+            f.affine[i] = aff; f.meanrstd[i] = mr;
+        }
+        bn_running_update(f, tid, NTHR);
+    }
+    bf16x8 wf[2], wd;
+#pragma unroll
+    for (int ks = 0; ks < 2; ++ks)
+#pragma unroll
+        for (int j = 0; j < 8; ++j) wf[ks][j] = r < 16 ? (bf16)a.w[(ks * 16 + 8 * h + j) * 16 + r] : (bf16)0.f;
+    {
+        const f32x4 w0 = *reinterpret_cast<const f32x4*>(a.w + r * 16 + 8 * h), w1 = *reinterpret_cast<const f32x4*>(a.w + r * 16 + 8 * h + 4);
+#pragma unroll
+        for (int j = 0; j < 4; ++j) { wd[j] = (bf16)w0[j]; wd[4 + j] = (bf16)w1[j]; }
+    }
+#pragma unroll
+    for (int k = 0; k < DT; ++k) {
+        const int i = tid + k * NTHR;
+        if (i < ND) dl_s[i] = tv[k];
+    }
+    __syncthreads();
+    {
+        const int cv = tid & 3;
+        float sc[8], sh[8];
+#pragma unroll
+        for (int j = 0; j < 8; ++j) { const float2 t = aff_s[cv * 8 + j]; sc[j] = t.x; sh[j] = t.y; }
+#pragma unroll
+        for (int it = 0; it < IT; ++it) {
+            const int v = tid + it * NTHR, gp = gp0 + (v >> 2);
+            bf16x8 o;
+            if ((v >> 2) < st_pix && (unsigned)gp < (unsigned)DL_NPIX) {
+                const bf16x8 x = __builtin_bit_cast(bf16x8, rv[it]);
+#pragma unroll
+                for (int j = 0; j < 8; ++j) o[j] = (bf16)swish_fast((float)x[j] * sc[j] + sh[j]);
+            } else {
+#pragma unroll
+                for (int j = 0; j < 8; ++j) o[j] = (bf16)0.f;
+            }
+            *reinterpret_cast<bf16x8*>(A_s + (v >> 2) * DL_AP + cv * 16) = o;
+        }
+    }
+    __syncthreads();
+    for (int t = wave; t < dls::st_tiles(z); t += WAVES) {
+        f32x16 acc;
+#pragma unroll
+        for (int j = 0; j < 16; ++j) acc[j] = 0.f;
+        const char* ap = A_s + (t * 32 + r) * DL_AP + h * 16;
+        const bf16x8 a0 = *reinterpret_cast<const bf16x8*>(ap), a1 = *reinterpret_cast<const bf16x8*>(ap + 32);
+        acc = __builtin_amdgcn_mfma_f32_32x32x16_bf16(a0, wf[0], acc, 0, 0, 0);
+        acc = __builtin_amdgcn_mfma_f32_32x32x16_bf16(a1, wf[1], acc, 0, 0, 0);
+        if (r < 16) {
+#pragma unroll
+            for (int j = 0; j < 16; ++j) P_s[(t * 32 + (j & 3) + 8 * (j >> 2) + 4 * h) * 16 + r] = acc[j];
+        }
+    }
+    constexpr int NT = (dls::OWN_ROWS_MAX / 32 + WAVES - 1) / WAVES;
+    const __amdgpu_buffer_rsrc_t orsrc = __builtin_amdgcn_make_buffer_rsrc(
+        a.db, 0, (int)((size_t)a.bwd_groups * a.B * DL_NPIX * DL_C * 2), 0x00020000);
+    const __amdgpu_buffer_rsrc_t rrsrc = __builtin_amdgcn_make_buffer_rsrc(
+        const_cast<bf16*>(a.r), 0, (int)((size_t)a.bwd_groups * a.B * DL_NPIX * DL_C * 2), 0x00020000);
+    unsigned off0[NT], off1[NT];
+    i32x4c rr0[NT], rr1[NT];
+#pragma unroll
+    for (int k = 0; k < NT; ++k) {
+        const int t = wave + k * WAVES;
+        const unsigned base = (unsigned)((n * DL_NPIX + dls::own_lo(z) * DL_IW + t * 32) * (DL_C * 2)) + (unsigned)((lane >> 4) * 16);
+        const int p0 = t * 32 + (lane & 15), p1 = p0 + 16;
+        off0[k] = p0 < own_pix ? base + (unsigned)((lane & 15) * (DL_C * 2)) : 0x40000000u;
+        off1[k] = p1 < own_pix ? base + (unsigned)((16 + (lane & 15)) * (DL_C * 2)) : 0x40000000u;
+        rr0[k] = i32x4c{0, 0, 0, 0}; rr1[k] = i32x4c{0, 0, 0, 0};
+        if (bwd) {
+            rr0[k] = __builtin_bit_cast(i32x4c, __builtin_amdgcn_raw_buffer_load_b128(rrsrc, (int)off0[k], 0, 0));
+            rr1[k] = __builtin_bit_cast(i32x4c, __builtin_amdgcn_raw_buffer_load_b128(rrsrc, (int)off1[k], 0, 0));
+        }
+    }
+    __syncthreads();
     float loss = 0.f;
-    for (int o = tid; o < DL_OH * DL_OW; o += DL_NTHR) {
-        const int oy = o / DL_OW, ox = o - oy * DL_OW;
-        const int kh0 = (oy + 1) & 1, kw0 = (ox + 1) & 1;
-        const int iy0 = (oy + 1 - kh0) >> 1, ix0 = (ox + 1 - kw0) >> 1;
-        float acc = 0.f;
-#pragma unroll
-        for (int ty = 0; ty < 2; ++ty)
-#pragma unroll
-            for (int tx = 0; tx < 2; ++tx) {
-                const int iy = iy0 - ty, ix = ix0 - tx;
-                if ((unsigned)iy < (unsigned)DL_IH && (unsigned)ix < (unsigned)DL_IW)
-                    acc += P_s[(iy * DL_IW + ix) * 16 + (kh0 + 2 * ty) * 4 + kw0 + 2 * tx];
-            }
-        const long long oidx = n * (DL_OH * DL_OW) + o;
-        const float p = __builtin_amdgcn_rcpf(1.0f + __expf(-acc));
-        if (a.logits) a.logits[oidx] = acc;
-        if (a.recon) a.recon[oidx] = p;
-        if (a.target) {
-            const float t = a.target[(long long)n_in_g * (DL_OH * DL_OW) + o];
-            const float lp = fmaxf(__logf(p), -100.f), lq = fmaxf(__logf(1.0f - p), -100.f);
-            loss += -(t * lp + (1.0f - t) * lq);
-            const float pq = p * (1.0f - p);
-            const float dl = a.coef[g] * (p - t) / fmaxf(pq, 1e-12f) * pq;
-            if (a.dlogit) a.dlogit[oidx] = dl;
-            dl_s[(oy + 1) * DL_DLW + ox + 1] = dl;
+    {
+        const int lo_lo = dls::lo_lo(z), st_lo = dls::st_lo(z), out_lo = dls::out_lo(z), out_hi = dls::out_hi(z);
+        const float coef = a.coef[g];
+        for (int o = tid; o < dls::lo_rows(z) * DL_OW; o += NTHR) {
+            const int l = o / DL_OW, ox = o - l * DL_OW, oy = lo_lo + l;
+            if ((unsigned)oy >= (unsigned)DL_OH) continue;
+            const int kh0 = (oy + 1) & 1, kw0 = (ox + 1) & 1;
+            const int iy0 = (oy + 1 - kh0) >> 1, ix0 = (ox + 1 - kw0) >> 1;
+            float acc = 0.f;
+#pragma unroll
+            for (int ty = 0; ty < 2; ++ty)
+#pragma unroll
+                for (int tx = 0; tx < 2; ++tx) {
+                    const int iy = iy0 - ty, ix = ix0 - tx, ixc = min(max(ix, 0), DL_IW - 1);
+                    const float pv = P_s[((iy - st_lo) * DL_IW + ixc) * 16 + (kh0 + 2 * ty) * 4 + kw0 + 2 * tx];
+                    acc += ix == ixc ? pv : 0.f;
+                }
+            const bool owned = oy >= out_lo && oy < out_hi;
+            const long long oidx = n * (DL_OH * DL_OW) + oy * DL_OW + ox;
+            const float p = __builtin_amdgcn_rcpf(1.0f + __expf(-acc));
+            if (owned) {
+                if (a.logits) a.logits[oidx] = acc;
+                if (a.recon) a.recon[oidx] = p;
+            }
+            if (a.target) {
+                const float t = dl_s[l * DL_DLW + ox + 1];
+                const float pq = p * (1.0f - p);
+                const float dl = coef * (p - t) / fmaxf(pq, 1e-12f) * pq;
+                if (owned) {
+                    const float lp = fmaxf(__logf(p), -100.f), lq = fmaxf(__logf(1.0f - p), -100.f);
+                    loss += -(t * lp + (1.0f - t) * lq);
+                    if (a.dlogit) a.dlogit[oidx] = dl;
+                }
+                dl_s[l * DL_DLW + ox + 1] = dl;
+            }
         }
     }
     if (a.loss_sum) {
@@ -176,67 +303,62 @@
     __syncthreads();
     if (a.loss_sum && tid == 0) {
         float s = 0.f;
-        for (int w = 0; w < DL_WAVES; ++w) s += part[w];
+        for (int w = 0; w < WAVES; ++w) s += part[w];
         atomicAdd(a.loss_sum + (blockIdx.x % MMVAE_LOSS_SLOTS) * 16 + g, s);
     }
     if (!bwd) return;
-    for (int px = tid; px < DL_ROWS; px += DL_NTHR) {
-        bf16x8 lo, hi;
-        if (px < DL_NPIX) {
-            const int iy = px / DL_IW, ix = px - iy * DL_IW;
-            const float* d0 = dl_s + (2 * iy) * DL_DLW + 2 * ix;
-#pragma unroll
-            for (int kw = 0; kw < 4; ++kw) {
-                lo[kw] = (bf16)d0[kw]; lo[4 + kw] = (bf16)d0[DL_DLW + kw];
-                hi[kw] = (bf16)d0[2 * DL_DLW + kw]; hi[4 + kw] = (bf16)d0[3 * DL_DLW + kw];
-            }
+    for (int i = tid; i < 2 * own_tiles * 32; i += NTHR) {
+        const int j = i >> 1, half = i & 1;
+        bf16x8 o;
+        if (j < own_pix) {
+            const float* d0 = dl_s + dls::dl_window(z, j, half);
+#pragma unroll
+            for (int kw = 0; kw < 4; ++kw) { o[kw] = (bf16)d0[kw]; o[4 + kw] = (bf16)d0[DL_DLW + kw]; }
         } else {
 #pragma unroll
-            for (int j = 0; j < 8; ++j) { lo[j] = (bf16)0.f; hi[j] = (bf16)0.f; }
-        }
-        *reinterpret_cast<bf16x8*>(pat_s + px * DL_PP) = lo;
-        *reinterpret_cast<bf16x8*>(pat_s + px * DL_PP + 16) = hi;
-    }
-    __syncthreads();
-    {
-        const __amdgpu_buffer_rsrc_t orsrc = __builtin_amdgcn_make_buffer_rsrc(
-            a.db, 0, (int)((size_t)a.bwd_groups * a.B * DL_NPIX * DL_C * 2), 0x00020000);
-        const __amdgpu_buffer_rsrc_t rrsrc = __builtin_amdgcn_make_buffer_rsrc(
-            const_cast<bf16*>(a.r), 0, (int)((size_t)a.bwd_groups * a.B * DL_NPIX * DL_C * 2), 0x00020000);
+            for (int e = 0; e < 8; ++e) o[e] = (bf16)0.f;
+        }
+        *reinterpret_cast<bf16x8*>(pat_s + j * DL_PP + half * 16) = o;
+    }
+    __syncthreads();
+    {
         const float2 af = aff_s[r], mr = mr_s[r];
         float s1 = 0.f, s2 = 0.f;
-        char* const scr = scr_s + wave * 2560;
-        for (int t = wave; t < DL_TILES; t += DL_WAVES) {
-            f32x16 acc;
-#pragma unroll
-            for (int j = 0; j < 16; ++j) acc[j] = 0.f;
-            const bf16x8 pa = *reinterpret_cast<const bf16x8*>(pat_s + (t * 32 + r) * DL_PP + h * 16);
-            acc = __builtin_amdgcn_mfma_f32_32x32x16_bf16(pa, wd, acc, 0, 0, 0);
-            const unsigned base = (unsigned)((n * DL_NPIX + t * 32) * (DL_C * 2)) + (unsigned)((lane >> 4) * 16);
-            const int p0 = t * 32 + (lane & 15), p1 = p0 + 16;
-            const unsigned off0 = p0 < DL_NPIX ? base + (unsigned)((lane & 15) * (DL_C * 2)) : 0x40000000u;
-            const unsigned off1 = p1 < DL_NPIX ? base + (unsigned)((16 + (lane & 15)) * (DL_C * 2)) : 0x40000000u;
-            const int left = DL_NPIX - t * 32;
-            if (left >= 32) cr_epilogue_tile<1, false>(acc, scr, lane, 32, off0, off1, orsrc, rrsrc, af.x, af.y, mr.x, mr.y, s1, s2, true);
-            else cr_epilogue_tile<1, true>(acc, scr, lane, left, off0, off1, orsrc, rrsrc, af.x, af.y, mr.x, mr.y, s1, s2, true);
+        char* const scr = scr_s + wave * dls::SCR;
+#pragma unroll
+        for (int k = 0; k < NT; ++k) {
+            const int t = wave + k * WAVES;
+            if (t < own_tiles) {
+                f32x16 acc;
+#pragma unroll
+                for (int j = 0; j < 16; ++j) acc[j] = 0.f;
+                const bf16x8 pa = *reinterpret_cast<const bf16x8*>(pat_s + (t * 32 + r) * DL_PP + h * 16);
+                acc = __builtin_amdgcn_mfma_f32_32x32x16_bf16(pa, wd, acc, 0, 0, 0);
+                const int left = own_pix - t * 32;
+                if (left >= 32) cr_epilogue_tile_r<1, false>(acc, scr, lane, 32, off0[k], off1[k], orsrc, rr0[k], rr1[k], af.x, af.y, mr.x, mr.y, s1, s2, true);
+                else cr_epilogue_tile_r<1, true>(acc, scr, lane, left, off0[k], off1[k], orsrc, rr0[k], rr1[k], af.x, af.y, mr.x, mr.y, s1, s2, true);
+            }
         }
         const float t1 = s1 + __shfl_xor(s1, 32, 64), t2 = s2 + __shfl_xor(s2, 32, 64);
-        if (h == 0) {
-            const int slot = (int)(blockIdx.x + wave) % MMVAE_STAT_SLOTS;
-            float2* d = a.red + ((size_t)g * MMVAE_STAT_SLOTS + slot) * DL_C + r;
-            atomicAdd(&d->x, t1);
-            atomicAdd(&d->y, t2);
-        }
-    }
-    __syncthreads();
+        if (h == 0) wsum[wave][r] = float2{t1, t2};
+    }
+    __syncthreads();
+    if (tid < DL_C) {
+        float2 t = wsum[0][tid];
+        for (int w = 1; w < WAVES; ++w) { t.x += wsum[w][tid].x; t.y += wsum[w][tid].y; }
+        const int slot = (int)(blockIdx.x + 8 * z) % MMVAE_STAT_SLOTS;
+        float2* d = a.red + ((size_t)g * MMVAE_STAT_SLOTS + slot) * DL_C + tid;
+        atomicAdd(&d->x, t.x);
+        atomicAdd(&d->y, t.y);
+    }
     {
         const int g4 = lane >> 4, q = (lane & 15) >> 2, p = lane & 3;
         f32x16 acc;
 #pragma unroll
         for (int j = 0; j < 16; ++j) acc[j] = 0.f;
-        for (int ks = wave; ks < DL_ROWS / 16; ks += DL_WAVES) {
+        for (int ks = wave; ks < own_tiles * 2; ks += WAVES) {
             const int row = ks * 16 + 8 * h + q;
-            const char* a0 = A_s + row * DL_AP + (16 * (g4 & 1) + 4 * p) * 2;
+            const char* a0 = A_s + (row + DL_IW) * DL_AP + (16 * (g4 & 1) + 4 * p) * 2;
             const char* b0 = pat_s + row * DL_PP + (4 * p) * 2;
             const bf16x8 af2 = tr_pair_d(a0, a0 + 4 * DL_AP);
             const bf16x8 bf2 = tr_pair_d(b0, b0 + 4 * DL_PP);
@@ -251,11 +373,11 @@
     __syncthreads();
     {
         const float* wred = reinterpret_cast<const float*>(scr_s);
-        float* dst = a.wslab + ((size_t)g * gridDim.x + blockIdx.x) * DL_C * 16;
-        for (int i = tid; i < DL_C * 16; i += DL_NTHR) {
+        float* dst = a.wslab + (((size_t)g * gridDim.x + blockIdx.x) * dls::HALVES + z) * DL_C * 16;
+        for (int i = tid; i < DL_C * 16; i += NTHR) {
             float s = 0.f;
 #pragma unroll
-            for (int w = 0; w < DL_WAVES; ++w) s += wred[w * DL_C * 16 + i];
+            for (int w = 0; w < WAVES; ++w) s += wred[w * DL_C * 16 + i];
             dst[i] = s;
         }
     }
@@ -578,14 +700,15 @@
 int launch_dec_last_mfma(const DecLastFusedArgs& a, hipStream_t s) {
     static std::atomic<unsigned> attr_set{0};
     if (mmvae_first_use_on_device(attr_set)) {
-        hipFuncSetAttribute(reinterpret_cast<const void*>(&dec_last_mfma_kernel<false>), hipFuncAttributeMaxDynamicSharedMemorySize, DL_LDS);
-        hipFuncSetAttribute(reinterpret_cast<const void*>(&dec_last_mfma_kernel<true>), hipFuncAttributeMaxDynamicSharedMemorySize, DL_LDS);
+        hipFuncSetAttribute(reinterpret_cast<const void*>(&dec_last_mfma_kernel), hipFuncAttributeMaxDynamicSharedMemorySize, DL_LDS);
+        hipFuncSetAttribute(reinterpret_cast<const void*>(&dec_last_half_kernel), hipFuncAttributeMaxDynamicSharedMemorySize, dls::LDS);
     }
     if (a.loglik) {
         MMVAE_REQUIRE(a.target && a.rows_per_target >= 1 && a.bwd_groups == 0 && !a.fin.training, "dec_last_mfma: importance-weighted form arguments");
-        MMVAE_LAUNCH(dec_last_mfma_kernel<true>, dim3(a.B, a.G), dim3(DL_NTHR), DL_LDS, s, a);
+        MMVAE_LAUNCH(dec_last_mfma_kernel, dim3(a.B, a.G), dim3(DL_NTHR), DL_LDS, s, a);
         return mmvae_check_launch("dec_last_mfma_iw");
     }
-    MMVAE_LAUNCH(dec_last_mfma_kernel<false>, dim3(a.B, a.G), dim3(DL_NTHR), DL_LDS, s, a);
-    return mmvae_check_launch("dec_last_mfma");
-}
+    MMVAE_LAUNCH(dec_last_half_kernel, dim3(a.B, a.G, dls::HALVES), dim3(dls::MAX_WAVES * 64), dls::LDS, s, a);
+    return mmvae_check_launch("dec_last_half");
+}
+int dec_last_wgrad_partials(const DecLastFusedArgs& a) { return dec_last_mfma_applies(a) ? dls::HALVES : dec_last_fused_strips(a.IH); }
diff --git a/multimodal-vae_amd/csrc/multimnist.hip b/multimodal-vae_amd/csrc/multimnist.hip
--- a/multimodal-vae_amd/csrc/multimnist.hip
+++ b/multimodal-vae_amd/csrc/multimnist.hip
@@ -481,7 +481,8 @@
     return MMVAE_OK;
 }
 
-int fused_tail(MMPlan& P, int groups, int training, const ConvTLastFwdArgs* last, int last_groups, int fused_bwd_groups, hipStream_t s) {
+int fused_tail(MMPlan& P, int groups, int training, const ConvTLastFwdArgs* last, int last_groups, int fused_bwd_groups, hipStream_t s,
+               float* dlogit_dump = nullptr) {
     MMPlan::W& w = P.w;
     const int B = P.B;
     const ConvL& L = P.convT[2];
@@ -497,12 +498,12 @@
     f.num_batches_tracked = P.buf.bn_nbt + b.idx;
     f.updates_per_group = 1; f.affine = w.aff_d[2]; f.meanrstd = w.mr_d[2]; f.eps = BN_EPS; f.momentum = BN_MOM; f.training = training;
     f.skip_update_mask = groups > 1 ? P.dec_skip_mask : 0u;
-    x.target = last->target; x.logits = last->logits; x.recon = last->recon; x.dlogit = nullptr;
+    x.target = last->target; x.logits = last->logits; x.recon = last->recon; x.dlogit = dlogit_dump;
     for (int k = 0; k < 4; ++k) x.coef[k] = last->coef[k];
     x.loss_sum = last->loss_sum;
     if (last->loglik) { x.loglik = last->loglik; x.rows_per_target = last->rows_per_target; x.B = last->rows; }
     if (x.bwd_groups > 0) {
-        const int chunks = x.bwd_groups * B * (dec_last_mfma_applies(x) ? 1 : dec_last_fused_strips(25));
+        const int chunks = x.bwd_groups * B * dec_last_wgrad_partials(x);
         x.wslab = P.slab.take((size_t)chunks * 32 * 16);
         MMVAE_REQUIRE(x.wslab != nullptr, "fused decoder tail: the weight-gradient slab pool is exhausted");
         x.db = w.d3; x.red = w.red_d[2];
@@ -1287,15 +1288,30 @@
         return MMVAE_OK;
     }
     MMVAE_TRY(use_ws(P, ws, wsb, false));
-    if (std::string(layer) == "dec_last_fused") {
+    if (std::string(layer) == "dec_last_fused" || std::string(layer) == "dec_last_fused_reduce") {
+        const bool reduce = std::string(layer) == "dec_last_fused_reduce";
         ConvTLastFwdArgs last{};
         last.target = (const float*)P->w.tmp_f32; last.loss_sum = P->w.sums;
         last.coef[0] = last.coef[1] = 1.f / (float)(P->B * NPIX);
+        if (reduce) { last.logits = P->w.logits; last.recon = P->w.recon; }
         for (int i = 0; i < iters; ++i) {
             P->slab.reset(P->w.slab, P->w.slab_floats);
-            MMVAE_TRY(fused_tail(*P, 3, 1, &last, 2, 2, s));
+            MMVAE_TRY(fused_tail(*P, 3, 1, &last, 2, 2, s, reduce ? P->w.dlogit : nullptr));
+            if (reduce) MMVAE_TRY(launch_wgrad_reduce(&P->slab, s));
             P->slab.jobs.clear(); P->slab.ring_jobs.clear();
         }
+        return MMVAE_OK;
+    }
+    if (std::string(layer) == "enc_conv1_mfma") {
+        const PackDesc& d = P->pk.d[P->conv[0].pk_fwd[0]];
+        for (int i = 0; i < iters; ++i)
+            MMVAE_TRY(launch_conv1_fwd_mfma(P->w.tmp_f32, P->B, P->buf.packed + d.dst_off, d.Kpad, P->w.r1, P->w.a1, s));
+        return MMVAE_OK;
+    }
+    if (std::string(layer) == "enc_conv1_wgrad_mfma") {
+        const PackDesc& gd = P->gk.d[P->conv[0].gk[0]];
+        for (int i = 0; i < iters; ++i)
+            MMVAE_TRY(launch_conv1_wgrad_mfma(P->w.tmp_f32, P->B, P->w.d1e, P->buf.gpk + gd.dst_off, gd.Kpad, s));
         return MMVAE_OK;
     }
     WgradParams wg{};
@@ -1316,7 +1332,9 @@
     MMPlan& P = *const_cast<MMPlan*>(Pc);
     GemmParams g{};
     WgradParams wg{};
-    if (std::string(layer) == "dec_last_fused") return 3.0 * 2.0 * 2 * P.B * 625 * 16 * 32;
+    if (std::string(layer) == "dec_last_fused" || std::string(layer) == "dec_last_fused_reduce")
+        return 3.0 * 2.0 * 2 * P.B * 625 * 16 * 32;
+    if (std::string(layer) == "enc_conv1_mfma" || std::string(layer) == "enc_conv1_wgrad_mfma") return 2.0 * P.B * 640 * 16 * 32;
     if (P.bound && layer_wgrad(P, layer, wg)) return wgrad_flops(wg);
     if (!P.bound || !layer_gemm(P, layer, g)) return -1.0;
     return gemm_flops(g);
@@ -1337,6 +1355,8 @@
         if (name == d + "_dgrad" || name == d + "_wgrad") return conv(P.convT[l], 2 * B);
     }
     if (name == "dec_last_wgrad" || name == "dec_last_dgrad_gemm") return conv(P.convT[3], 2 * B);
+    if (name == "dec_last_fused" || name == "dec_last_fused_reduce") return 3.0 * conv(P.convT[3], 2 * B);
+    if (name == "enc_conv1_mfma" || name == "enc_conv1_wgrad_mfma") return conv(P.conv[0], B);
     return mm_layer_flops(Pc, layer);
 }
 double mm_layer_algo_bytes(const MMPlan* Pc, const char* layer) {
@@ -1356,6 +1376,9 @@
         if (name == d + "_dgrad") return conv(P.convT[l], 2 * B, false);
         if (name == d + "_wgrad") return conv(P.convT[l], 2 * B, true);
     }
+    if (name == "enc_conv1_mfma") return (double)B * (2500 * 4.0 + 2 * 625 * 32 * 2.0) + 32 * 16 * 2.0;
+    if (name == "enc_conv1_wgrad_mfma") return (double)B * (2500 * 4.0 + 625 * 32 * 2.0) + 32 * 16 * 4.0;
+    if (name == "dec_last_fused" || name == "dec_last_fused_reduce") return 2.0 * B * (2 * 625 * 32 * 2.0 + 2500 * 4.0) + 32 * 16 * 4.0;
     return 0.0;
 }
 long long mm_debug_offset(MMPlan* P, const char* name) {
diff --git a/multimodal-vae_amd/csrc/thin.h b/multimodal-vae_amd/csrc/thin.h
--- a/multimodal-vae_amd/csrc/thin.h
+++ b/multimodal-vae_amd/csrc/thin.h
@@ -50,6 +50,7 @@
 };
 int dec_last_fused_strips(int IH);
 bool dec_last_mfma_applies(const DecLastFusedArgs& a);
+int dec_last_wgrad_partials(const DecLastFusedArgs& a);
 int launch_dec_last_mfma(const DecLastFusedArgs& a, hipStream_t s);
 int launch_dec_last_fused(const DecLastFusedArgs& a, hipStream_t s);
 bool dec_last_ca_applies(const DecLastFusedArgs& a);
diff --git a/multimodal-vae_amd/csrc/thin_split_geo.h b/multimodal-vae_amd/csrc/thin_split_geo.h
--- /dev/null
+++ b/multimodal-vae_amd/csrc/thin_split_geo.h
@@ -0,0 +1,99 @@
+#pragma once
+
+namespace c1s {
+
+constexpr int IMG = 50, OH = 25, NPIX = 625, C = 32;
+constexpr int HALVES = 2, TILES = 10, PIX = TILES * 32;
+constexpr int IROWS = 28;
+constexpr int IW = 54;
+constexpr int PP = 48;
+
+constexpr int pix0(int z) { return z * PIX; }
+constexpr int npix(int z) { return NPIX - pix0(z) < PIX ? NPIX - pix0(z) : PIX; }
+constexpr int oy_lo(int z) { return pix0(z) / OH; }
+constexpr int oy_hi(int z) { return (pix0(z) + npix(z) - 1) / OH; }
+constexpr int y0(int z) { return 2 * oy_lo(z) - 1; }
+constexpr int ld_row0(int z) { return y0(z) < 0 ? 0 : y0(z); }
+constexpr int ld_rows(int z) { return (y0(z) + IROWS - 1 > IMG - 1 ? IMG - 1 : y0(z) + IROWS - 1) - ld_row0(z) + 1; }
+constexpr int pad_row(int z) { return y0(z) < 0 ? 0 : IROWS - 1; }
+constexpr int LD_ROWS = 27, LD_VEC = LD_ROWS * (IMG / 2);
+
+constexpr int cell(int z, int y, int x) { return (y - y0(z)) * IW + x + 2; }
+constexpr int window(int z, int lp, int half) {
+    return cell(z, 2 * ((pix0(z) + lp) / OH) - 1 + 2 * half, 2 * ((pix0(z) + lp) % OH) - 1);
+}
+
+static_assert(pix0(0) == 0 && pix0(1) == npix(0) && pix0(1) + npix(1) == NPIX && HALVES == 2, "the halves partition the 625 pixels");
+static_assert(2 * oy_hi(0) + 2 <= y0(0) + IROWS - 1 && 2 * oy_hi(1) + 2 <= y0(1) + IROWS - 1, "staged rows cover every row a window reads");
+static_assert(ld_rows(0) == LD_ROWS && ld_rows(1) == LD_ROWS, "both halves load 27 image rows");
+static_assert((ld_row0(0) * IMG) % 2 == 0 && (ld_row0(1) * IMG) % 2 == 0 && (IMG * IMG) % 2 == 0 && IMG % 2 == 0,
+              "8-byte vectors: a half starts on an even float of an image, an image on an even float of the batch, a vector stays in its row");
+static_assert(y0(0) + pad_row(0) == -1 && y0(1) + pad_row(1) == IMG, "exactly one staged row of each half lies outside the image");
+static_assert((IW * 2) % 4 == 0, "a pair of columns is one aligned 4-byte word of LDS");
+
+constexpr int IMG_BYTES = (IROWS * IW * 2 + 15) / 16 * 16;
+constexpr int HALF_CU = 160 * 1024 / 2;
+
+constexpr int F_WAVES = 4, F_NTHR = F_WAVES * 64;
+constexpr int F_OFF_IMG = 0, F_OFF_PAT = F_OFF_IMG + IMG_BYTES, F_OFF_SCR = F_OFF_PAT + PIX * PP, F_LDS = F_OFF_SCR + F_WAVES * 2560;
+static_assert(F_LDS <= HALF_CU, "conv1 forward: two workgroups per CU");
+
+}
+
+namespace dls {
+
+constexpr int IH = 25, IW = 25, OH = 50, OW = 50, C = 32, NPIX = IH * IW;
+constexpr int HALVES = 2;
+constexpr int own_lo(int z) { return z ? 13 : 0; }
+constexpr int own_hi(int z) { return z ? IH : 13; }
+constexpr int own_pix(int z) { return (own_hi(z) - own_lo(z)) * IW; }
+constexpr int own_tiles(int z) { return (own_pix(z) + 31) / 32; }
+constexpr int st_lo(int z) { return own_lo(z) - 1; }
+constexpr int st_rows(int z) { return own_hi(z) - own_lo(z) + 2; }
+constexpr int st_pix(int z) { return st_rows(z) * IW; }
+constexpr int st_tiles(int z) { return (st_pix(z) + 31) / 32; }
+constexpr int lo_lo(int z) { return 2 * own_lo(z) - 1; }
+constexpr int lo_rows(int z) { return 2 * (own_hi(z) - own_lo(z)) + 2; }
+constexpr int out_lo(int z) { return 2 * own_lo(z); }
+constexpr int out_hi(int z) { return 2 * own_hi(z); }
+constexpr int ST_ROWS_MAX = 384, OWN_ROWS_MAX = 352, LO_ROWS_MAX = 28;
+constexpr int AP = 80;
+constexpr int PP = 48;
+constexpr int DLW = 52;
+constexpr int SCR = 2560;
+constexpr int MAX_WAVES = 8;
+
+constexpr int st_pixel(int z, int iy, int ix) { return (iy - st_lo(z)) * IW + ix; }
+constexpr int dl_cell(int z, int oy, int ox) { return (oy - lo_lo(z)) * DLW + ox + 1; }
+constexpr int dl_window(int z, int j, int half) { return dl_cell(z, 2 * (own_lo(z) + j / IW) - 1 + 2 * half, 2 * (j % IW) - 1); }
+
+static_assert(own_lo(0) == 0 && own_hi(0) == own_lo(1) && own_hi(1) == IH, "the owned input rows partition [0, 25)");
+static_assert(out_lo(0) == 0 && out_hi(0) == out_lo(1) && out_hi(1) == OH, "the owned output rows partition [0, 50)");
+static_assert(st_lo(0) <= own_lo(0) - 1 && st_lo(0) + st_rows(0) >= own_hi(0) + 1 && st_lo(1) <= own_lo(1) - 1 && st_lo(1) + st_rows(1) >= own_hi(1) + 1,
+              "one halo row on each side");
+static_assert((lo_lo(0) + 1) / 2 - 1 >= st_lo(0) && (lo_lo(0) + lo_rows(0)) / 2 < st_lo(0) + st_rows(0) &&
+              (lo_lo(1) + 1) / 2 - 1 >= st_lo(1) && (lo_lo(1) + lo_rows(1)) / 2 < st_lo(1) + st_rows(1), "staged rows cover every row a logit reads");
+static_assert(2 * own_lo(0) - 1 >= lo_lo(0) && 2 * (own_hi(0) - 1) + 2 < lo_lo(0) + lo_rows(0) &&
+              2 * own_lo(1) - 1 >= lo_lo(1) && 2 * (own_hi(1) - 1) + 2 < lo_lo(1) + lo_rows(1), "the dlogit rows cover every row a window reads");
+static_assert(st_tiles(0) * 32 <= ST_ROWS_MAX && st_tiles(1) * 32 <= ST_ROWS_MAX && own_tiles(0) * 32 <= OWN_ROWS_MAX && own_tiles(1) * 32 <= OWN_ROWS_MAX &&
+              lo_rows(0) <= LO_ROWS_MAX && lo_rows(1) <= LO_ROWS_MAX, "buffer extents");
+static_assert(OWN_ROWS_MAX + IW + 4 <= ST_ROWS_MAX, "the weight gradient reads A at owned row + 25 (+ 4: transposed pair) inside the tile");
+static_assert((IW * AP) % 16 == 0, "the owned pixels start on a 16-byte boundary of A");
+
+constexpr int OFF_A = 0;
+constexpr int OFF_P = OFF_A + ST_ROWS_MAX * AP;
+constexpr int P_BYTES = ST_ROWS_MAX * 64;
+constexpr int OFF_DL = OFF_P + P_BYTES;
+constexpr int DL_BYTES = LO_ROWS_MAX * DLW * 4;
+constexpr int SCR_BYTES = MAX_WAVES * SCR;
+constexpr int OFF_TAB = OFF_DL + (DL_BYTES > SCR_BYTES ? DL_BYTES : SCR_BYTES);
+constexpr int LDS = OFF_TAB + 2 * C * 8;
+constexpr int STATIC_LDS = MAX_WAVES * 4 + MAX_WAVES * C * 8;
+static_assert(OWN_ROWS_MAX * PP <= P_BYTES, "the patches reuse the P buffer");
+static_assert(MAX_WAVES * C * 16 * 4 <= SCR_BYTES, "the weight-gradient partials reuse the epilogue scratch");
+static_assert(OFF_P % 16 == 0 && OFF_DL % 16 == 0 && OFF_TAB % 16 == 0, "16-byte aligned regions");
+static_assert(LDS <= (160 * 1024 - STATIC_LDS) / 2, "two workgroups per CU");
+constexpr int P_LAST = 2, PAT_FIRST = 3, DL_LAST = 3, SCR_FIRST = 4;
+static_assert(P_LAST < PAT_FIRST && DL_LAST < SCR_FIRST, "regions that share space are never live together");
+
+}
```

Measured after the change: 1803 ELBO-steps/s, median of 6. 2.9% higher.
